# thepowerfuldeez/stylemc

Measured on AMD Instinct MI355X. Metric: find_direction images/sec @ FFHQ-1024 bs=4, 1/2/4/8 GPU; dir cosine-sim vs ref, higher is better.
Workload: dtype f32; 1 GPU; find_direction step: 2x StyleGAN2 S-space synthesis fwd + 1 bwd (HIP), CLIP ViT-B/32 fwd/bwd (HIP), IR-SE50 fwd/bwd (HIP), SGD; resolution=1024, batch_per_gpu=4, global_batch=4, n_seeds=129, parallelism=dp1, clip_type=small, clip_impl=hip, id_impl=hip, batched_loss_pairs=True, landmarks_loss_coef=0, conv_products=x3, vit_products=fp32, irse_products=fp32, direction_finite=True, world_size=1

## Files before the change

### include/stylemc_hip.h

```cpp
#ifndef STYLEMC_HIP_H
#define STYLEMC_HIP_H

#include <stdint.h>

#ifdef __cplusplus
extern "C" {
#endif

#define SMC_ABI_VERSION 6

#define SMC_OK 0
#define SMC_ERR_INVALID 1
#define SMC_ERR_UNSUPPORTED 2
#define SMC_ERR_LAUNCH 3

#define SMC_ACT_LINEAR 1
#define SMC_ACT_RELU 2
#define SMC_ACT_LRELU 3
#define SMC_ACT_TANH 4
#define SMC_ACT_SIGMOID 5
#define SMC_ACT_ELU 6
#define SMC_ACT_SELU 7
#define SMC_ACT_SOFTPLUS 8
#define SMC_ACT_SWISH 9
// ... 21 lines not shown
    int out_sy, out_sx;
    const float* wk;
    const float* wino_u;
    const void* wk_x3;
} smc_conv_phase;

int64_t smc_conv_weights_x3_bytes(int ntaps, int cin, int cout);
int smc_conv_weights_x3(const float* wk, int ntaps, int cin, int cout, void* wk_x3, void* stream);

#define SMC_EPI_STORE 0
#define SMC_EPI_MODACT 1
#define SMC_EPI_PRELU 2
#define SMC_EPI_PRELU_GRAD 3
#define SMC_EPI_AFFINE 4

typedef struct {
    int mode;
    const float* d;
    const float* noise;
    int64_t noise_nstride;
    const float* noise_strength;
    const float* bias;
    int act;
    float alpha, gain, clamp;
    float* u_save;
    const float* scale_c;
    const float* alpha_c;
    const float* act_ref;
    const float* residual;
    int residual_stride;
    int grad_from_y;
} smc_conv_epilogue;

int smc_conv_gemm_last_x3(void);
int64_t smc_conv_gemm_workspace_size(int n, int cin, int cout, int y_h, int y_w, const smc_conv_phase* phases,
                                     int nphases);

#define SMC_ROUTE_SPLIT_K 1
#define SMC_ROUTE_PER_SAMPLE 2
#define SMC_ROUTE_PRESCALE 4
#define SMC_ROUTE_WSAMPLE 8
int smc_conv_gemm_last_route(void);
int smc_conv_gemm_last_route_flags(void);
int smc_conv_gemm_route_count(void);
const char* smc_conv_gemm_route_name(int route);

int smc_conv_gemm_f32(const float* x, int n, int cin, int in_h, int in_w, float* y, int cout, int y_h, int y_w,
                      const smc_conv_phase* phases, int nphases, const float* s_in, const smc_conv_epilogue* epi,
                      float* workspace, int64_t workspace_bytes, void* stream);

int64_t smc_conv_gemm_aux_workspace_size(int n, int cin, int cout, int y_h, int y_w, const smc_conv_phase* phases,
                                         int nphases);
int smc_conv_gemm_aux_f32(const float* x, int n, int cin, int in_h, int in_w, float* y, int cout, int y_h, int y_w,
                          const smc_conv_phase* phases, int nphases, const float* s_in, const smc_conv_epilogue* epi,
                          float* workspace, int64_t workspace_bytes, void* stream);

int smc_conv3x3_wino_supported(int n, int cin, int cout, int h, int w);
int smc_conv3x3_wino_f32(const float* x, int n, int cin, int h, int w, float* y, int cout, const float* uw,
                         const float* s_in, const smc_conv_epilogue* epi, void* stream);
int64_t smc_conv3x3_wino_workspace_size(int n, int cin, int cout, int h, int w);
int smc_conv3x3_wino_ws_f32(const float* x, int n, int cin, int h, int w, float* y, int cout, const float* uw,
                            const float* s_in, const smc_conv_epilogue* epi, float* workspace, int64_t workspace_bytes,
                            void* stream);
int smc_set_wino_x3(int mode);
int smc_wino_weights_f32(const float* w, int cout, int cin, int flip, float* uw, void* stream);

int smc_conv3x3_wino4_supported(int n, int cin, int cout, int h, int w);
int smc_conv3x3_wino4_f32(const float* x, int n, int cin, int h, int w, float* y, int cout, const float* uw,
                          const float* s_in, const smc_conv_epilogue* epi, void* stream);
int smc_wino4_weights_f32(const float* w, int cout, int cin, int flip, float* uw, void* stream);

int smc_wino_sp_supported(int n, int cin, int cout, int h, int w);
int64_t smc_wino_sp_workspace_size(int n, int cin, int cout, int h, int w);
int smc_wino_taps_f32(const smc_conv_phase* phase, int cin, int cout, float* uw, void* stream);
int smc_conv3x3_wino_sp_f32(const float* x, int n, int cin, int h, int w, float* y, int cout, const float* uw,
                            const smc_conv_epilogue* epi, float* workspace, int64_t workspace_bytes, void* stream);

int smc_modconv_epilogue_f32(const float* src, int nsplit, int64_t split_stride, float* y, int n, int c, int h,
                             int w, const smc_conv_epilogue* epi, void* stream);

int smc_modconv_blur_act_f32(const float* t, int nsplit, int64_t split_stride, float* y, int n, int c, int t_h,
                             int t_w, int t_pitch, int y_h, int y_w, const float* f, int fh, int fw, int padx0,
                             int pady0, float fgain, int flip, const smc_conv_epilogue* epi, void* stream);

int smc_modconv_blur_act_bwd_f32(const float* g, const float* u, float* dt, float* dd, int n, int c, int u_h, int u_w,
                                 int t_h, int t_w, int t_pitch, const float* f, int fh, int fw, int padx0, int pady0,
                                 float fgain, int flip, const smc_conv_epilogue* epi, void* workspace,
                                 int64_t workspace_bytes, void* stream);
int64_t smc_modconv_blur_act_bwd_workspace_size(int n, int c, int u_h, int u_w, int t_h, int t_w);

int smc_row_dot_f32(const float* a, int64_t lda, const float* b, int64_t ldb, float* out, int rows, int len,
                    void* stream);

int smc_direction_head_f32(const float* e, int64_t lde, const float* src, int64_t lds, const float* t, float* loss,
                           float* grad, int rows, int len, float eps, void* stream);

int smc_modconv_demod_f32(const float* s, const float* wsq, float* d, int n, int cin, int cout, float eps,
                          void* stream);

int smc_modconv_act_bwd_f32(const float* g, const float* u, float* du, float* dd, int n, int c, int h, int w,
                            const smc_conv_epilogue* epi, void* workspace, int64_t workspace_bytes, void* stream);
int64_t smc_modconv_act_bwd_workspace_size(int n, int c, int h, int w);

int smc_channel_dot_f32(const float* a, const float* b, const float* scale, float* out, float* a_scaled,
                        int64_t rows, int64_t len, int accumulate, void* stream);

int smc_modconv_demod_bwd_f32(const float* s, const float* d, const float* dd, const float* wsq, float* ds, int n,
                              int cin, int cout, void* stream);

int smc_torgb_fwd_f32(const float* x, const float* w, const float* s, const float* b, float* y, int n, int cin,
                      int cout, int h, int w_, float clamp, void* stream);

int smc_torgb_bwd_f32(const float* g, const float* y, const float* w, const float* s, float* dx, int n, int cin,
                      int cout, int h, int w_, float clamp, int scale, int accumulate, void* stream);

int smc_torgb_act_bwd_f32(const float* g_rgb, const float* y_rgb, const float* w, const float* s, float clamp_rgb,
                          const float* g_next, const float* y, float* du, int n, int cin, int cout, int h, int w_,
                          const smc_conv_epilogue* epi, void* stream);

int smc_face_crop_f32(const float* x, int64_t planes, int in_h, int in_w, int pool_h, int pool_w, int crop_y0,
                      int crop_x0, int crop_h, int crop_w, int out_h, int out_w, float* y, void* stream);
int smc_face_crop_bwd_f32(const float* dy, int64_t planes, int in_h, int in_w, int pool_h, int pool_w, int crop_y0,
                          int crop_x0, int crop_h, int crop_w, int out_h, int out_w, float* dx, void* stream);

int smc_clip_unprocess_f32(const float* img, int n, int channels, int in_h, int in_w, int out_h, int out_w,
                           const float* mean, const float* std_, float* y, void* stream);
int smc_clip_unprocess_bwd_f32(const float* img, const float* dy, int n, int channels, int in_h, int in_w, int out_h,
                               int out_w, const float* mean, const float* std_, float* dimg, void* stream);
int smc_clip_preprocess_nada_f32(const float* img, int n, int channels, int in_h, int in_w, int out_h, int out_w,
                                 const float* mean, const float* std_, float* y, void* stream);
int smc_clip_preprocess_nada_bwd_f32(const float* img, const float* dy, int n, int channels, int in_h, int in_w,
                                     int out_h, int out_w, const float* mean, const float* std_, float* dimg,
                                     void* stream);

#define SMC_LIN_ACT_NONE 0
#define SMC_LIN_ACT_QUICKGELU 1

typedef struct {
    const float* bias;
    const float* dact_pre;
    int ld_dact;
    int act;
    float* pre_save;
    int ld_pre;
    const float* residual;
    int ld_res;
} smc_linear_epilogue;

int64_t smc_linear_workspace_size(int M, int N, int K);
int smc_linear_f32(const float* a, int lda, const float* b, int ldb, float* c, int ldc, int M, int N, int K,
                   const smc_linear_epilogue* epi, float* workspace, int64_t workspace_bytes, void* stream);

int64_t smc_linear_counter_ints(int M, int N);
int smc_linear_ex_f32(const float* a, int lda, const float* b, int ldb, float* c, int ldc, int M, int N, int K,
                      const smc_linear_epilogue* epi, float* workspace, int64_t workspace_bytes, const float* bt,
                      const void* planes, int* counters, void* stream);
int64_t smc_linear_x3_planes_bytes(int K, int N);
int smc_linear_x3_planes(const float* b, int ldb, int K, int N, void* planes, void* stream);

#define SMC_LIN_REDUCE_NONE 0
#define SMC_LIN_REDUCE_KERNEL 1
#define SMC_LIN_REDUCE_INLAUNCH 2
int smc_linear_last_route(void);
int smc_linear_last_nsplit(void);
int smc_linear_last_reduce(void);
int smc_linear_route_count(void);
// ... 87 lines not shown
```

### stylemc_amd/_hip.py

```python
import contextlib
import ctypes
import os
import threading

import torch

PKG = os.path.dirname(os.path.abspath(__file__))
LIB_PATH = os.environ.get("SMC_HIP_LIB", os.path.join(PKG, "_lib", "libstylemc_hip.so"))

c_int, c_int64, c_float, c_void_p, c_char_p = ctypes.c_int, ctypes.c_int64, ctypes.c_float, ctypes.c_void_p, ctypes.c_char_p

ACT_CODES = {"linear": 1, "relu": 2, "lrelu": 3, "tanh": 4, "sigmoid": 5, "elu": 6, "selu": 7, "softplus": 8,
             "swish": 9}
EPI_STORE, EPI_MODACT, EPI_PRELU, EPI_PRELU_GRAD, EPI_AFFINE = 0, 1, 2, 3, 4
ROUTE_SPLIT_K, ROUTE_PER_SAMPLE, ROUTE_PRESCALE, ROUTE_WSAMPLE = 1, 2, 4, 8


class ConvPhase(ctypes.Structure):
    _fields_ = [("ntaps", c_int), ("tap_dy", c_int * 9), ("tap_dx", c_int * 9), ("in_stride", c_int),
                ("out_h", c_int), ("out_w", c_int), ("out_oy", c_int), ("out_ox", c_int), ("out_sy", c_int),
                ("out_sx", c_int), ("wk", c_void_p), ("wino_u", c_void_p), ("wk_x3", c_void_p)]


class ConvEpilogue(ctypes.Structure):
    _fields_ = [("mode", c_int), ("d", c_void_p), ("noise", c_void_p), ("noise_nstride", c_int64),
                ("noise_strength", c_void_p), ("bias", c_void_p), ("act", c_int), ("alpha", c_float),
                ("gain", c_float), ("clamp", c_float), ("u_save", c_void_p), ("scale_c", c_void_p),
                ("alpha_c", c_void_p), ("act_ref", c_void_p), ("residual", c_void_p), ("residual_stride", c_int),
                ("grad_from_y", c_int)]


class LinearEpilogue(ctypes.Structure):
    _fields_ = [("bias", c_void_p), ("dact_pre", c_void_p), ("ld_dact", c_int), ("act", c_int),
                ("pre_save", c_void_p), ("ld_pre", c_int), ("residual", c_void_p), ("ld_res", c_int)]


class VitConfig(ctypes.Structure):
    _fields_ = [("width", c_int), ("layers", c_int), ("heads", c_int), ("patch", c_int), ("grid", c_int),
                ("out_dim", c_int), ("in_ch", c_int), ("ln_eps", c_float), ("products", c_int)]


LIN_ACT_NONE, LIN_ACT_QUICKGELU = 0, 1
LIN_REDUCE_NONE, LIN_REDUCE_KERNEL, LIN_REDUCE_INLAUNCH = 0, 1, 2

P = c_void_p
_SIGS = {
    "smc_abi_version": (c_int, []),
    "smc_set_plan_batch": (c_int, [c_int, c_int]),
    "smc_conv_gemm_last_x3": (c_int, []),
    "smc_conv_gemm_last_route": (c_int, []),
    "smc_conv_gemm_last_route_flags": (c_int, []),
    "smc_conv_gemm_route_count": (c_int, []),
    "smc_conv_gemm_route_name": (c_char_p, [c_int]),
    "smc_last_error": (c_char_p, []),
    "smc_bias_act_f32": (c_int, [P, P, P, P, P, P, c_int64, c_int64, c_int64, c_int, c_int, c_float, c_float, c_float,
                                 P]),
    "smc_upfirdn2d_f32": (c_int, [P, P, P, c_int64] + [c_int] * 15 + [c_float, P]),
    "smc_conv_gemm_workspace_size": (c_int64, [c_int, c_int, c_int, c_int, c_int, P, c_int]),
    "smc_conv_gemm_f32": (c_int, [P, c_int, c_int, c_int, c_int, P, c_int, c_int, c_int, P, c_int, P, P, P, c_int64,
                                  P]),
    "smc_conv_gemm_aux_workspace_size": (c_int64, [c_int, c_int, c_int, c_int, c_int, P, c_int]),
    "smc_conv_gemm_aux_f32": (c_int, [P, c_int, c_int, c_int, c_int, P, c_int, c_int, c_int, P, c_int, P, P, P,
                                      c_int64, P]),
    "smc_conv_weights_x3_bytes": (c_int64, [c_int, c_int, c_int]),
    "smc_conv_weights_x3": (c_int, [P, c_int, c_int, c_int, P, P]),
    "smc_conv3x3_wino_supported": (c_int, [c_int, c_int, c_int, c_int, c_int]),
    "smc_conv3x3_wino_f32": (c_int, [P, c_int, c_int, c_int, c_int, P, c_int, P, P, P, P]),
    "smc_conv3x3_wino_workspace_size": (c_int64, [c_int, c_int, c_int, c_int, c_int]),
    "smc_set_wino_x3": (c_int, [c_int]),
    "smc_conv3x3_wino_ws_f32": (c_int, [P, c_int, c_int, c_int, c_int, P, c_int, P, P, P, P, c_int64, P]),
    "smc_wino_weights_f32": (c_int, [P, c_int, c_int, c_int, P, P]),
    "smc_conv3x3_wino4_supported": (c_int, [c_int, c_int, c_int, c_int, c_int]),
    "smc_conv3x3_wino4_f32": (c_int, [P, c_int, c_int, c_int, c_int, P, c_int, P, P, P, P]),
    "smc_wino4_weights_f32": (c_int, [P, c_int, c_int, c_int, P, P]),
    "smc_wino_sp_supported": (c_int, [c_int, c_int, c_int, c_int, c_int]),
    "smc_wino_sp_workspace_size": (c_int64, [c_int, c_int, c_int, c_int, c_int]),
    "smc_wino_taps_f32": (c_int, [P, c_int, c_int, P, P]),
    "smc_conv3x3_wino_sp_f32": (c_int, [P, c_int, c_int, c_int, c_int, P, c_int, P, P, P, c_int64, P]),
    "smc_modconv_epilogue_f32": (c_int, [P, c_int, c_int64, P, c_int, c_int, c_int, c_int, P, P]),
    "smc_modconv_blur_act_f32": (c_int, [P, c_int, c_int64, P, c_int, c_int, c_int, c_int, c_int, c_int, c_int, P,
                                         c_int, c_int, c_int, c_int, c_float, c_int, P, P]),
    "smc_modconv_blur_act_bwd_f32": (c_int, [P, P, P, P, c_int, c_int, c_int, c_int, c_int, c_int, c_int, P, c_int,
                                             c_int, c_int, c_int, c_float, c_int, P, P, c_int64, P]),
    "smc_modconv_blur_act_bwd_workspace_size": (c_int64, [c_int] * 6),
    "smc_modconv_demod_f32": (c_int, [P, P, P, c_int, c_int, c_int, c_float, P]),
    "smc_row_dot_f32": (c_int, [P, c_int64, P, c_int64, P, c_int, c_int, P]),
    "smc_direction_head_f32": (c_int, [P, c_int64, P, c_int64, P, P, P, c_int, c_int, c_float, P]),
    "smc_modconv_act_bwd_f32": (c_int, [P, P, P, P, c_int, c_int, c_int, c_int, P, P, c_int64, P]),
    "smc_modconv_act_bwd_workspace_size": (c_int64, [c_int] * 4),
    "smc_channel_dot_f32": (c_int, [P, P, P, P, P, c_int64, c_int64, c_int, P]),
    "smc_modconv_demod_bwd_f32": (c_int, [P, P, P, P, P, c_int, c_int, c_int, P]),
    "smc_torgb_fwd_f32": (c_int, [P, P, P, P, P, c_int, c_int, c_int, c_int, c_int, c_float, P]),
    "smc_torgb_bwd_f32": (c_int, [P, P, P, P, P, c_int, c_int, c_int, c_int, c_int, c_float, c_int, c_int, P]),
    "smc_torgb_act_bwd_f32": (c_int, [P, P, P, P, c_float, P, P, P, c_int, c_int, c_int, c_int, c_int, P, P]),
    "smc_face_crop_f32": (c_int, [P, c_int64] + [c_int] * 10 + [P, P]),
    "smc_face_crop_bwd_f32": (c_int, [P, c_int64] + [c_int] * 10 + [P, P]),
    "smc_clip_unprocess_f32": (c_int, [P] + [c_int] * 6 + [P, P, P, P]),
    "smc_clip_unprocess_bwd_f32": (c_int, [P, P] + [c_int] * 6 + [P, P, P, P]),
    "smc_clip_preprocess_nada_f32": (c_int, [P] + [c_int] * 6 + [P, P, P, P]),
    "smc_clip_preprocess_nada_bwd_f32": (c_int, [P, P] + [c_int] * 6 + [P, P, P, P]),
    "smc_linear_workspace_size": (c_int64, [c_int, c_int, c_int]),
    "smc_linear_f32": (c_int, [P, c_int, P, c_int, P, c_int, c_int, c_int, c_int, P, P, c_int64, P]),
    "smc_linear_counter_ints": (c_int64, [c_int, c_int]),
    "smc_linear_ex_f32": (c_int, [P, c_int, P, c_int, P, c_int, c_int, c_int, c_int, P, P, c_int64, P, P, P, P]),
    "smc_linear_x3_planes_bytes": (c_int64, [c_int, c_int]),
    "smc_linear_x3_planes": (c_int, [P, c_int, c_int, c_int, P, P]),
    "smc_linear_last_route": (c_int, []),
    "smc_linear_last_nsplit": (c_int, []),
    "smc_linear_last_reduce": (c_int, []),
    "smc_linear_route_count": (c_int, []),
    "smc_linear_route_name": (c_char_p, [c_int]),
    "smc_layernorm_fwd_f32": (c_int, [P, c_int64, P, P, P, c_int64, P, P, c_int, c_int, c_float, P]),
    "smc_layernorm_bwd_f32": (c_int, [P, c_int64, P, c_int64, P, P, P, P, c_int64, P, c_int64, c_int, c_int, P]),
    "smc_attention_fwd_f32": (c_int, [P, P, P, c_int, c_int, c_int, c_int, c_float, P]),
    "smc_attention_bwd_f32": (c_int, [P, P, P, P, c_int, c_int, c_int, c_int, c_float, P]),
    "smc_attention_causal_fwd_f32": (c_int, [P, P, c_int, c_int, c_int, c_int, c_float, P]),
    "smc_patch_im2col_f32": (c_int, [P, P, c_int, c_int, c_int, c_int, c_int, P]),
    "smc_vit_packed_floats": (c_int64, [P]),
    "smc_vit_saved_floats": (c_int64, [P, c_int]),
    "smc_vit_pack_x3": (c_int, [P, P, P]),
    "smc_vit_workspace_bytes": (c_int64, [P, c_int]),
    "smc_vit_forward_f32": (c_int, [P, P, P, c_int, P, P, P, c_int64, P]),
    "smc_vit_backward_f32": (c_int, [P, P, P, c_int, c_int, P, P, P, c_int64, P]),
    "smc_irse_saved_floats": (c_int64, [P, c_int]),
    "smc_irse_workspace_bytes": (c_int64, [P, c_int]),
    "smc_irse_forward_f32": (c_int, [P, P, c_int, P, P, P, c_int64, P]),
    "smc_irse_backward_f32": (c_int, [P, P, c_int, c_int, P, P, P, c_int64, P]),
}

_lib = None
_lock = threading.Lock()


def exported_symbols():
    return sorted(_SIGS)


def load(path=None):
    global _lib
    if _lib is not None and path is None:
        return _lib
    with _lock:
        if _lib is not None and path is None:
            return _lib
        p = path or LIB_PATH
        if not os.path.exists(p):
            raise RuntimeError(f"stylemc_amd: HIP kernel library not found at {p}; build it with "
                               f"`python -m stylemc_amd.build` (there is no CPU fallback)")
        lib = ctypes.CDLL(p, mode=ctypes.RTLD_LOCAL)
        for name, (res, args) in _SIGS.items():
            fn = getattr(lib, name)
            fn.restype = res
            fn.argtypes = args
        if lib.smc_abi_version() != 6:
            raise RuntimeError("stylemc_amd: ABI version mismatch, rebuild the library")
        if path is None:
            _lib = lib
        return lib


def check(rc, name):
    if rc != 0:
        msg = load().smc_last_error().decode(errors="replace")
        raise RuntimeError(f"{name} failed (code {rc}): {msg}")
# ... 89 lines not shown
```

### stylemc_amd/csrc/conv_gemm.hip

```cpp
#include <algorithm>
#include <cstdlib>
#include <type_traits>

#include "common.hpp"

namespace {

constexpr int BK = 16;
constexpr int NT = 256;
typedef float f32x16 __attribute__((ext_vector_type(16)));

struct PhaseDev {
    int ntaps;
    int dy[9];
    int dx[9];
    int in_stride;
    int out_h, out_w, out_oy, out_ox, out_sy, out_sx;
    const float* wk;
    int64_t wstride;
    const short* wx3;
    int64_t wx3_stride;
};

struct GemmParams {
    const float* x;
    int n, cin, in_h, in_w;
    float* y;
    int cout, y_h, y_w;
    PhaseDev ph[4];
    int nphases;
    const float* s;
    int mode;
    const float* d;
    const float* noise;
    int64_t noise_nstride;
    const float* noise_strength;
    const float* bias;
    int act;
    float alpha, gain, clamp;
    float* u_save;
    smc::EpiExt ext;
    int nsplit;
    int64_t split_stride;
    int per_sample;
    int ntn;
};

template <int WO, int WM, int TO, int TM>
__device__ __forceinline__ void gemm_epilogue(const GemmParams& p, const PhaseDev& ph, const f32x16 (&acc)[TO][TM],
                                              int m0, int o0, int M, int hw_out, int split, int wo, int wm, int kh,
                                              int l32, float* lds) {
    constexpr int BO = WO * TO * 32;
    constexpr int BM = WM * TM * 32;
    const int64_t plane = (int64_t)p.y_h * p.y_w;
    if (p.nsplit > 1) {
        float* dst = p.y + (int64_t)split * p.split_stride;
#pragma unroll
        for (int j = 0; j < TM; ++j) {
            const int mc = m0 + wm * TM * 32 + j * 32 + l32;
            if (mc >= M) continue;
            const int en = mc / hw_out;
            const int erem = mc - en * hw_out;
            const int ea = erem / ph.out_w;
            const int64_t pix = (int64_t)(ph.out_oy + ph.out_sy * ea) * p.y_w + ph.out_ox + ph.out_sx * (erem - ea * ph.out_w);
#pragma unroll
            for (int i = 0; i < TO; ++i)
#pragma unroll
                for (int r = 0; r < 16; ++r) {
                    const int o = o0 + wo * TO * 32 + i * 32 + (r & 3) + 8 * (r >> 2) + 4 * kh;
                    if (o < p.cout) dst[((int64_t)en * p.cout + o) * plane + pix] = acc[i][j][r];
                }
        }
        return;
    }
    const int tid = threadIdx.x;
    const int en0 = m0 / hw_out;
    const bool one_img = (min(m0 + BM, M) - 1) / hw_out == en0;
    const int mode = p.mode;
    __syncthreads();
    for (int t = tid; t < BO; t += NT) {
        const int o = o0 + t;
        float mul = 1.f, add = 0.f, al = 0.f;
        if (o < p.cout) {
            if (mode == SMC_EPI_MODACT) {
                mul = (p.d && one_img ? p.d[(int64_t)en0 * p.cout + o] : 1.f) * (p.ext.scale_c ? p.ext.scale_c[o] : 1.f);
                add = p.bias ? p.bias[o] : 0.f;
            } else if (mode == SMC_EPI_PRELU || mode == SMC_EPI_AFFINE) {
                mul = p.ext.scale_c ? p.ext.scale_c[o] : 1.f;
                add = p.bias ? p.bias[o] : 0.f;
            }
            if ((mode == SMC_EPI_PRELU || mode == SMC_EPI_PRELU_GRAD) && p.ext.alpha_c) al = p.ext.alpha_c[o];
        }
        lds[t] = mul;
        lds[BO + t] = add;
        lds[2 * BO + t] = al;
    }
    __syncthreads();
    const float nstr = p.noise_strength ? *p.noise_strength : 1.f;
    const int rs = p.ext.rs;
    const int rh = p.y_h / rs, rw = p.y_w / rs;
    auto body = [&](auto mode_c, auto kind_c) {
        constexpr int MODE = decltype(mode_c)::value;
        constexpr int KIND = decltype(kind_c)::value;
        constexpr bool EX_REF = MODE == SMC_EPI_PRELU_GRAD;
#pragma unroll
        for (int j = 0; j < TM; ++j) {
            const int mc = m0 + wm * TM * 32 + j * 32 + l32;
            if (mc >= M) continue;
            const int en = mc / hw_out;
            const int erem = mc - en * hw_out;
            const int ea = erem / ph.out_w;
            const int eb = erem - ea * ph.out_w;
            const int yy = ph.out_oy + ph.out_sy * ea;
            const int xx = ph.out_ox + ph.out_sx * eb;
            const int64_t pix = (int64_t)yy * p.y_w + xx;
            const bool res_here = p.ext.residual && yy % rs == 0 && xx % rs == 0;
            const bool need_ex = EX_REF || p.ext.residual;
            float nz = 0.f;
            if (MODE == SMC_EPI_MODACT && p.noise) nz = p.noise[en * p.noise_nstride + pix] * nstr;
#pragma unroll
            for (int i = 0; i < TO; ++i) {
                const int ol0 = wo * TO * 32 + i * 32 + 4 * kh;
                float ex[16];
                if (need_ex) {
#pragma unroll
                    for (int r = 0; r < 16; ++r) {
                        const int o = min(o0 + ol0 + (r & 3) + 8 * (r >> 2), p.cout - 1);
                        if (EX_REF) ex[r] = p.ext.act_ref[((int64_t)en * p.cout + o) * plane + pix];
                        else ex[r] = res_here ? p.ext.residual[(((int64_t)en * p.cout + o) * rh + yy / rs) * rw + xx / rs] : 0.f;
// ... 150 lines not shown
            ws_[q] = s_on_w ? sblk[ci0 + wkk] : 1.f;
        }
    };
    auto store_step = [&](int stage) {
        float* Ws = smem + stage * TILE;
        float* Xs = Ws + BKT * BO;
#pragma unroll
        for (int r = 0; r < XR; ++r) {
            float v = xr[r];
            if (s_on_x) {
                const float4 sv = sr[r / 4];
                v *= (r & 3) == 0 ? sv.x : (r & 3) == 1 ? sv.y : (r & 3) == 2 ? sv.z : sv.w;
            }
            if constexpr (!BUF) v = xok ? v : 0.f;
            Xs[(kr0 + r) * BM + ml] = v;
        }
#pragma unroll
        for (int q = 0; q < WPT; ++q) {
            const int v = tid + q * NT;
            const int wkk = v / (BO / 4), wc4 = v - wkk * (BO / 4);
            float4 w = wr[q];
            const float sc = (o0 + wc4 * 4 >= p.cout) ? 0.f : ws_[q];
            w.x *= sc; w.y *= sc; w.z *= sc; w.w *= sc;
            if (v < WV) *reinterpret_cast<float4*>(&Ws[wkk * BO + wc4 * 4]) = w;
        }
    };

    f32x16 acc[TO][TM];
#pragma unroll
    for (int i = 0; i < TO; ++i)
#pragma unroll
        for (int j = 0; j < TM; ++j)
#pragma unroll
            for (int r = 0; r < 16; ++r) acc[i][j][r] = 0.f;

    const int kh = lane >> 5, l32 = lane & 31;
    int stage = 0;
    if (ks_begin < ks_end) {
        load_step(ks_begin);
        store_step(0);
    }
    __syncthreads();
    for (int ks = ks_begin; ks < ks_end; ++ks) {
        const bool more = ks + 1 < ks_end;
        if (more) load_step(ks + 1);
        const float* Ws = smem + stage * TILE;
        const float* Xs = Ws + BKT * BO;
        const float* wrow = Ws + kh * BO + wo * TO * 32 + l32;
        const float* xrow = Xs + kh * BM + wm * TM * 32 + l32;
#pragma unroll
        for (int k0 = 0; k0 < BKT; k0 += 16) {
            float af[8][TO], bf[8][TM];
#pragma unroll
            for (int q = 0; q < 8; ++q) {
#pragma unroll
                for (int i = 0; i < TO; ++i) af[q][i] = wrow[(k0 + 2 * q) * BO + i * 32];
#pragma unroll
                for (int j = 0; j < TM; ++j) bf[q][j] = xrow[(k0 + 2 * q) * BM + j * 32];
            }
            __builtin_amdgcn_sched_barrier(0);
#pragma unroll
            for (int q = 0; q < 8; ++q)
#pragma unroll
                for (int i = 0; i < TO; ++i)
#pragma unroll
                    for (int j = 0; j < TM; ++j)
                        acc[i][j] = __builtin_amdgcn_mfma_f32_32x32x2f32(af[q][i], bf[q][j], acc[i][j], 0, 0, 0);
        }
        if (more) store_step(stage ^ 1);
        __syncthreads();
        stage ^= 1;
    }

    gemm_epilogue<WO, WM, TO, TM>(p, ph, acc, m0, o0, M, hw_out, split, wo, wm, kh, l32, smem);
}


template <int WF>
struct WeightDma {
    static constexpr int ww = WF % 1024 == 0 ? 4 : 1;
    static constexpr int bytes = ww * 4;
};

template <int N>
__device__ __forceinline__ void wait_vmcnt() {
    asm volatile("s_waitcnt vmcnt(%0)" ::"n"(N) : "memory");
}

template <int WO, int WM, int TO, int TM, int BKT, int NST, int TAG = 0>
__global__ __launch_bounds__(NT, 2) void conv_gemm_lds_kernel(GemmParams p) {
    static_assert(WO * WM == 4, "4 waves");
    constexpr int BO = WO * TO * 32;
    constexpr int BM = WM * TM * 32;
    constexpr int TILE = BKT * (BO + BM);
    constexpr int NCH = BM / 64;
    static_assert(NCH >= 1 && NCH <= 4 && 4 % NCH == 0, "BM in {64,128,256}");
    constexpr int RSTEP = 4 / NCH;
    constexpr int XI = BKT * NCH / 4;
    constexpr int WF = BKT * BO;
    constexpr int WW = WeightDma<WF>::ww;
    static_assert(WF % (256 * WW) == 0, "weight slab must split evenly over the 4 waves");
    constexpr int WI = WF / (256 * WW);
    constexpr int PER = XI + WI;
    static_assert(NST >= 2 && NST <= 4 && PER * (NST - 2) <= 63, "vmcnt range");
    __shared__ __attribute__((aligned(16))) float smem[NST * TILE];

    const int tid = threadIdx.x;
    const int lane = tid & 63;
    const int wave = __builtin_amdgcn_readfirstlane(tid >> 6);
    const int wo = wave / WM, wm = wave % WM;
    const int phase = blockIdx.z / p.nsplit;
    const int split = blockIdx.z - phase * p.nsplit;
    const PhaseDev& ph = p.ph[phase];
    const int hw_out = ph.out_h * ph.out_w;
    int tm = blockIdx.x, tn = blockIdx.y;
    if (p.ntn) {
        const int nwg = gridDim.x, orig = blockIdx.x;
        const int xcd = orig % 8, q8 = nwg / 8, r8 = nwg % 8;
        const int wgid = (xcd < r8 ? xcd * (q8 + 1) : r8 * (q8 + 1) + (xcd - r8) * q8) + orig / 8;
        tm = wgid / p.ntn;
        tn = wgid - tm * p.ntn;
    }
    int M = p.n * hw_out;
    int m0 = tm * BM;
    if (p.per_sample) {
        const int tps = (hw_out + BM - 1) / BM;
        const int nb = tm / tps;
        if (nb >= p.n) return;
        m0 = nb * hw_out + (tm - nb * tps) * BM;
        M = (nb + 1) * hw_out;
    }
    if (m0 >= M) return;
    const int o0 = tn * BO;
    const int cpk = p.cin / BKT;
    const int ks_total = ph.ntaps * cpk;
    const int ks_begin = (int)((int64_t)ks_total * split / p.nsplit);
    const int ks_end = (int)((int64_t)ks_total * (split + 1) / p.nsplit);

    const int cw = wave % NCH, r0 = wave / NCH;
    const int m = m0 + cw * 64 + lane;
    const bool mvalid = m < M;
    int nn = 0, a = 0, b = 0;
    if (mvalid) {
        nn = m / hw_out;
        const int rem = m - nn * hw_out;
        a = rem / ph.out_w;
        b = rem - a * ph.out_w;
    }
    const int in_hw = p.in_h * p.in_w;
    const __amdgpu_buffer_rsrc_t xrsrc = __builtin_amdgcn_make_buffer_rsrc(
        (void*)p.x, (short)0, (int)((int64_t)p.n * p.cin * in_hw * 4), 0x00020000);
    const int xvbase = nn * p.cin * in_hw * 4;
    const int ay = a * ph.in_stride, bx = b * ph.in_stride;
    const float* wk = ph.wk + (ph.wstride ? (int64_t)(m0 / hw_out) * ph.wstride : 0);

    auto issue = [&](int ks, int slot) {
        const int t = ks / cpk;
        const int ci0 = (ks - t * cpk) * BKT;
        const int iy = ay + ph.dy[t], ix = bx + ph.dx[t];
        const bool ok = mvalid && iy >= 0 && iy < p.in_h && ix >= 0 && ix < p.in_w;
        const int voff = ok ? xvbase + (iy * p.in_w + ix) * 4 : 0x7ffffff0;
        float* xs = smem + slot * TILE + BKT * BO;
#pragma unroll
        for (int j = 0; j < XI; ++j) {
            const int row = r0 + RSTEP * j;
            __builtin_amdgcn_raw_ptr_buffer_load_lds(
                xrsrc, (__attribute__((address_space(3))) void*)(xs + row * BM + cw * 64), 4, voff,
                (ci0 + row) * in_hw * 4, 0, 0);
        }
        float* ws = smem + slot * TILE;
        const float* wrow = wk + ((int64_t)t * p.cin + ci0) * p.cout + o0;
#pragma unroll
        for (int j = 0; j < WI; ++j) {
            const int f0 = (wave + 4 * j) * 64 * WW;
            const int f = f0 + lane * WW;
            const int row = f / BO, col = f - row * BO;
            const void* src = (const void*)(wrow + (int64_t)row * p.cout + col);
            auto* dst = (__attribute__((address_space(3))) void*)(ws + f0);
            if constexpr (WW == 4) __builtin_amdgcn_global_load_lds(src, dst, 16, 0, 0);
            else __builtin_amdgcn_global_load_lds(src, dst, 4, 0, 0);
        }
    };

    f32x16 acc[TO][TM];
#pragma unroll
    for (int i = 0; i < TO; ++i)
#pragma unroll
        for (int j = 0; j < TM; ++j)
#pragma unroll
            for (int r = 0; r < 16; ++r) acc[i][j][r] = 0.f;

    const int kh = lane >> 5, l32 = lane & 31;
    int issued = ks_begin;
#pragma unroll
    for (int q = 0; q < NST - 1; ++q) {
        if (issued < ks_end) {
            issue(issued, (issued - ks_begin) % NST);
            ++issued;
        }
    }
    for (int ks = ks_begin; ks < ks_end; ++ks) {
        const int ahead = issued - ks - 1;
        if constexpr (NST == 2) {
            wait_vmcnt<0>();
        } else if constexpr (NST == 3) {
            if (ahead >= 1) wait_vmcnt<PER>();
            else wait_vmcnt<0>();
        } else {
            if (ahead >= 2) wait_vmcnt<2 * PER>();
            else if (ahead == 1) wait_vmcnt<PER>();
            else wait_vmcnt<0>();
        }
        __builtin_amdgcn_s_barrier();
        asm volatile("" ::: "memory");
        const int slot = (ks - ks_begin) % NST;
        const float* Ws = smem + slot * TILE;
        const float* Xs = Ws + BKT * BO;
        const float* wrow = Ws + kh * BO + wo * TO * 32 + l32;
        const float* xrow = Xs + kh * BM + wm * TM * 32 + l32;
#pragma unroll
        for (int k0 = 0; k0 < BKT; k0 += 16) {
            float af[8][TO], bf[8][TM];
            auto frag = [&](int q) {
#pragma unroll
                for (int i = 0; i < TO; ++i) af[q][i] = wrow[(k0 + 2 * q) * BO + i * 32];
#pragma unroll
                for (int j = 0; j < TM; ++j) bf[q][j] = xrow[(k0 + 2 * q) * BM + j * 32];
            };
            frag(0);
            frag(1);
            __builtin_amdgcn_sched_barrier(0);
#pragma unroll
            for (int q = 0; q < 8; ++q) {
#pragma unroll
                for (int i = 0; i < TO; ++i)
#pragma unroll
                    for (int j = 0; j < TM; ++j)
                        acc[i][j] = __builtin_amdgcn_mfma_f32_32x32x2f32(af[q][i], bf[q][j], acc[i][j], 0, 0, 0);
                __builtin_amdgcn_sched_barrier(0);
                if (q == 0 && k0 == 0 && issued < ks_end) {
                    issue(issued, (issued - ks_begin) % NST);
                    ++issued;
                }
                if (q + 2 < 8) frag(q + 2);
                __builtin_amdgcn_sched_barrier(0);
            }
        }
        asm volatile("s_waitcnt lgkmcnt(0)" ::: "memory");
    }
    gemm_epilogue<WO, WM, TO, TM>(p, ph, acc, m0, o0, M, hw_out, split, wo, wm, kh, l32, smem);
}


typedef short bf16x8 __attribute__((ext_vector_type(8)));

__device__ __forceinline__ void x3_split8(const float (&x)[8], bf16x8 (&t)[3]) {
    unsigned u0[8], u1[8], u2[8];
#pragma unroll
    for (int j = 0; j < 8; ++j) {
        const unsigned u = __float_as_uint(x[j]);
        const float r1 = x[j] - __uint_as_float(u & 0xffff0000u);
        const unsigned v = __float_as_uint(r1);
        const float r2 = r1 - __uint_as_float(v & 0xffff0000u);
        u0[j] = u;
        u1[j] = v;
        u2[j] = __float_as_uint(r2);
    }
    typedef unsigned u32x4 __attribute__((ext_vector_type(4)));
    u32x4 w0, w1, w2;
#pragma unroll
    for (int j = 0; j < 4; ++j) {
        w0[j] = __builtin_amdgcn_perm(u0[2 * j + 1], u0[2 * j], 0x07060302u);
        w1[j] = __builtin_amdgcn_perm(u1[2 * j + 1], u1[2 * j], 0x07060302u);
        w2[j] = __builtin_amdgcn_perm(u2[2 * j + 1], u2[2 * j], 0x07060302u);
    }
    t[0] = __builtin_bit_cast(bf16x8, w0);
    t[1] = __builtin_bit_cast(bf16x8, w1);
    t[2] = __builtin_bit_cast(bf16x8, w2);
}

__device__ __forceinline__ f32x16 x3_mma(const bf16x8 (&a)[3], const bf16x8 (&b)[3], f32x16 acc) {
    acc = __builtin_amdgcn_mfma_f32_32x32x16_bf16(a[2], b[0], acc, 0, 0, 0);
    acc = __builtin_amdgcn_mfma_f32_32x32x16_bf16(a[1], b[1], acc, 0, 0, 0);
    acc = __builtin_amdgcn_mfma_f32_32x32x16_bf16(a[0], b[2], acc, 0, 0, 0);
    acc = __builtin_amdgcn_mfma_f32_32x32x16_bf16(a[1], b[0], acc, 0, 0, 0);
    acc = __builtin_amdgcn_mfma_f32_32x32x16_bf16(a[0], b[1], acc, 0, 0, 0);
    return __builtin_amdgcn_mfma_f32_32x32x16_bf16(a[0], b[0], acc, 0, 0, 0);
}

__global__ __launch_bounds__(256) void x3_weights_kernel(const float* wk, const float* s_in, short* out, int ntaps,
                                                         int cin, int cout, int n) {
    const int64_t per = (int64_t)ntaps * cin * cout;
    const int64_t total = per * n;
    for (int64_t e = blockIdx.x * (int64_t)blockDim.x + threadIdx.x; e < total; e += (int64_t)gridDim.x * blockDim.x) {
        const int ee = (int)(e & 7);
        int64_t r = e >> 3;
        const int o = (int)(r % cout);
        r /= cout;
        const int kq = (int)(r & 1);
        r >>= 1;
        const int c16 = (int)(r % (cin / 16));
        r /= cin / 16;
        const int t = (int)(r % ntaps);
        const int nn = (int)(r / ntaps);
        const int ci = c16 * 16 + kq * 8 + ee;
        const float v = wk[((int64_t)t * cin + ci) * cout + o] * (s_in ? s_in[(int64_t)nn * cin + ci] : 1.f);
        const unsigned u = __float_as_uint(v);
        const float r1 = v - __uint_as_float(u & 0xffff0000u);
        const unsigned w = __float_as_uint(r1);
        const float r2 = r1 - __uint_as_float(w & 0xffff0000u);
        const unsigned term[3] = {u >> 16, w >> 16, __float_as_uint(r2) >> 16};
        short* dst = out + nn * per * 3;
#pragma unroll
        for (int sidx = 0; sidx < 3; ++sidx)
            dst[((((int64_t)t * (cin / 16) + c16) * 3 + sidx) * 2 + kq) * ((int64_t)cout * 8) + (int64_t)o * 8 + ee] =
                (short)term[sidx];
    }
}

#ifndef SMC_X3_NST
#define SMC_X3_NST 2
#endif
#ifndef SMC_X3_K32_SMALL
#define SMC_X3_K32_SMALL 1
#endif
#ifndef SMC_X3_WO1
#define SMC_X3_WO1 1
#endif
#ifndef SMC_X3_WO1_K16
#define SMC_X3_WO1_K16 1
#endif
#ifndef SMC_X3_PROBE
#define SMC_X3_PROBE 0
#endif

#ifndef SMC_X3_WIDE
#define SMC_X3_WIDE 1
#endif

template <int WO, int WM, int TO, int TM, int BKT, int NST = SMC_X3_NST, int TAG = 0, bool AS = false>
__global__ __launch_bounds__(NT, 2) void conv_gemm_x3_kernel(GemmParams p) {
    static_assert(WO * WM == 4, "4 waves");
    static_assert(BKT % 16 == 0, "16-channel chunks");
    static_assert(!AS || (BKT == 16 && TM == 1 && NST == 2), "streamed A fragments: one 16-channel chunk per step");
    constexpr int BO = WO * TO * 32;
    constexpr int BM = WM * TM * 32;
    constexpr int NKC = BKT / 16;
    constexpr int WB = NKC * 6 * BO * 16;
    constexpr int XB = BKT * BM * 4;
    constexpr int STAGE = WB + XB;
    constexpr int NCH = BM / 64;
    static_assert(NCH >= 1 && NCH <= 4 && 4 % NCH == 0, "BM in {64,128,256}");
    constexpr int RSTEP = 4 / NCH;
    constexpr int XI = BKT * NCH / 4;
    static_assert(WB % 1024 == 0, "weight planes split into whole 1-KB DMAs");
    constexpr int WLI = WB / 1024;
    constexpr int WIW = (WLI + 3) / 4;
    constexpr int PER = XI + WIW;
    static_assert(NST >= 2 && NST <= 4 && PER * (NST - 2) <= 63, "vmcnt range");
    __shared__ __attribute__((aligned(16))) char smem[NST * STAGE];

    const int tid = threadIdx.x;
    const int lane = tid & 63;
    const int wave = __builtin_amdgcn_readfirstlane(tid >> 6);
    const int wo = wave / WM, wm = wave % WM;
    const int phase = blockIdx.z / p.nsplit;
    const int split = blockIdx.z - phase * p.nsplit;
    const PhaseDev& ph = p.ph[phase];
    const int hw_out = ph.out_h * ph.out_w;
    int tm = blockIdx.x, tn = blockIdx.y;
    if (p.ntn) {
// ... 302 lines not shown
#pragma unroll
        for (int j = 0; j < TM; ++j)
#pragma unroll
            for (int r = 0; r < 16; ++r) acc[i][j][r] = 0.f;

    const int kh = lane >> 5, l32 = lane & 31;
    if (ks_total > 0) issue(0, 0);
    for (int ks = 0; ks < ks_total; ++ks) {
        wait_vmcnt<0>();
        __builtin_amdgcn_s_barrier();
        asm volatile("" ::: "memory");
        const int slot = ks & 1;
        const float* Xs = smem + slot * STAGE + kh * PITCH + 3 + wm * TM * 32 + l32;
        const float* Ws = smem + slot * STAGE + C::XF + kh * BO + wo * TO * 32 + l32;
#pragma unroll
        for (int tt = 0; tt < 3; ++tt) {
#pragma unroll
            for (int k0 = 0; k0 < BKT; k0 += 8) {
                float af[4][TO], bf[4][TM];
#pragma unroll
                for (int q = 0; q < 4; ++q) {
#pragma unroll
                    for (int i = 0; i < TO; ++i) af[q][i] = Ws[(tt * BKT + k0 + 2 * q) * BO + i * 32];
#pragma unroll
                    for (int j = 0; j < TM; ++j) bf[q][j] = Xs[(k0 + 2 * q) * PITCH + tt + j * 32];
                }
                __builtin_amdgcn_sched_barrier(0);
#pragma unroll
                for (int q = 0; q < 4; ++q)
#pragma unroll
                    for (int i = 0; i < TO; ++i)
#pragma unroll
                        for (int j = 0; j < TM; ++j)
                            acc[i][j] = __builtin_amdgcn_mfma_f32_32x32x2f32(af[q][i], bf[q][j], acc[i][j], 0, 0, 0);
                __builtin_amdgcn_sched_barrier(0);
                if (tt == 0 && k0 == 0 && ks + 1 < ks_total) issue(ks + 1, slot ^ 1);
            }
        }
        asm volatile("s_waitcnt lgkmcnt(0)" ::: "memory");
    }
    gemm_epilogue<WO, WM, TO, TM>(p, ph, acc, m0, o0, p.n * hw, hw, 0, wo, wm, kh, l32, smem);
}

__global__ __launch_bounds__(256) void xscale_kernel(const float* x, const float* s, float* out, int64_t hw,
                                                     int64_t planes) {
    const int64_t per = hw / 4;
    const int64_t total = per * planes;
    for (int64_t v = blockIdx.x * (int64_t)blockDim.x + threadIdx.x; v < total; v += (int64_t)gridDim.x * blockDim.x) {
        const int64_t pl = v / per;
        const float sc = s[pl];
        float4 a = reinterpret_cast<const float4*>(x)[v];
        a.x *= sc; a.y *= sc; a.z *= sc; a.w *= sc;
        reinterpret_cast<float4*>(out)[v] = a;
    }
}

__global__ __launch_bounds__(256) void wscale_kernel(const float* wk, const float* s, float* out, int rows, int cin,
                                                     int cout, int n) {
    const int64_t per = (int64_t)rows * cout / 4;
    const int64_t total = per * n;
    for (int64_t v = blockIdx.x * (int64_t)blockDim.x + threadIdx.x; v < total; v += (int64_t)gridDim.x * blockDim.x) {
        const int64_t nn = v / per;
        const int64_t e = (v - nn * per) * 4;
        const int row = (int)(e / cout);
        float4 w = *reinterpret_cast<const float4*>(wk + e);
        const float sc = s[nn * cin + row % cin];
        w.x *= sc; w.y *= sc; w.z *= sc; w.w *= sc;
        *reinterpret_cast<float4*>(out + nn * (int64_t)rows * cout + e) = w;
    }
}


struct ConvTParams {
    const float* w[4][4];
};

template <int S>
struct ShiftPhases;
template <> struct ShiftPhases<0> { static constexpr int n = 4; static constexpr int p[4] = {0, 1, 2, 3}; };
template <> struct ShiftPhases<1> { static constexpr int n = 2; static constexpr int p[4] = {0, 1, 0, 0}; };
template <> struct ShiftPhases<2> { static constexpr int n = 2; static constexpr int p[4] = {0, 2, 0, 0}; };
template <> struct ShiftPhases<3> { static constexpr int n = 1; static constexpr int p[4] = {0, 0, 0, 0}; };

__host__ __device__ constexpr int shift_nph(int s) { return s == 0 ? 4 : (s == 3 ? 1 : 2); }

template <int S, int TO, int TM, int BKT, int BO, int BM>
__device__ __forceinline__ void convt_mma(const float* Ws, const float* Xs, int wo, int wm, int kh, int l32,
                                          f32x16 (&acc)[4][TO][TM]) {
    constexpr int NP = ShiftPhases<S>::n;
#pragma unroll
    for (int k0 = 0; k0 < BKT; k0 += 4) {
        float af[2][NP][TO], bf[2][TM];
#pragma unroll
        for (int q = 0; q < 2; ++q) {
            const int kk = k0 + 2 * q + kh;
#pragma unroll
            for (int j = 0; j < TM; ++j) bf[q][j] = Xs[kk * BM + wm * TM * 32 + j * 32 + l32];
#pragma unroll
            for (int ph = 0; ph < NP; ++ph)
#pragma unroll
                for (int i = 0; i < TO; ++i) af[q][ph][i] = Ws[(ph * BKT + kk) * BO + wo * TO * 32 + i * 32 + l32];
        }
        __builtin_amdgcn_sched_barrier(0);
#pragma unroll
        for (int q = 0; q < 2; ++q)
#pragma unroll
            for (int ph = 0; ph < NP; ++ph)
#pragma unroll
                for (int i = 0; i < TO; ++i)
#pragma unroll
                    for (int j = 0; j < TM; ++j)
                        acc[ShiftPhases<S>::p[ph]][i][j] = __builtin_amdgcn_mfma_f32_32x32x2f32(
                            af[q][ph][i], bf[q][j], acc[ShiftPhases<S>::p[ph]][i][j], 0, 0, 0);
    }
}

template <int WO, int WM, int TO, int TM, int BKT>
__global__ __launch_bounds__(NT, 1) void convt_gemm_kernel(GemmParams p, ConvTParams q) {
    static_assert(WO * WM == 4, "4 waves");
    constexpr int BO = WO * TO * 32;
    constexpr int BM = WM * TM * 32;
    constexpr int XR = BKT * BM / NT;
    constexpr int WV = BKT * BO / 4;
    constexpr int WPT = (WV + NT - 1) / NT;
    constexpr int TILE = BKT * (4 * BO + BM);
    static_assert(NT % BM == 0 && XR % 4 == 0, "thread->position map");
    __shared__ float smem[2 * TILE];

    const int tid = threadIdx.x, lane = tid & 63, wave = tid >> 6;
    const int wo = wave / WM, wm = wave % WM;
    const int gh = p.in_h + 1, gw = p.in_w + 1, hw_g = gh * gw;
    const int M = p.n * hw_g;
    const int m0 = blockIdx.x * BM;
    const int o0 = blockIdx.y * BO;
    const int split = blockIdx.z;
    const int cpk = p.cin / BKT;
    const int ks_total = 4 * cpk;
    const int ks_begin = (int)((int64_t)ks_total * split / p.nsplit);
    const int ks_end = (int)((int64_t)ks_total * (split + 1) / p.nsplit);

    const int ml = tid % BM, kr0 = (tid / BM) * XR;
    const int m = m0 + ml;
    const bool mvalid = m < M;
    int nn = 0, a = 0, b = 0;
    if (mvalid) {
        nn = m / hw_g;
        const int rem = m - nn * hw_g;
        a = rem / gw;
        b = rem - a * gw;
    }
    const int64_t in_hw = (int64_t)p.in_h * p.in_w;
    const float* xbase = p.x + (int64_t)nn * p.cin * in_hw + (int64_t)kr0 * in_hw;
    const bool has_s = p.s != nullptr;
    const float* swhere = has_s ? p.s + (int64_t)nn * p.cin + kr0 : p.x;

    float xr[XR];
    float4 sr[XR / 4];
    float4 wr[4][WPT];
    bool xok = false;

    auto load_step = [&](int ks) {
        const int c = ks >> 2, sh = ks & 3;
        const int ci0 = c * BKT;
        const int iy = a - (sh & 1), ix = b - ((sh >> 1) & 1);
        xok = mvalid && iy >= 0 && iy < p.in_h && ix >= 0 && ix < p.in_w;
        const float* src = xbase + (int64_t)ci0 * in_hw + (xok ? (int64_t)iy * p.in_w + ix : 0);
#pragma unroll
        for (int r = 0; r < XR; ++r) xr[r] = src[r * in_hw];
// ... 20 lines not shown
        float* Xs = Ws + 4 * BKT * BO;
#pragma unroll
        for (int r = 0; r < XR; ++r) {
            const float4 sv = sr[r / 4];
            const float sc = has_s ? ((r & 3) == 0 ? sv.x : (r & 3) == 1 ? sv.y : (r & 3) == 2 ? sv.z : sv.w) : 1.f;
            Xs[(kr0 + r) * BM + ml] = xok ? xr[r] * sc : 0.f;
        }
        const int nph = shift_nph(sh);
#pragma unroll
        for (int ph = 0; ph < 4; ++ph) {
            if (ph >= nph) break;
#pragma unroll
            for (int t = 0; t < WPT; ++t) {
                const int v = tid + t * NT;
                const int wkk = v / (BO / 4), wc4 = v - wkk * (BO / 4);
                float4 w = wr[ph][t];
                if (o0 + wc4 * 4 >= p.cout) w = make_float4(0.f, 0.f, 0.f, 0.f);
                if (v < WV) *reinterpret_cast<float4*>(&Ws[(ph * BKT + wkk) * BO + wc4 * 4]) = w;
            }
        }
    };

    f32x16 acc[4][TO][TM];
#pragma unroll
    for (int ph = 0; ph < 4; ++ph)
#pragma unroll
        for (int i = 0; i < TO; ++i)
#pragma unroll
            for (int j = 0; j < TM; ++j)
#pragma unroll
                for (int r = 0; r < 16; ++r) acc[ph][i][j][r] = 0.f;

    const int kh = lane >> 5, l32 = lane & 31;
    int stage = 0;
    if (ks_begin < ks_end) {
        load_step(ks_begin);
        store_step(0, ks_begin & 3);
    }
    __syncthreads();
    for (int ks = ks_begin; ks < ks_end; ++ks) {
        const bool more = ks + 1 < ks_end;
        if (more) load_step(ks + 1);
        const float* Ws = smem + stage * TILE;
        const float* Xs = Ws + 4 * BKT * BO;
        switch (ks & 3) {
            case 0: convt_mma<0, TO, TM, BKT, BO, BM>(Ws, Xs, wo, wm, kh, l32, acc); break;
            case 1: convt_mma<1, TO, TM, BKT, BO, BM>(Ws, Xs, wo, wm, kh, l32, acc); break;
            case 2: convt_mma<2, TO, TM, BKT, BO, BM>(Ws, Xs, wo, wm, kh, l32, acc); break;
            default: convt_mma<3, TO, TM, BKT, BO, BM>(Ws, Xs, wo, wm, kh, l32, acc); break;
        }
        if (more) store_step(stage ^ 1, (ks + 1) & 3);
        __syncthreads();
        stage ^= 1;
    }

    float* dst = p.nsplit > 1 ? p.y + (int64_t)split * p.split_stride : p.y;
    const int64_t plane = (int64_t)p.y_h * p.y_w;
#pragma unroll
    for (int j = 0; j < TM; ++j) {
        const int mc = m0 + wm * TM * 32 + j * 32 + l32;
        if (mc >= M) continue;
        const int en = mc / hw_g;
        const int erem = mc - en * hw_g;
        const int ea = erem / gw;
        const int eb = erem - ea * gw;
#pragma unroll
        for (int i = 0; i < TO; ++i) {
#pragma unroll
            for (int r = 0; r < 16; ++r) {
                const int o = o0 + wo * TO * 32 + i * 32 + (r & 3) + 8 * (r >> 2) + 4 * kh;
                if (o >= p.cout) continue;
                float* row0 = dst + ((int64_t)en * p.cout + o) * plane + (int64_t)(2 * ea) * p.y_w + 2 * eb;
                row0[0] = acc[0][i][j][r];
                if (eb < p.in_w) row0[1] = acc[1][i][j][r];
                if (ea < p.in_h) {
                    row0[p.y_w] = acc[2][i][j][r];
                    if (eb < p.in_w) row0[p.y_w + 1] = acc[3][i][j][r];
                }
            }
        }
    }
}

struct ConvTTaps {
    int tap[4][4];
};

template <int S>
__host__ __device__ constexpr int shift_phase(int j) {
    return S == 0 ? j : (S == 1 ? (j ? 1 : 0) : (S == 2 ? (j ? 2 : 0) : 0));
}

template <int S, int TO, int TM, int BKT, int BO, int BM>
__device__ __forceinline__ void convt_lds_mma(const float* Ws, const float* Xs, int wo, int wm, int kh, int l32,
                                              f32x16 (&acc)[4][TO][TM]) {
    constexpr int NP = shift_nph(S);
    const float* wrow = Ws + kh * BO + wo * TO * 32 + l32;
    const float* xrow = Xs + kh * BM + wm * TM * 32 + l32;
    float af[2][NP][TO], bf[2][TM];
    auto frag = [&](int q, int b) {
#pragma unroll
        for (int j = 0; j < TM; ++j) bf[b][j] = xrow[(2 * q) * BM + j * 32];
#pragma unroll
        for (int ph = 0; ph < NP; ++ph)
#pragma unroll
            for (int i = 0; i < TO; ++i) af[b][ph][i] = wrow[(ph * BKT + 2 * q) * BO + i * 32];
    };
    frag(0, 0);
#pragma unroll
    for (int q = 0; q < BKT / 2; ++q) {
        if (q + 1 < BKT / 2) frag(q + 1, (q + 1) & 1);
        __builtin_amdgcn_sched_barrier(0);
#pragma unroll
        for (int ph = 0; ph < NP; ++ph)
#pragma unroll
            for (int i = 0; i < TO; ++i)
#pragma unroll
                for (int j = 0; j < TM; ++j)
                    acc[shift_phase<S>(ph)][i][j] = __builtin_amdgcn_mfma_f32_32x32x2f32(
                        af[q & 1][ph][i], bf[q & 1][j], acc[shift_phase<S>(ph)][i][j], 0, 0, 0);
        __builtin_amdgcn_sched_barrier(0);
    }
}

template <int WO, int WM, int TO, int TM, int BKT>
__global__ __launch_bounds__(NT, 2) void convt_lds_kernel(GemmParams p, ConvTTaps tt) {
    static_assert(WO * WM == 4, "4 waves");
    constexpr int BO = WO * TO * 32;
    constexpr int BM = WM * TM * 32;
    constexpr int NCH = BM / 64;
    static_assert(NCH >= 1 && NCH <= 4 && 4 % NCH == 0, "BM in {64,128,256}");
    constexpr int RSTEP = 4 / NCH;
    constexpr int XI = BKT * NCH / 4;
    constexpr int WSL = BKT * BO;
    static_assert(WSL % 256 == 0, "weight slabs split into whole 1-KB DMAs");
    constexpr int TILE = BKT * BM + 4 * WSL;
    __shared__ __attribute__((aligned(16))) float smem[2 * TILE];

    const int tid = threadIdx.x;
    const int lane = tid & 63;
    const int wave = __builtin_amdgcn_readfirstlane(tid >> 6);
    const int wo = wave / WM, wm = wave % WM;
    const int gh = p.in_h + 1, gw = p.in_w + 1, hw_g = gh * gw;
    int tm = blockIdx.x, tn = blockIdx.y;
    if (p.ntn) {
        const int nwg = gridDim.x, orig = blockIdx.x;
        const int xcd = orig % 8, q8 = nwg / 8, r8 = nwg % 8;
        const int wgid = (xcd < r8 ? xcd * (q8 + 1) : r8 * (q8 + 1) + (xcd - r8) * q8) + orig / 8;
        tm = wgid / p.ntn;
        tn = wgid - tm * p.ntn;
    }
    int M = p.n * hw_g;
    int m0 = tm * BM;
    if (p.per_sample) {
        const int tps = (hw_g + BM - 1) / BM;
        const int nb = tm / tps;
        if (nb >= p.n) return;
        m0 = nb * hw_g + (tm - nb * tps) * BM;
        M = (nb + 1) * hw_g;
    }
    if (m0 >= M) return;
    const int o0 = tn * BO;
    const int split = blockIdx.z;
    const int cpk = p.cin / BKT;
    const int c_begin = (int)((int64_t)cpk * split / p.nsplit);
    const int c_end = (int)((int64_t)cpk * (split + 1) / p.nsplit);
    const int ks_begin = 4 * c_begin, ks_end = 4 * c_end;

    const int cw = wave % NCH, r0 = wave / NCH;
    const int m = m0 + cw * 64 + lane;
    const bool mvalid = m < M;
    int nn = 0, a = 0, b = 0;
    if (mvalid) {
        nn = m / hw_g;
// ... 15 lines not shown
        const int voff = ok ? xvbase + (iy * p.in_w + ix) * 4 : 0x7ffffff0;
        float* xs = smem + slot * TILE;
#pragma unroll
        for (int j = 0; j < XI; ++j) {
            const int row = r0 + RSTEP * j;
            __builtin_amdgcn_raw_ptr_buffer_load_lds(
                xrsrc, (__attribute__((address_space(3))) void*)(xs + row * BM + cw * 64), 4, voff,
                (ci0 + row) * in_hw * 4, 0, 0);
        }
        float* ws = xs + BKT * BM;
        const int nph = shift_nph(sh);
        for (int j = wave; j < nph * (WSL / 256); j += 4) {
            const int pj = j / (WSL / 256);
            const int phase = sh == 0 ? pj : (sh == 1 ? (pj ? 1 : 0) : (sh == 2 ? (pj ? 2 : 0) : 0));
            const int f = (j - pj * (WSL / 256)) * 256 + lane * 4;
            const int row = f / BO, col = f - row * BO;
            const PhaseDev& q = p.ph[phase];
            const float* src = q.wk + (q.wstride ? (int64_t)wn * q.wstride : 0) +
                               ((int64_t)tt.tap[sh][phase] * p.cin + ci0 + row) * p.cout + o0 + col;
            __builtin_amdgcn_global_load_lds((const void*)src,
                                             (__attribute__((address_space(3))) void*)(ws + pj * WSL + f - lane * 4),
                                             16, 0, 0);
        }
    };

    f32x16 acc[4][TO][TM];
#pragma unroll
    for (int ph = 0; ph < 4; ++ph)
#pragma unroll
        for (int i = 0; i < TO; ++i)
#pragma unroll
            for (int j = 0; j < TM; ++j)
#pragma unroll
                for (int r = 0; r < 16; ++r) acc[ph][i][j][r] = 0.f;

    const int kh = lane >> 5, l32 = lane & 31;
    if (ks_begin < ks_end) issue(ks_begin, 0);
    auto step = [&](auto S_, int ks) {
        constexpr int S = decltype(S_)::value;
        wait_vmcnt<0>();
        __builtin_amdgcn_s_barrier();
        asm volatile("" ::: "memory");
        if (ks + 1 < ks_end) issue(ks + 1, (S + 1) & 1);
        const float* Xs = smem + (S & 1) * TILE;
        convt_lds_mma<S, TO, TM, BKT, BO, BM>(Xs + BKT * BM, Xs, wo, wm, kh, l32, acc);
        asm volatile("s_waitcnt lgkmcnt(0)" ::: "memory");
    };
    for (int ks = ks_begin; ks < ks_end; ks += 4) {
        step(std::integral_constant<int, 0>{}, ks);
        step(std::integral_constant<int, 1>{}, ks + 1);
        step(std::integral_constant<int, 2>{}, ks + 2);
        step(std::integral_constant<int, 3>{}, ks + 3);
    }

    float* dst = p.nsplit > 1 ? p.y + (int64_t)split * p.split_stride : p.y;
    const int64_t plane = (int64_t)p.y_h * p.y_w;
#pragma unroll
    for (int j = 0; j < TM; ++j) {
        const int mc = m0 + wm * TM * 32 + j * 32 + l32;
        if (mc >= M) continue;
        const int en = mc / hw_g;
        const int erem = mc - en * hw_g;
        const int ea = erem / gw;
        const int eb = erem - ea * gw;
#pragma unroll
        for (int i = 0; i < TO; ++i) {
#pragma unroll
            for (int r = 0; r < 16; ++r) {
                const int o = o0 + wo * TO * 32 + i * 32 + (r & 3) + 8 * (r >> 2) + 4 * kh;
                float* row0 = dst + ((int64_t)en * p.cout + o) * plane + (int64_t)(2 * ea) * p.y_w + 2 * eb;
                row0[0] = acc[0][i][j][r];
                if (eb < p.in_w) row0[1] = acc[1][i][j][r];
                if (ea < p.in_h) {
                    row0[p.y_w] = acc[2][i][j][r];
                    if (eb < p.in_w) row0[p.y_w + 1] = acc[3][i][j][r];
                }
            }
        }
    }
}

template <int WO, int WM, int TO, int TM>
__global__ __launch_bounds__(NT, 2) void convt_x3_kernel(GemmParams p, ConvTTaps tt) {
    static_assert(WO * WM == 4, "4 waves");
    constexpr int BKT = 16;
    constexpr int BO = WO * TO * 32;
    constexpr int BM = WM * TM * 32;
    constexpr int NCH = BM / 64;
    static_assert(NCH >= 1 && NCH <= 4 && 4 % NCH == 0, "BM in {64,128,256}");
    constexpr int RSTEP = 4 / NCH;
    constexpr int XI = BKT * NCH / 4;
    constexpr int PB = 6 * BO * 16;
    static_assert(PB % 1024 == 0, "phase planes split into whole 1-KB DMAs");
    constexpr int XB = BKT * BM * 4;
    constexpr int STAGE = XB + 4 * PB;
    __shared__ __attribute__((aligned(16))) char smem[2 * STAGE];

    const int tid = threadIdx.x;
    const int lane = tid & 63;
    const int wave = __builtin_amdgcn_readfirstlane(tid >> 6);
    const int wo = wave / WM, wm = wave % WM;
    const int gh = p.in_h + 1, gw = p.in_w + 1, hw_g = gh * gw;
    int tm = blockIdx.x, tn = blockIdx.y;
    if (p.ntn) {
        const int nwg = gridDim.x, orig = blockIdx.x;
        const int xcd = orig % 8, q8 = nwg / 8, r8 = nwg % 8;
        const int wgid = (xcd < r8 ? xcd * (q8 + 1) : r8 * (q8 + 1) + (xcd - r8) * q8) + orig / 8;
        tm = wgid / p.ntn;
        tn = wgid - tm * p.ntn;
    }
    int M = p.n * hw_g;
    int m0 = tm * BM;
    if (p.per_sample) {
        const int tps = (hw_g + BM - 1) / BM;
        const int nb = tm / tps;
        if (nb >= p.n) return;
        m0 = nb * hw_g + (tm - nb * tps) * BM;
        M = (nb + 1) * hw_g;
    }
    if (m0 >= M) return;
    const int o0 = tn * BO;
    const int split = blockIdx.z;
    const int cpk = p.cin / BKT;
    const int c_begin = (int)((int64_t)cpk * split / p.nsplit);
    const int c_end = (int)((int64_t)cpk * (split + 1) / p.nsplit);
    const int ks_begin = 4 * c_begin, ks_end = 4 * c_end;

    const int cw = wave % NCH, r0 = wave / NCH;
    const int m = m0 + cw * 64 + lane;
    const bool mvalid = m < M;
    int nn = 0, a = 0, b = 0;
    if (mvalid) {
        nn = m / hw_g;
        const int rem = m - nn * hw_g;
        a = rem / gw;
        b = rem - a * gw;
    }
    const int in_hw = p.in_h * p.in_w;
    const __amdgpu_buffer_rsrc_t xrsrc = __builtin_amdgcn_make_buffer_rsrc(
        (void*)p.x, (short)0, (int)((int64_t)p.n * p.cin * in_hw * 4), 0x00020000);
    const int xvbase = nn * p.cin * in_hw * 4;
    const int wn = m0 / hw_g;
    const int c16n = p.cin / 16;

    auto issue = [&](int ks, int slot) {
        const int c = ks >> 2, sh = ks & 3;
        const int ci0 = c * BKT;
        const int iy = a - (sh & 1), ix = b - (sh >> 1);
        const bool ok = mvalid && iy >= 0 && iy < p.in_h && ix >= 0 && ix < p.in_w;
        const int voff = ok ? xvbase + (iy * p.in_w + ix) * 4 : 0x7ffffff0;
        char* st = smem + slot * STAGE;
        float* xs = reinterpret_cast<float*>(st);
#pragma unroll
        for (int j = 0; j < XI; ++j) {
            const int row = r0 + RSTEP * j;
            __builtin_amdgcn_raw_ptr_buffer_load_lds(
                xrsrc, (__attribute__((address_space(3))) void*)(xs + row * BM + cw * 64), 4, voff,
                (ci0 + row) * in_hw * 4, 0, 0);
        }
        const int nph = shift_nph(sh);
        for (int j = wave; j < nph * (PB / 1024); j += 4) {
            const int pj = j / (PB / 1024);
            const int phase = sh == 0 ? pj : (sh == 1 ? (pj ? 1 : 0) : (sh == 2 ? (pj ? 2 : 0) : 0));
            const int L = (j - pj * (PB / 1024)) * 64 + lane;
            const int run = L / BO, o = L - run * BO;
            const PhaseDev& q = p.ph[phase];
            const short* src = q.wx3 + (q.wx3_stride ? (int64_t)wn * q.wx3_stride : 0) +
                               ((((int64_t)tt.tap[sh][phase] * c16n + ci0 / 16) * 6 + run) * p.cout + o0 + o) * 8;
            __builtin_amdgcn_global_load_lds((const void*)src, (__attribute__((address_space(3))) void*)(st + XB + j * 1024),
                                             16, 0, 0);
        }
    };

    f32x16 acc[4][TO][TM];
#pragma unroll
    for (int ph = 0; ph < 4; ++ph)
#pragma unroll
        for (int i = 0; i < TO; ++i)
#pragma unroll
            for (int j = 0; j < TM; ++j)
#pragma unroll
                for (int r = 0; r < 16; ++r) acc[ph][i][j][r] = 0.f;

    const int kh = lane >> 5, l32 = lane & 31;
    if (ks_begin < ks_end) issue(ks_begin, 0);
    auto step = [&](auto S_, int ks) {
        constexpr int S = decltype(S_)::value;
        constexpr int NP = shift_nph(S);
        wait_vmcnt<0>();
        __builtin_amdgcn_s_barrier();
        asm volatile("" ::: "memory");
        const char* st = smem + (S & 1) * STAGE;
        const float* xcol = reinterpret_cast<const float*>(st) + wm * TM * 32 + l32;
        bf16x8 bt[TM][3];
#pragma unroll
        for (int j = 0; j < TM; ++j) {
            float xv[8];
#pragma unroll
            for (int e = 0; e < 8; ++e) xv[e] = xcol[(8 * kh + e) * BM + j * 32];
            x3_split8(xv, bt[j]);
        }
        __builtin_amdgcn_sched_barrier(0);
        if (ks + 1 < ks_end) issue(ks + 1, (S + 1) & 1);
#pragma unroll
        for (int pj = 0; pj < NP; ++pj) {
            const short* Wp = reinterpret_cast<const short*>(st + XB + pj * PB);
            bf16x8 at[TO][3];
#pragma unroll
            for (int i = 0; i < TO; ++i)
#pragma unroll
                for (int s = 0; s < 3; ++s)
                    at[i][s] = *reinterpret_cast<const bf16x8*>(Wp + (((s * 2 + kh) * BO) + wo * TO * 32 + i * 32 + l32) * 8);
#pragma unroll
            for (int i = 0; i < TO; ++i)
#pragma unroll
                for (int j = 0; j < TM; ++j)
                    acc[shift_phase<S>(pj)][i][j] = x3_mma(at[i], bt[j], acc[shift_phase<S>(pj)][i][j]);
        }
        asm volatile("s_waitcnt lgkmcnt(0)" ::: "memory");
    };
    for (int ks = ks_begin; ks < ks_end; ks += 4) {
        step(std::integral_constant<int, 0>{}, ks);
        step(std::integral_constant<int, 1>{}, ks + 1);
        step(std::integral_constant<int, 2>{}, ks + 2);
        step(std::integral_constant<int, 3>{}, ks + 3);
    }

    float* dst = p.nsplit > 1 ? p.y + (int64_t)split * p.split_stride : p.y;
    const int64_t plane = (int64_t)p.y_h * p.y_w;
#pragma unroll
    for (int j = 0; j < TM; ++j) {
        const int mc = m0 + wm * TM * 32 + j * 32 + l32;
        if (mc >= M) continue;
        const int en = mc / hw_g;
        const int erem = mc - en * hw_g;
        const int ea = erem / gw;
        const int eb = erem - ea * gw;
#pragma unroll
        for (int i = 0; i < TO; ++i) {
#pragma unroll
            for (int r = 0; r < 16; ++r) {
                const int o = o0 + wo * TO * 32 + i * 32 + (r & 3) + 8 * (r >> 2) + 4 * kh;
                float* row0 = dst + ((int64_t)en * p.cout + o) * plane + (int64_t)(2 * ea) * p.y_w + 2 * eb;
                row0[0] = acc[0][i][j][r];
                if (eb < p.in_w) row0[1] = acc[1][i][j][r];
                if (ea < p.in_h) {
                    row0[p.y_w] = acc[2][i][j][r];
                    if (eb < p.in_w) row0[p.y_w + 1] = acc[3][i][j][r];
                }
            }
        }
    }
}

bool convt_structure(int cin, int cout, int in_h, int in_w, int y_h, int y_w, const smc_conv_phase* ph, int nph,
                     const smc_conv_epilogue* epi, ConvTParams* q) {
    if (nph != 4 || y_h != 2 * in_h + 1 || y_w != 2 * in_w + 1) return false;
    if (epi && (epi->mode != SMC_EPI_STORE || epi->residual)) return false;
    ConvTParams t{};
    int count = 0;
    for (int k = 0; k < 4; ++k) {
        const int py = k >> 1, px = k & 1;
        const smc_conv_phase& f = ph[k];
        if (f.in_stride != 1 || f.out_sy != 2 || f.out_sx != 2 || f.out_oy != py || f.out_ox != px) return false;
        for (int tp = 0; tp < f.ntaps; ++tp) {
            const int dy = f.tap_dy[tp], dx = f.tap_dx[tp];
            if ((dy != 0 && dy != -1) || (dx != 0 && dx != -1)) return false;
            const int s = (dy == -1 ? 1 : 0) + (dx == -1 ? 2 : 0);
            if (t.w[s][k]) return false;
            t.w[s][k] = f.wk + (int64_t)tp * cin * cout;
            ++count;
        }
    }
    if (count != 9) return false;
    for (int s = 0; s < 4; ++s)
        for (int k = 0; k < 4; ++k) {
            const bool want = s == 0 || (s == 1 && (k == 0 || k == 1)) || (s == 2 && (k == 0 || k == 2)) || (s == 3 && k == 0);
            if (want != (t.w[s][k] != nullptr)) return false;
        }
    if (q) *q = t;
    return true;
}

bool convt_fusable(int cin, int cout, int in_h, int in_w, int y_h, int y_w, const smc_conv_phase* ph, int nph,
                   const smc_conv_epilogue* epi, ConvTParams* q) {
    return cout <= 32 && convt_structure(cin, cout, in_h, in_w, y_h, y_w, ph, nph, epi, q);
}

struct ConvTCfg {
    int bo, bm, id;
};

ConvTCfg convt_cfg(int cout) {
    if (cout % 128 == 0) return {128, 64, 0};
    if (cout % 64 == 0) return {64, 128, 1};
    return {32, 128, 3};
}

int plan_split_convt(int n, int cin, int cout, int in_h, int in_w) {
    const ConvTCfg c = convt_cfg(cout);
    const int64_t M = (int64_t)smc::plan_batch(n) * (in_h + 1) * (in_w + 1);
    const int64_t blocks = smc::ceil_div(M, c.bm) * smc::ceil_div(cout, c.bo);
    const int ks = 4 * (cin / BK);
    const int64_t target = 2LL * smc::device_cu_count();
    if (blocks >= target) return 1;
    int s = (int)smc::ceil_div(target, blocks > 0 ? blocks : 1);
    int cap = ks / 4;
    if (cap > 16) cap = 16;
    if (s > cap) s = cap;
    return s < 1 ? 1 : s;
}

struct ConvTL {
    int bo, bm, id;
};

bool convt_lds_plan(int n, int cin, int cout, int in_h, int in_w, int y_h, int y_w, const smc_conv_phase* ph, int nph,
                    const smc_conv_epilogue* epi, ConvTTaps* tt, ConvTL* cfg) {
    ConvTParams q{};
    if (!convt_structure(cin, cout, in_h, in_w, y_h, y_w, ph, nph, epi, &q)) return false;
    if (cin % 16 != 0 || cout % 32 != 0 || cout > 64 || (int64_t)n * cin * in_h * in_w * 4 >= (1LL << 31)) return false;
    if (tt) {
        for (int sh = 0; sh < 4; ++sh)
            for (int k = 0; k < 4; ++k)
                tt->tap[sh][k] = q.w[sh][k] ? (int)((q.w[sh][k] - ph[k].wk) / ((int64_t)cin * cout)) : -1;
    }
    if (cfg) *cfg = cout % 64 == 0 ? ConvTL{64, 128, 1} : ConvTL{32, 128, 0};
    return true;
}

int plan_split_convt_lds(int n, int cin, int cout, int in_h, int in_w, const ConvTL& c, bool per_sample) {
    n = smc::plan_batch(n);
    const int64_t hw_g = (int64_t)(in_h + 1) * (in_w + 1);
    const int64_t mt = per_sample ? n * smc::ceil_div(hw_g, c.bm) : smc::ceil_div(n * hw_g, c.bm);
    const int64_t blocks = mt * (cout / c.bo);
    const int64_t target = 2LL * smc::device_cu_count();
    if (blocks >= target) return 1;
    int s = (int)smc::ceil_div(target, blocks > 0 ? blocks : 1);
    int cap = (cin / 16) / 2;
    if (cap > 16) cap = 16;
    if (s > cap) s = cap;
    return s < 1 ? 1 : s;
}

struct Cfg {
    int bo, bm;
};

int pick_cfg(int cout, Cfg* c) {
    if (cout % 128 == 0) { *c = {128, 128}; return 0; }
    if (cout % 64 == 0) { *c = {64, 128}; return 5; }
    if (cout % 32 == 0 || cout == 16) { *c = {32, 128}; return 4; }
    return -1;
}

int plan_split(int n, int cin, int cout, const smc_conv_phase* ph, int nph, const Cfg& c, int target_per_cu = 2) {
    int64_t blocks = 0;
    int min_ks = 1 << 30;
    for (int i = 0; i < nph; ++i) {
        const int64_t M = (int64_t)smc::plan_batch(n) * ph[i].out_h * ph[i].out_w;
        blocks += smc::ceil_div(M, c.bm) * smc::ceil_div(cout, c.bo);
        const int ks = ph[i].ntaps * (cin / BK);
        if (ks < min_ks) min_ks = ks;
    }
    const int64_t target = (int64_t)target_per_cu * smc::device_cu_count();
    if (blocks >= target) return 1;
    int s = (int)smc::ceil_div(target, blocks > 0 ? blocks : 1);
    int cap = min_ks / 4;
    if (cap > 16) cap = 16;
    if (s > cap) s = cap;
    return s < 1 ? 1 : s;
}

bool lds_shape_ok(int n, int cin, int cout, int in_h, int in_w, const smc_conv_phase* ph, int nph, const Cfg& c,
                  bool* scaled_ok) {
    bool so = true;
    for (int i = 0; i < nph; ++i) so = so && ((int64_t)ph[i].out_h * ph[i].out_w) % c.bm == 0;
    if (scaled_ok) *scaled_ok = so;
    return cout % c.bo == 0 && cin % BK == 0 && (int64_t)n * cin * in_h * in_w * 4 < (1LL << 31);
}

bool row_ok(int n, int cin, int cout, int in_h, int in_w, int y_h, int y_w, const smc_conv_phase* ph, int nph,
            const Cfg& c, RowTaps* rt) {
    if (nph != 1 || cin % 16 != 0 || cout % c.bo != 0 || in_w % c.bm != 0 || in_w % 4 != 0) return false;
    const smc_conv_phase& q = ph[0];
    if (q.ntaps != 9 || q.in_stride != 1 || q.out_h != in_h || q.out_w != in_w || y_h != in_h || y_w != in_w ||
        q.out_oy != 0 || q.out_ox != 0 || q.out_sy != 1 || q.out_sx != 1)
        return false;
    int seen = 0;
    for (int t = 0; t < 9; ++t) {
        const int dy = q.tap_dy[t], dx = q.tap_dx[t];
        if (dy < -1 || dy > 1 || dx < -1 || dx > 1) return false;
        const int bit = 1 << ((dy + 1) * 3 + dx + 1);
        if (seen & bit) return false;
        seen |= bit;
        if (rt) rt->t[dy + 1][dx + 1] = t;
    }
    return seen == 511 && (int64_t)n * cin * in_h * in_w * 4 < (1LL << 31);
}

bool phases_x3(const smc_conv_phase* ph, int nph) {
    for (int i = 0; i < nph; ++i)
        if (!ph[i].wk_x3) return false;
    return nph > 0;
}

int64_t wsample_floats(int n, int cin, int cout, const smc_conv_phase* ph, int nph) {
    int64_t t = 0;
    for (int i = 0; i < nph; ++i) t += (int64_t)ph[i].ntaps * cin * cout;
    if (phases_x3(ph, nph)) t = (t * 3 + 1) / 2;
    return ((t * n + 63) / 64) * 64;
}

bool lds_bk32(int cfg, int cin) { return cfg == 0 && cin % 32 == 0 && cin >= 512; }

bool small_tile_ok(int n, int cin, int cout, int in_h, int in_w, const smc_conv_phase* ph, int nph, bool has_s,
                   const Cfg& base) {
    if (cout % 64 != 0) return false;
    int64_t blocks = 0;
    int taps_all = 0;
    for (int i = 0; i < nph; ++i) {
        blocks += smc::ceil_div((int64_t)smc::plan_batch(n) * ph[i].out_h * ph[i].out_w, base.bm) *
                  smc::ceil_div(cout, base.bo);
        taps_all += ph[i].ntaps;
    }
    if (blocks >= 128) return false;
    const Cfg sm{64, 64};
    bool scaled_ok = false;
    if (!lds_shape_ok(n, cin, cout, in_h, in_w, ph, nph, sm, &scaled_ok)) return false;
    return !has_s || scaled_ok || (int64_t)taps_all * cout <= (int64_t)in_h * in_w;
}

int64_t prescale_floats(int n, int cin, int cout, const smc_conv_phase* ph, int nph) {
    int64_t hw = 0;
    int taps_all = 0;
    for (int i = 0; i < nph; ++i) {
        if (ph[i].in_stride != 1) return 0;
        hw = std::max<int64_t>(hw, (int64_t)ph[i].out_h * ph[i].out_w);
        taps_all += ph[i].ntaps;
    }
    return hw <= (int64_t)taps_all * cout ? (((int64_t)n * cin * hw + 63) / 64) * 64 : 0;
}

int validate(const float* x, int n, int cin, int in_h, int in_w, float* y, int cout, int y_h, int y_w,
             const smc_conv_phase* phases, int nphases) {
    SMC_CHECK(x && y && phases, "smc_conv_gemm_f32: null pointer");
    SMC_CHECK(n >= 1 && in_h >= 1 && in_w >= 1 && y_h >= 1 && y_w >= 1, "smc_conv_gemm_f32: bad shape");
    SMC_CHECK(nphases >= 1 && nphases <= 4, "smc_conv_gemm_f32: 1..4 phases (got %d)", nphases);
    if (cin % BK != 0) {
        smc::set_error("smc_conv_gemm_f32: cin=%d must be a multiple of %d", cin, BK);
        return SMC_ERR_UNSUPPORTED;
    }
    Cfg c;
    if (pick_cfg(cout, &c) < 0) {
        smc::set_error("smc_conv_gemm_f32: cout=%d must be 16 or a multiple of 32", cout);
        return SMC_ERR_UNSUPPORTED;
    }
    for (int i = 0; i < nphases; ++i) {
        const smc_conv_phase& q = phases[i];
        SMC_CHECK(q.ntaps >= 1 && q.ntaps <= 9, "smc_conv_gemm_f32: phase %d ntaps=%d", i, q.ntaps);
        SMC_CHECK(q.in_stride >= 1 && q.out_h >= 1 && q.out_w >= 1 && q.out_sy >= 1 && q.out_sx >= 1,
                  "smc_conv_gemm_f32: phase %d bad geometry", i);
        SMC_CHECK(q.out_oy >= 0 && q.out_ox >= 0 && q.out_oy + q.out_sy * (q.out_h - 1) < y_h &&
                      q.out_ox + q.out_sx * (q.out_w - 1) < y_w,
                  "smc_conv_gemm_f32: phase %d writes outside y", i);
        SMC_CHECK(q.wk != nullptr && (reinterpret_cast<uintptr_t>(q.wk) & 15) == 0,
                  "smc_conv_gemm_f32: phase %d weights must be 16-B aligned", i);
    }
    return SMC_OK;
}

}

namespace {

#ifndef SMC_AUX_SPLIT_PER_CU
#define SMC_AUX_SPLIT_PER_CU 2
#endif
constexpr int kSplitPerCuAux = SMC_AUX_SPLIT_PER_CU;

int64_t workspace_size_impl(int n, int cin, int cout, int y_h, int y_w, const smc_conv_phase* phases, int nphases,
                            int split_per_cu) {
    Cfg c;
    if (pick_cfg(cout, &c) < 0 || cin % BK != 0 || nphases < 1 || nphases > 4 || !phases) return 0;
    int s;
    ConvTL tl;
    if (nphases == 4 && y_h % 2 == 1 && y_w % 2 == 1 &&
        convt_lds_plan(n, cin, cout, (y_h - 1) / 2, (y_w - 1) / 2, y_h, y_w, phases, nphases, nullptr, nullptr, &tl))
        s = std::max(plan_split_convt_lds(n, cin, cout, (y_h - 1) / 2, (y_w - 1) / 2, tl, true),
                     plan_split_convt_lds(n, cin, cout, (y_h - 1) / 2, (y_w - 1) / 2, tl, false));
    else if (nphases == 4 && y_h % 2 == 1 && y_w % 2 == 1 &&
             convt_fusable(cin, cout, (y_h - 1) / 2, (y_w - 1) / 2, y_h, y_w, phases, nphases, nullptr, nullptr))
        s = plan_split_convt(n, cin, cout, (y_h - 1) / 2, (y_w - 1) / 2);
    else
        s = plan_split(n, cin, cout, phases, nphases, c, split_per_cu);
    if (cout % 64 == 0) s = std::max(s, plan_split(n, cin, cout, phases, nphases, Cfg{64, 64}, split_per_cu));
    int64_t bytes = s > 1 ? (int64_t)s * n * cout * y_h * y_w * (int64_t)sizeof(float) : 0;
    bool scaled_ok = false;
    const int64_t pre = prescale_floats(n, cin, cout, phases, nphases);
    if (lds_shape_ok(n, cin, cout, 1, 1, phases, nphases, c, &scaled_ok) || pre > 0)
        bytes = ((bytes + 255) / 256) * 256 +
                std::max(wsample_floats(n, cin, cout, phases, nphases), pre) * (int64_t)sizeof(float);
    return bytes;
}

}

SMC_API int64_t smc_conv_gemm_workspace_size(int n, int cin, int cout, int y_h, int y_w, const smc_conv_phase* phases,
                                             int nphases) {
    return workspace_size_impl(n, cin, cout, y_h, y_w, phases, nphases, 2);
}

namespace {

thread_local int g_last_x3 = 0;

#define SMC_ROUTES(X)                                                   \
    X(R_CONVT_X3_1421, "convt_x3_kernel<1,4,2,1>")                      \
    X(R_CONVT_X3_2212, "convt_x3_kernel<2,2,1,2>")                      \
    X(R_CONVT_X3_1411, "convt_x3_kernel<1,4,1,1>")                      \
    X(R_CONVT_LDS_2212, "convt_lds_kernel<2,2,1,2,16>")                 \
    X(R_CONVT_LDS_1411, "convt_lds_kernel<1,4,1,1,16>")                 \
    X(R_CONVT_GEMM_2221, "convt_gemm_kernel<2,2,2,1,16>")               \
    X(R_CONVT_GEMM_1421, "convt_gemm_kernel<1,4,2,1,16>")               \
// ... 12 lines not shown
    X(R_X3_2211_16_T1, "conv_gemm_x3_kernel<2,2,1,1,16,NST,1>")         \
    X(R_X3_2211_32, "conv_gemm_x3_kernel<2,2,1,1,32>")                  \
    X(R_X3_2211_16, "conv_gemm_x3_kernel<2,2,1,1,16>")                  \
    X(R_X3_1411_32, "conv_gemm_x3_kernel<1,4,1,1,32>")                  \
    X(R_X3_1411_16, "conv_gemm_x3_kernel<1,4,1,1,16>")                  \
    X(R_X3_2212_32, "conv_gemm_x3_kernel<2,2,1,2,32>")                  \
    X(R_X3_2212_16, "conv_gemm_x3_kernel<2,2,1,2,16>")                  \
    X(R_ROW_1412, "conv_row_kernel<1,4,1,2,8>")                         \
    X(R_ROW_1422, "conv_row_kernel<1,4,2,2,8>")                         \
    X(R_LDS_2222_32_T1, "conv_gemm_lds_kernel<2,2,2,2,32,2,1>")         \
    X(R_LDS_2222_32, "conv_gemm_lds_kernel<2,2,2,2,32,2>")              \
    X(R_LDS_2222_16_T1, "conv_gemm_lds_kernel<2,2,2,2,16,2,1>")         \
    X(R_LDS_2222_16, "conv_gemm_lds_kernel<2,2,2,2,16,2>")              \
    X(R_LDS_2211_32_T1, "conv_gemm_lds_kernel<2,2,1,1,32,2,1>")         \
    X(R_LDS_2211_16_T1, "conv_gemm_lds_kernel<2,2,1,1,16,2,1>")         \
    X(R_LDS_2211_16, "conv_gemm_lds_kernel<2,2,1,1,16,2>")              \
    X(R_LDS_1411_16_T1, "conv_gemm_lds_kernel<1,4,1,1,16,2,1>")         \
    X(R_LDS_1411_16, "conv_gemm_lds_kernel<1,4,1,1,16,2>")              \
    X(R_LDS_2212_16_T1, "conv_gemm_lds_kernel<2,2,1,2,16,2,1>")         \
    X(R_LDS_2212_16, "conv_gemm_lds_kernel<2,2,1,2,16,2>")              \
    SMC_ROUTES_REG(X, 2222, "2,2,2,2")                                  \
    SMC_ROUTES_REG(X, 1411, "1,4,1,1")                                  \
    SMC_ROUTES_REG(X, 2212, "2,2,1,2")                                  \
    SMC_ROUTES_REG(X, 2211, "2,2,1,1")
#define SMC_ROUTES_REG(X, T, S)                                         \
    X(R_REG_##T##_32_BUF_T1, "conv_gemm_kernel<" S ",32,true,1>")       \
    X(R_REG_##T##_16_BUF_T1, "conv_gemm_kernel<" S ",16,true,1>")       \
    X(R_REG_##T##_32_BUF, "conv_gemm_kernel<" S ",32,true>")            \
    X(R_REG_##T##_32, "conv_gemm_kernel<" S ",32,false>")               \
    X(R_REG_##T##_16_BUF, "conv_gemm_kernel<" S ",16,true>")            \
    X(R_REG_##T##_16, "conv_gemm_kernel<" S ",16,false>")

enum Route {
    R_NONE = 0,
#define SMC_ROUTE_ENUM(id, name) id,
    SMC_ROUTES(SMC_ROUTE_ENUM)
#undef SMC_ROUTE_ENUM
    kRouteCount
};

constexpr const char* kRouteNames[] = {
    "none",
#define SMC_ROUTE_NAME(id, name) name,
    SMC_ROUTES(SMC_ROUTE_NAME)
#undef SMC_ROUTE_NAME
};
static_assert(sizeof(kRouteNames) / sizeof(kRouteNames[0]) == kRouteCount, "one name per route");
static_assert(R_REG_2211_16 == kRouteCount - 1, "the route list and the enum agree");

thread_local int g_last_route = R_NONE;
thread_local int g_last_flags = 0;

int conv_gemm_impl(const float* x, int n, int cin, int in_h, int in_w, float* y, int cout, int y_h, int y_w,
                   const smc_conv_phase* phases, int nphases, const float* s_in, const smc_conv_epilogue* epi,
                   float* workspace, int64_t workspace_bytes, void* stream, int tag) {
    g_last_x3 = 0;
    g_last_route = R_NONE;
    g_last_flags = 0;
    int rc = validate(x, n, cin, in_h, in_w, y, cout, y_h, y_w, phases, nphases);
    if (rc != SMC_OK) return rc;
    Cfg c;
    int cfg = pick_cfg(cout, &c);
    ConvTParams ctp{};
    ConvTTaps ctt{};
    ConvTL tl{};
    const bool x3 = phases_x3(phases, nphases);
    const bool convt_lds = convt_lds_plan(n, cin, cout, in_h, in_w, y_h, y_w, phases, nphases, epi, &ctt, &tl);
    const bool fused_t = !convt_lds && convt_fusable(cin, cout, in_h, in_w, y_h, y_w, phases, nphases, epi, &ctp);
    const int64_t pre_fl = prescale_floats(n, cin, cout, phases, nphases);
    const bool prescale = s_in && !fused_t && pre_fl > 0 && (int64_t)n * cin * in_h * in_w <= pre_fl &&
                          (in_h * in_w) % 4 == 0 && (reinterpret_cast<uintptr_t>(x) & 15) == 0;
    const float* s_prescale = s_in;
    if (prescale) s_in = nullptr;
    if (!fused_t && !convt_lds && small_tile_ok(n, cin, cout, in_h, in_w, phases, nphases, s_in != nullptr, c)) {
        cfg = 3;
        c = Cfg{64, 64};
    }
    if (SMC_X3_WIDE && x3 && !tag && !s_in && cfg == 0 && !fused_t && !convt_lds && cout % 256 == 0 &&
        plan_split(n, cin, cout, phases, nphases, Cfg{256, 128}) == 1 &&
        lds_shape_ok(n, cin, cout, in_h, in_w, phases, nphases, Cfg{256, 128}, nullptr)) {
        cfg = 6;
        c = Cfg{256, 128};
    }
    const bool t_per_sample = convt_lds && s_in && ((int64_t)(in_h + 1) * (in_w + 1)) % tl.bm != 0;
    const int nsplit = convt_lds ? plan_split_convt_lds(n, cin, cout, in_h, in_w, tl, t_per_sample)
                                 : fused_t ? plan_split_convt(n, cin, cout, in_h, in_w)
                                           : plan_split(n, cin, cout, phases, nphases, c, tag ? kSplitPerCuAux : 2);
    const int64_t plane_elems = (int64_t)n * cout * y_h * y_w;
    if (nsplit > 1) {
        const int64_t need = nsplit * plane_elems * (int64_t)sizeof(float);
        SMC_CHECK(workspace && workspace_bytes >= need, "smc_conv_gemm_f32: workspace %lld < %lld bytes",
                  (long long)workspace_bytes, (long long)need);
    }
    if (nsplit > 1) g_last_flags |= SMC_ROUTE_SPLIT_K;
    if (prescale) {
        g_last_flags |= SMC_ROUTE_PRESCALE;
        const int64_t part = nsplit > 1 ? ((nsplit * plane_elems * (int64_t)sizeof(float) + 255) / 256) * 256 : 0;
        const int64_t need = part + pre_fl * (int64_t)sizeof(float);
        SMC_CHECK(workspace && workspace_bytes >= need, "smc_conv_gemm_f32: workspace %lld < %lld bytes",
                  (long long)workspace_bytes, (long long)need);
        float* xs = reinterpret_cast<float*>(reinterpret_cast<char*>(workspace) + part);
        const int64_t planes = (int64_t)n * cin, hw = (int64_t)in_h * in_w;
        hipLaunchKernelGGL(xscale_kernel, dim3((unsigned)std::min<int64_t>(smc::ceil_div(planes * hw / 4, 256), 4096)),
                           dim3(256), 0, smc::as_stream(stream), x, s_prescale, xs, hw, planes);
        rc = smc::check_launch("smc_conv_gemm_f32 (prescaled input)");
        if (rc != SMC_OK) return rc;
        x = xs;
    }
    GemmParams p{};
    p.x = x; p.n = n; p.cin = cin; p.in_h = in_h; p.in_w = in_w;
    p.y = nsplit > 1 ? workspace : y;
    p.cout = cout; p.y_h = y_h; p.y_w = y_w;
    p.nphases = nphases;
    int64_t max_m = 0;
    for (int i = 0; i < nphases; ++i) {
        const smc_conv_phase& q = phases[i];
        PhaseDev& d = p.ph[i];
        d.ntaps = q.ntaps;
        for (int t = 0; t < 9; ++t) { d.dy[t] = q.tap_dy[t]; d.dx[t] = q.tap_dx[t]; }
        d.in_stride = q.in_stride; d.out_h = q.out_h; d.out_w = q.out_w;
        d.out_oy = q.out_oy; d.out_ox = q.out_ox; d.out_sy = q.out_sy; d.out_sx = q.out_sx;
        d.wk = q.wk;
        d.wx3 = reinterpret_cast<const short*>(q.wk_x3);
        d.wx3_stride = 0;
        const int64_t M = (int64_t)n * q.out_h * q.out_w;
        if (M > max_m) max_m = M;
    }
    SMC_CHECK(max_m < (1LL << 31), "smc_conv_gemm_f32: too many positions");
    p.s = s_in;
    smc_conv_epilogue e{};
    e.mode = SMC_EPI_STORE; e.act = SMC_ACT_LINEAR; e.gain = 1.f; e.clamp = -1.f;
    if (epi) e = *epi;
    p.mode = e.mode; p.d = e.d; p.noise = e.noise; p.noise_nstride = e.noise_nstride;
    p.noise_strength = e.noise_strength; p.bias = e.bias; p.act = e.act; p.alpha = e.alpha; p.gain = e.gain;
    p.clamp = e.clamp; p.u_save = e.u_save;
    p.ext = smc::epi_ext(epi);
    if ((e.mode == SMC_EPI_PRELU || e.mode == SMC_EPI_PRELU_GRAD) && !e.alpha_c) {
        smc::set_error("smc_conv_gemm_f32: PReLU epilogue needs alpha_c");
        return SMC_ERR_INVALID;
    }
    SMC_CHECK(e.mode != SMC_EPI_PRELU_GRAD || e.act_ref, "smc_conv_gemm_f32: PRELU_GRAD needs act_ref");
    SMC_CHECK(e.mode >= SMC_EPI_STORE && e.mode <= SMC_EPI_AFFINE, "smc_conv_gemm_f32: bad epilogue mode %d", e.mode);
    p.nsplit = nsplit;
    p.split_stride = plane_elems;

    hipStream_t st = smc::as_stream(stream);
    auto make_wsample = [&]() -> int {
        g_last_flags |= SMC_ROUTE_WSAMPLE;
        const int64_t part = nsplit > 1 ? ((nsplit * plane_elems * (int64_t)sizeof(float) + 255) / 256) * 256 : 0;
        const int64_t need = part + wsample_floats(n, cin, cout, phases, nphases) * (int64_t)sizeof(float);
        SMC_CHECK(workspace && workspace_bytes >= need, "smc_conv_gemm_f32: workspace %lld < %lld bytes",
                  (long long)workspace_bytes, (long long)need);
        float* wsamp = reinterpret_cast<float*>(reinterpret_cast<char*>(workspace) + part);
        if (x3) {
            short* wp = reinterpret_cast<short*>(wsamp);
            int64_t off = 0;
            for (int i = 0; i < nphases; ++i) {
                const int64_t per = (int64_t)phases[i].ntaps * cin * cout;
                hipLaunchKernelGGL(x3_weights_kernel, dim3((unsigned)std::min<int64_t>(smc::ceil_div(per * n, 256), 4096)),
                                   dim3(256), 0, st, phases[i].wk, s_in, wp + off, phases[i].ntaps, cin, cout, n);
                p.ph[i].wx3 = wp + off;
                p.ph[i].wx3_stride = per * 3;
                off += per * 3 * n;
            }
            return smc::check_launch("smc_conv_gemm_f32 (per-sample split weights)");
        }
        int64_t off = 0;
// ... 110 lines not shown
            { g_last_route = R_LDS_2222_32; hipLaunchKernelGGL((conv_gemm_lds_kernel<2, 2, 2, 2, 32, 2>), grid, dim3(NT), 0, st, p); }
        else if (cfg == 0) SMC_LAUNCH_LDS(2, 2, 2, 2);
        else if (cfg == 3 && cin % 32 == 0 && tag)
            { g_last_route = R_LDS_2211_32_T1; hipLaunchKernelGGL((conv_gemm_lds_kernel<2, 2, 1, 1, 32, 2, 1>), grid, dim3(NT), 0, st, p); }
        else if (cfg == 3) SMC_LAUNCH_LDS(2, 2, 1, 1);
        else if (cfg == 4) SMC_LAUNCH_LDS(1, 4, 1, 1);
        else SMC_LAUNCH_LDS(2, 2, 1, 2);
#undef SMC_LAUNCH_LDS
        rc = smc::check_launch("smc_conv_gemm_f32 (LDS-DMA)");
        if (rc != SMC_OK || nsplit == 1) return rc;
        return smc_modconv_epilogue_f32(workspace, nsplit, plane_elems, y, n, cout, y_h, y_w, &e, stream);
    }
    const bool k32 = cin % 32 == 0 && cin >= 512;
    const bool buf = (int64_t)n * cin * in_h * in_w * 4 < (1LL << 31);
#define SMC_LAUNCH(WO_, WM_, TO_, TM_)                                                                       \
    do {                                                                                                   \
        if (k32 && buf && tag) { g_last_route = R_REG_##WO_##WM_##TO_##TM_##_32_BUF_T1; hipLaunchKernelGGL((conv_gemm_kernel<WO_, WM_, TO_, TM_, 32, true, 1>), grid, dim3(NT), 0, st, p); } \
        else if (buf && tag) { g_last_route = R_REG_##WO_##WM_##TO_##TM_##_16_BUF_T1; hipLaunchKernelGGL((conv_gemm_kernel<WO_, WM_, TO_, TM_, 16, true, 1>), grid, dim3(NT), 0, st, p); } \
        else if (k32 && buf) { g_last_route = R_REG_##WO_##WM_##TO_##TM_##_32_BUF; hipLaunchKernelGGL((conv_gemm_kernel<WO_, WM_, TO_, TM_, 32, true>), grid, dim3(NT), 0, st, p); }   \
        else if (k32) { g_last_route = R_REG_##WO_##WM_##TO_##TM_##_32; hipLaunchKernelGGL((conv_gemm_kernel<WO_, WM_, TO_, TM_, 32, false>), grid, dim3(NT), 0, st, p); }    \
        else if (buf) { g_last_route = R_REG_##WO_##WM_##TO_##TM_##_16_BUF; hipLaunchKernelGGL((conv_gemm_kernel<WO_, WM_, TO_, TM_, 16, true>), grid, dim3(NT), 0, st, p); }     \
        else { g_last_route = R_REG_##WO_##WM_##TO_##TM_##_16; hipLaunchKernelGGL((conv_gemm_kernel<WO_, WM_, TO_, TM_, 16, false>), grid, dim3(NT), 0, st, p); }             \
    } while (0)
    if (cfg == 0) SMC_LAUNCH(2, 2, 2, 2);
    else if (cfg == 4) SMC_LAUNCH(1, 4, 1, 1);
    else if (cfg == 5) SMC_LAUNCH(2, 2, 1, 2);
    else SMC_LAUNCH(2, 2, 1, 1);
#undef SMC_LAUNCH
    rc = smc::check_launch("smc_conv_gemm_f32");
    if (rc != SMC_OK || nsplit == 1) return rc;
    return smc_modconv_epilogue_f32(workspace, nsplit, plane_elems, y, n, cout, y_h, y_w, &e, stream);
}

}

SMC_API int smc_conv_gemm_last_x3(void) { return g_last_x3; }

SMC_API int smc_conv_gemm_last_route(void) { return g_last_route; }

SMC_API int smc_conv_gemm_last_route_flags(void) { return g_last_flags; }

SMC_API int smc_conv_gemm_route_count(void) { return kRouteCount; }

SMC_API const char* smc_conv_gemm_route_name(int route) {
    return route >= 0 && route < kRouteCount ? kRouteNames[route] : nullptr;
}

SMC_API int64_t smc_conv_weights_x3_bytes(int ntaps, int cin, int cout) {
    if (ntaps < 1 || ntaps > 9 || cin < 16 || cin % 16 || cout < 1) return 0;
    return (int64_t)ntaps * cin * cout * 3 * (int64_t)sizeof(short);
}

SMC_API int smc_conv_weights_x3(const float* wk, int ntaps, int cin, int cout, void* wk_x3, void* stream) {
    SMC_CHECK(wk && wk_x3, "smc_conv_weights_x3: null pointer");
    SMC_CHECK(smc_conv_weights_x3_bytes(ntaps, cin, cout) > 0, "smc_conv_weights_x3: bad shape taps=%d cin=%d cout=%d",
              ntaps, cin, cout);
    SMC_CHECK((reinterpret_cast<uintptr_t>(wk_x3) & 15) == 0, "smc_conv_weights_x3: planes must be 16-B aligned");
    const int64_t total = (int64_t)ntaps * cin * cout;
    hipLaunchKernelGGL(x3_weights_kernel, dim3((unsigned)std::min<int64_t>(smc::ceil_div(total, 256), 4096)), dim3(256),
                       0, smc::as_stream(stream), wk, nullptr, reinterpret_cast<short*>(wk_x3), ntaps, cin, cout, 1);
    return smc::check_launch("smc_conv_weights_x3");
}

SMC_API int smc_conv_gemm_f32(const float* x, int n, int cin, int in_h, int in_w, float* y, int cout, int y_h,
                              int y_w, const smc_conv_phase* phases, int nphases, const float* s_in,
                              const smc_conv_epilogue* epi, float* workspace, int64_t workspace_bytes,
                              void* stream) {
    return conv_gemm_impl(x, n, cin, in_h, in_w, y, cout, y_h, y_w, phases, nphases, s_in, epi, workspace,
                          workspace_bytes, stream, 0);
}

namespace smc {
int64_t conv_gemm_aux_workspace_size(int n, int cin, int cout, int y_h, int y_w, const smc_conv_phase* phases,
                                     int nphases) {
    return workspace_size_impl(n, cin, cout, y_h, y_w, phases, nphases, kSplitPerCuAux);
}

int conv_gemm_aux(const float* x, int n, int cin, int in_h, int in_w, float* y, int cout, int y_h, int y_w,
                  const smc_conv_phase* phases, int nphases, const float* s_in, const smc_conv_epilogue* epi,
                  float* workspace, int64_t workspace_bytes, void* stream) {
    return conv_gemm_impl(x, n, cin, in_h, in_w, y, cout, y_h, y_w, phases, nphases, s_in, epi, workspace,
                          workspace_bytes, stream, 1);
}
}

SMC_API int64_t smc_conv_gemm_aux_workspace_size(int n, int cin, int cout, int y_h, int y_w,
                                                 const smc_conv_phase* phases, int nphases) {
    return smc::conv_gemm_aux_workspace_size(n, cin, cout, y_h, y_w, phases, nphases);
}

SMC_API int smc_conv_gemm_aux_f32(const float* x, int n, int cin, int in_h, int in_w, float* y, int cout, int y_h,
                                  int y_w, const smc_conv_phase* phases, int nphases, const float* s_in,
                                  const smc_conv_epilogue* epi, float* workspace, int64_t workspace_bytes,
                                  void* stream) {
    return smc::conv_gemm_aux(x, n, cin, in_h, in_w, y, cout, y_h, y_w, phases, nphases, s_in, epi, workspace,
                              workspace_bytes, stream);
}
```

### stylemc_amd/csrc/modconv_aux.hip

```cpp
#include "common.hpp"

namespace {

struct Epi {
    int mode;
    const float* d;
    const float* noise;
    int64_t noise_nstride;
    const float* noise_strength;
    const float* bias;
    int act;
    float alpha, gain, clamp;
    float* u_save;
    smc::EpiExt ext;
    int grad_from_y;
    float* dd_part;
};

Epi to_epi(const smc_conv_epilogue* e) {
    Epi r{};
    r.mode = SMC_EPI_STORE;
    r.act = SMC_ACT_LINEAR;
    r.gain = 1.f;
    r.clamp = -1.f;
    if (e) {
        r.mode = e->mode; r.d = e->d; r.noise = e->noise; r.noise_nstride = e->noise_nstride;
        r.noise_strength = e->noise_strength; r.bias = e->bias; r.act = e->act; r.alpha = e->alpha;
        r.gain = e->gain; r.clamp = e->clamp; r.u_save = e->u_save; r.grad_from_y = e->grad_from_y;
    }
    r.ext = smc::epi_ext(e);
    return r;
}

__device__ __forceinline__ float wave_sum(float v) {
#pragma unroll
    for (int off = 32; off > 0; off >>= 1) v += __shfl_xor(v, off, 64);
    return v;
}

__device__ __forceinline__ float block_sum256(float v, float* red) {
    v = wave_sum(v);
    const int lane = threadIdx.x & 63, wave = threadIdx.x >> 6;
    __syncthreads();
    if (lane == 0) red[wave] = v;
    __syncthreads();
    return red[0] + red[1] + red[2] + red[3];
}


__global__ __launch_bounds__(256) void epilogue_kernel(const float* src, int nsplit, int64_t split_stride, float* y,
                                                       int c, int h, int w, int64_t total, Epi e) {
    const float nstr = e.noise_strength ? *e.noise_strength : 1.f;
    const int64_t stride = (int64_t)gridDim.x * blockDim.x;
    const int64_t hw = (int64_t)h * w;
    for (int64_t idx = (int64_t)blockIdx.x * blockDim.x + threadIdx.x; idx < total; idx += stride) {
        float v = src[idx];
        for (int s0 = 1; s0 < nsplit; s0 += 8) {
            float t[8];
#pragma unroll
            for (int k = 0; k < 8; ++k) t[k] = src[min(s0 + k, nsplit - 1) * split_stride + idx];
#pragma unroll
            for (int k = 0; k < 8; ++k)
                if (s0 + k < nsplit) v += t[k];
        }
        if (e.mode == SMC_EPI_STORE && !e.ext.residual) {
            y[idx] = v;
            continue;
        }
        const int64_t nc = idx / hw;
        const int64_t pix = idx - nc * hw;
        const int n = (int)(nc / c), o = (int)(nc - (int64_t)n * c);
        const int yy = (int)(pix / w), xx = (int)(pix - (int64_t)yy * w);
        if (e.mode == SMC_EPI_MODACT) {
            if (e.u_save) e.u_save[idx] = v;
            const float nz = e.noise ? e.noise[n * e.noise_nstride + pix] * nstr : 0.f;
            const float dd = (e.d ? e.d[nc] : 1.f) * (e.ext.scale_c ? e.ext.scale_c[o] : 1.f);
            float r = smc::epi_y(v, dd, nz, e.bias ? e.bias[o] : 0.f, e.act, e.alpha, e.gain, e.clamp);
            if (e.ext.residual) r = smc::epi_ext_apply(SMC_EPI_STORE, r, n, o, idx, yy, xx, c, h, w, nullptr, nullptr, e.ext);
            y[idx] = r;
        } else {
            y[idx] = smc::epi_ext_apply(e.mode, v, n, o, idx, yy, xx, c, h, w, e.bias, e.u_save, e.ext);
        }
    }
}

// ... 50 lines not shown
        const int64_t idx = nc * (int64_t)y_h * y_w + pix;
        if (e.mode == SMC_EPI_STORE) {
            y[idx] = u;
            continue;
        }
        if (e.u_save) e.u_save[idx] = u;
        const float nz = e.noise ? e.noise[n * e.noise_nstride + pix] * nstr : 0.f;
        y[idx] = smc::epi_y(u, dv, nz, bv, e.act, e.alpha, e.gain, e.clamp);
    }
}


constexpr int kFH = 32, kFW = 64;
inline dim3 fir_grid_bwd(int64_t planes, int w, int h) {
    return dim3((unsigned)planes, (unsigned)smc::ceil_div(w, kFW), (unsigned)smc::ceil_div(h, kFH));
}
inline dim3 fir_grid_fwd(int64_t planes, int w, int h) {
    return dim3((unsigned)smc::ceil_div(w, kFW), (unsigned)smc::ceil_div(h, kFH), (unsigned)planes);
}

template <int FH, int FW>
__device__ __forceinline__ void fir_block(const float* tile, int stride, int ly0, int lx0, const float (&tp)[FH][FW],
                                          float (&out)[4][2]) {
#pragma unroll
    for (int i = 0; i < 4; ++i) out[i][0] = out[i][1] = 0.f;
#pragma unroll
    for (int r = 0; r < 4 + FH - 1; ++r) {
        float v[2 + FW - 1];
#pragma unroll
        for (int c = 0; c < 2 + FW - 1; ++c) v[c] = tile[(ly0 + r) * stride + lx0 + c];
#pragma unroll
        for (int i = 0; i < 4; ++i) {
            const int jy = r - i;
            if (jy < 0 || jy >= FH) continue;
#pragma unroll
            for (int j = 0; j < 2; ++j)
#pragma unroll
                for (int jx = 0; jx < FW; ++jx) out[i][j] = __fmaf_rn(tp[jy][jx], v[j + jx], out[i][j]);
        }
    }
}

template <int FH, int FW>
__device__ __forceinline__ void fir_block_split(const float* tile, int stride, int ly0, int lx0,
                                                const float (&tp)[FH][FW], float (&out)[4][2]) {
#pragma unroll
    for (int i = 0; i < 4; ++i) out[i][0] = out[i][1] = 0.f;
#pragma unroll
    for (int r = 0; r < 4 + FH - 1; ++r) {
        float v[2][FW];
#pragma unroll
        for (int j = 0; j < 2; ++j)
#pragma unroll
            for (int c = 0; c < FW; ++c) v[j][c] = tile[(ly0 + r) * stride + lx0 + 32 * j + c];
#pragma unroll
        for (int i = 0; i < 4; ++i) {
            const int jy = r - i;
            if (jy < 0 || jy >= FH) continue;
#pragma unroll
            for (int j = 0; j < 2; ++j)
#pragma unroll
                for (int jx = 0; jx < FW; ++jx) out[i][j] = __fmaf_rn(tp[jy][jx], v[j][jx], out[i][j]);
        }
    }
}

template <int FH, int FW>
__device__ __forceinline__ void load_taps(const float* f, int flip, float fgain, float (&tp)[FH][FW]) {
    if (FH == 4 && FW == 4 && !f) {
        constexpr float k[4] = {1.f, 3.f, 3.f, 1.f};
#pragma unroll
        for (int jy = 0; jy < FH; ++jy)
#pragma unroll
            for (int jx = 0; jx < FW; ++jx) tp[jy][jx] = k[jy] * k[jx] * (1.f / 64.f) * fgain;
        return;
    }
#pragma unroll
    for (int jy = 0; jy < FH; ++jy)
#pragma unroll
        for (int jx = 0; jx < FW; ++jx)
            tp[jy][jx] = f[(flip ? jy : FH - 1 - jy) * FW + (flip ? jx : FW - 1 - jx)] * fgain;
}

template <int FH, int FW>
__device__ __forceinline__ void std_taps(float (&tp)[FH][FW]) {
    constexpr float k[4] = {1.f, 3.f, 3.f, 1.f};
#pragma unroll
    for (int jy = 0; jy < FH; ++jy)
#pragma unroll
        for (int jx = 0; jx < FW; ++jx) tp[jy][jx] = k[jy] * k[jx] * 0.0625f;
}

template <int FH, int FW>
__global__ __launch_bounds__(256) void blur_act_fast(const float* t, int nsplit, int64_t split_stride, float* y, int c,
                                                     int t_h, int t_w, int tp_w, int y_h, int y_w, const float* f,
                                                     int padx0, int pady0, float fgain, int flip, Epi e) {
    constexpr int ROWS = kFH + FH - 1, COLS = kFW + FW - 1, STRIDE = COLS + 1;
    __shared__ float tile[ROWS * STRIDE];
    const int tid = threadIdx.x, tx = tid & 31, ty = tid >> 5;
    const int ox0 = blockIdx.x * kFW, oy0 = blockIdx.y * kFH;
    const int64_t nc = blockIdx.z;
    const int n = (int)(nc / c), o = (int)(nc - (int64_t)n * c);
    float tp[FH][FW];
    load_taps<FH, FW>(f, flip, fgain, tp);
    const int iy0 = oy0 - pady0, ix0 = ox0 - padx0;
    const float* tpl = t + nc * (int64_t)t_h * tp_w;
    constexpr int NL = (ROWS * COLS + 255) / 256;
    float v[NL];
    int off[NL];
#pragma unroll
    for (int l = 0; l < NL; ++l) {
        const int i = tid + 256 * l;
        const int r = i / COLS, cc = i - r * COLS;
        const int iy = iy0 + r, ix = ix0 + cc;
        const bool ok = i < ROWS * COLS && iy >= 0 && iy < t_h && ix >= 0 && ix < t_w;
        off[l] = ok ? iy * tp_w + ix : -1;
        const float a = tpl[ok ? off[l] : 0];
        v[l] = ok ? a : 0.f;
    }
    for (int s = 1; s < nsplit; ++s) {
        const float* sp = tpl + s * split_stride;
#pragma unroll
        for (int l = 0; l < NL; ++l) {
            const float a = sp[off[l] >= 0 ? off[l] : 0];
            v[l] += off[l] >= 0 ? a : 0.f;
        }
    }
#pragma unroll
    for (int l = 0; l < NL; ++l) {
        const int i = tid + 256 * l;
        const int r = i / COLS, cc = i - r * COLS;
        if (i < ROWS * COLS) tile[r * STRIDE + cc] = v[l];
    }
    __syncthreads();
    float out[4][2];
    fir_block<FH, FW>(tile, STRIDE, 4 * ty, 2 * tx, tp, out);
    const float nstr = e.noise_strength ? *e.noise_strength : 1.f;
    const float dv = e.d ? e.d[nc] : 1.f;
    const float bv = e.bias ? e.bias[o] : 0.f;
    const int64_t plane = nc * (int64_t)y_h * y_w;
    const int ox = ox0 + 2 * tx;
    if (ox >= y_w) return;
    const bool pair = (y_w & 1) == 0 && ((e.noise_nstride & 1) == 0) &&
                      (((uintptr_t)y | (uintptr_t)e.u_save | (uintptr_t)e.noise) & 7) == 0;
#pragma unroll
    for (int i = 0; i < 4; ++i) {
        const int oy = oy0 + 4 * ty + i;
        if (oy >= y_h) continue;
        const int64_t pix = (int64_t)oy * y_w + ox;
        if (pair) {
            const float2 u2 = make_float2(out[i][0], out[i][1]);
            if (e.mode == SMC_EPI_STORE) {
                *reinterpret_cast<float2*>(y + plane + pix) = u2;
                continue;
            }
            if (e.u_save) *reinterpret_cast<float2*>(e.u_save + plane + pix) = u2;
            float2 nz = make_float2(0.f, 0.f);
            if (e.noise) {
                nz = *reinterpret_cast<const float2*>(e.noise + n * e.noise_nstride + pix);
                nz.x *= nstr;
                nz.y *= nstr;
            }
            *reinterpret_cast<float2*>(y + plane + pix) =
                make_float2(smc::epi_y(u2.x, dv, nz.x, bv, e.act, e.alpha, e.gain, e.clamp),
                            smc::epi_y(u2.y, dv, nz.y, bv, e.act, e.alpha, e.gain, e.clamp));
            continue;
        }
#pragma unroll
        for (int j = 0; j < 2; ++j) {
            if (ox + j >= y_w) continue;
            const float u = out[i][j];
            if (e.mode == SMC_EPI_STORE) {
                y[plane + pix + j] = u;
                continue;
            }
            if (e.u_save) e.u_save[plane + pix + j] = u;
            const float nz = e.noise ? e.noise[n * e.noise_nstride + pix + j] * nstr : 0.f;
            y[plane + pix + j] = smc::epi_y(u, dv, nz, bv, e.act, e.alpha, e.gain, e.clamp);
        }
    }
}

#ifndef SMC_BLUR_TPB
#define SMC_BLUR_TPB 4
#endif
#ifndef SMC_BLUR_NT
#define SMC_BLUR_NT 1
#endif
#ifndef SMC_BLUR_WGS
#define SMC_BLUR_WGS 4
#endif
#ifndef SMC_BLUR_STDF
#define SMC_BLUR_STDF 1
#endif
#ifndef SMC_BLUR_PIPE
#define SMC_BLUR_PIPE 1
#endif
template <bool NT>
__device__ __forceinline__ void st_f2(float* p, float2 v) {
    if (NT) {
        typedef float f32x2 __attribute__((ext_vector_type(2)));
        __builtin_nontemporal_store(f32x2{v.x, v.y}, reinterpret_cast<f32x2*>(p));
    } else {
        *reinterpret_cast<float2*>(p) = v;
    }
}

template <int FH, int FW, int TPB, bool NT, bool STDF = false>
__global__ __launch_bounds__(256, STDF ? SMC_BLUR_WGS : 1) void blur_act_v4(const float* t, int nsplit, int64_t split_stride, float* y, int c,
                                                   int t_h, int t_w, int tp_w, int y_h, int y_w, const float* f,
                                                   int padx0, int pady0, float fgain, int flip, Epi e) {
    constexpr int ROWS = kFH + FH - 1, COLS = kFW + FW - 1, STRIDE = COLS + 1;
    constexpr int G4 = (kFW + 8) / 4 + 1;
    constexpr int NL = (ROWS * G4 + 255) / 256;
    __shared__ float tile[ROWS * STRIDE];
    const int tid = threadIdx.x, tx = tid & 31, ty = tid >> 5;
    const int ox0 = blockIdx.x * kFW;
    const int64_t nc = blockIdx.z;
    const int n = (int)(nc / c), o = (int)(nc - (int64_t)n * c);
    float tp[FH][FW];
    if constexpr (STDF) std_taps<FH, FW>(tp);
    else load_taps<FH, FW>(f, flip, fgain, tp);
    const float nstr = e.noise_strength ? *e.noise_strength : 1.f;
    const float dv = e.d ? e.d[nc] : 1.f;
    const float bv = e.bias ? e.bias[o] : 0.f;
    const int ix0 = ox0 - padx0;
    const int64_t pbase = nc * (int64_t)t_h * tp_w;
    const int pmis = (int)(pbase & 3);
    const float* tpl = t + (pbase - pmis);
    float4 v[NL];
    int off[NL];
    int gx[NL];
    auto load_tile = [&](int tb) {
        const int iy0 = (blockIdx.y * TPB + tb) * kFH - pady0;
#pragma unroll
        for (int l = 0; l < NL; ++l) {
            const int i = tid + 256 * l;
            const int r = i / G4, q = i - r * G4;
            const int iy = iy0 + r;
            const int row = pmis + iy * tp_w;
            const int g0 = ((row + ox0 - 4) & ~3) + 4 * q;
            gx[l] = g0 - row;
            const bool ok = i < ROWS * G4 && iy >= 0 && iy < t_h && gx[l] + 3 >= 0 && gx[l] < t_w;
            off[l] = ok ? g0 : -1;
            v[l] = *reinterpret_cast<const float4*>(tpl + (ok ? g0 : 0));
        }
    };
    if (blockIdx.y * TPB * kFH < y_h) load_tile(0);
    for (int tb = 0; tb < TPB; ++tb) {
        const int oy0 = (blockIdx.y * TPB + tb) * kFH;
        if (oy0 >= y_h) break;
        if (tb > 0) __syncthreads();
        if (!SMC_BLUR_PIPE && tb > 0) load_tile(tb);
        for (int s = 1; s < nsplit; ++s) {
            const float* sp = tpl + s * split_stride;
#pragma unroll
            for (int l = 0; l < NL; ++l) {
                const float4 a = *reinterpret_cast<const float4*>(sp + (off[l] >= 0 ? off[l] : 0));
                v[l].x += a.x; v[l].y += a.y; v[l].z += a.z; v[l].w += a.w;
            }
        }
#pragma unroll
        for (int l = 0; l < NL; ++l) {
            const int i = tid + 256 * l;
            if (i >= ROWS * G4) continue;
            const int r = i / G4;
            const float a[4] = {v[l].x, v[l].y, v[l].z, v[l].w};
#pragma unroll
            for (int k = 0; k < 4; ++k) {
                const int ix = gx[l] + k;
                const int cc = ix - ix0;
                if (cc >= 0 && cc < COLS) tile[r * STRIDE + cc] = (off[l] >= 0 && ix >= 0 && ix < t_w) ? a[k] : 0.f;
            }
        }
        __syncthreads();
        if (SMC_BLUR_PIPE && tb + 1 < TPB && oy0 + kFH < y_h) load_tile(tb + 1);
        float out[4][2];
        fir_block<FH, FW>(tile, STRIDE, 4 * ty, 2 * tx, tp, out);
        const int64_t plane = nc * (int64_t)y_h * y_w;
        const int ox = ox0 + 2 * tx;
        if (ox >= y_w) continue;
        float2 nz[4];
#pragma unroll
        for (int i = 0; i < 4; ++i) {
            const int oy = min(oy0 + 4 * ty + i, y_h - 1);
            nz[i] = make_float2(0.f, 0.f);
            if (e.mode != SMC_EPI_STORE && e.noise) {
                nz[i] = *reinterpret_cast<const float2*>(e.noise + n * e.noise_nstride + (int64_t)oy * y_w + ox);
                nz[i].x *= nstr;
                nz[i].y *= nstr;
            }
        }
        const bool lrelu_clamp = e.act == SMC_ACT_LRELU && e.alpha >= 0.f && e.alpha <= 1.f && e.clamp >= 0.f;
#pragma unroll
        for (int i = 0; i < 4; ++i) {
            const int oy = oy0 + 4 * ty + i;
            if (oy >= y_h) continue;
            const int64_t pix = (int64_t)oy * y_w + ox;
            const float2 u2 = make_float2(out[i][0], out[i][1]);
            if (e.mode == SMC_EPI_STORE) {
                st_f2<NT>(y + plane + pix, u2);
                continue;
            }
            if (e.u_save) st_f2<NT>(e.u_save + plane + pix, u2);
            float2 q;
            if (lrelu_clamp) {
                const float zx = __fmaf_rn(u2.x, dv, nz[i].x) + bv, zy = __fmaf_rn(u2.y, dv, nz[i].y) + bv;
                q.x = smc::lrelu_gain_clamp(zx, e.alpha, e.gain, e.clamp);
                q.y = smc::lrelu_gain_clamp(zy, e.alpha, e.gain, e.clamp);
            } else {
                q = make_float2(smc::epi_y(u2.x, dv, nz[i].x, bv, e.act, e.alpha, e.gain, e.clamp),
                                smc::epi_y(u2.y, dv, nz[i].y, bv, e.act, e.alpha, e.gain, e.clamp));
            }
            st_f2<NT>(y + plane + pix, q);
        }
    }
}

template <int FH, int FW, bool V2 = false, bool FROMY = false>
__global__ __launch_bounds__(256) void blur_act_bwd_fast(const float* g, const float* u, float* dt, float* dd, int c,
                                                         int u_h, int u_w, int t_h, int t_w, int tp_w, const float* f,
                                                         int padx0,
                                                         int pady0, float fgain, int flip, Epi e) {
    constexpr int ROWS = kFH + FH - 1, COLS = kFW + FW - 1, STRIDE = COLS + 1;
    __shared__ __attribute__((aligned(16))) float tile[ROWS * STRIDE];
    __shared__ float red[4];
    const int tid = threadIdx.x, tx = tid & 31, ty = tid >> 5;
    const int ox0 = blockIdx.y * kFW, oy0 = blockIdx.z * kFH;
    const int64_t nc = blockIdx.x;
    const int n = (int)(nc / c), o = (int)(nc - (int64_t)n * c);
    float tp[FH][FW];
    load_taps<FH, FW>(f, flip, fgain, tp);
    const float nstr = e.noise_strength ? *e.noise_strength : 1.f;
    const float dv = e.d ? e.d[nc] : 1.f;
    const float bv = e.bias ? e.bias[o] : 0.f;
    const int iy0 = oy0 - pady0, ix0 = ox0 - padx0;
    const int64_t uplane = nc * (int64_t)u_h * u_w;
    float part = 0.f;
    const float* up = u + uplane;
    const float* gp = g + uplane;
    const float* np_ = !FROMY && e.noise ? e.noise + n * e.noise_nstride : nullptr;
    auto elem = [&](float uu, float gg, float nn, int iy, int ix) {
        if constexpr (FROMY) return smc::act_grad_y(e.act, gg, uu, e.alpha, e.gain, e.clamp) * dv;
        const float yv = smc::epi_y(uu, dv, nn * nstr, bv, e.act, e.alpha, e.gain, e.clamp);
        const float dz = smc::act_grad_y(e.act, gg, yv, e.alpha, e.gain, e.clamp);
        if (iy >= oy0 && iy < oy0 + kFH && ix >= ox0 && ix < ox0 + kFW) part += dz * uu;
        return dz * dv;
    };
    if constexpr (V2) {
        constexpr int C2 = (COLS + 1) / 2;
        constexpr int NL = (ROWS * C2 + 255) / 256;
        float2 uv[NL], gv[NL], nv[NL];
#pragma unroll
        for (int l = 0; l < NL; ++l) {
            const int i = tid + 256 * l;
            const int r = i / C2, c2 = i - r * C2;
            const int iy = iy0 + r, ix = ix0 + 2 * c2;
            const bool ok = i < ROWS * C2 && iy >= 0 && iy < u_h && ix >= 0 && ix < u_w;
            const int pix = ok ? iy * u_w + ix : 0;
            uv[l] = *reinterpret_cast<const float2*>(up + pix);
            gv[l] = *reinterpret_cast<const float2*>(gp + pix);
            nv[l] = np_ ? *reinterpret_cast<const float2*>(np_ + pix) : make_float2(0.f, 0.f);
        }
#pragma unroll
        for (int l = 0; l < NL; ++l) {
            const int i = tid + 256 * l;
            const int r = i / C2, c2 = i - r * C2;
            const int iy = iy0 + r, ix = ix0 + 2 * c2;
            const bool ok = i < ROWS * C2 && iy >= 0 && iy < u_h && ix >= 0 && ix < u_w;
            float2 v = make_float2(0.f, 0.f);
            if (ok) {
                v.x = elem(uv[l].x, gv[l].x, nv[l].x, iy, ix);
                v.y = elem(uv[l].y, gv[l].y, nv[l].y, iy, ix + 1);
            }
            if (i < ROWS * C2) *reinterpret_cast<float2*>(&tile[r * STRIDE + 2 * c2]) = v;
        }
    } else {
        constexpr int NL = (ROWS * COLS + 255) / 256;
        float uv[NL], gv[NL], nv[NL];
#pragma unroll
        for (int l = 0; l < NL; ++l) {
            const int i = tid + 256 * l;
            const int r = i / COLS, cc = i - r * COLS;
            const int iy = iy0 + r, ix = ix0 + cc;
            const bool ok = i < ROWS * COLS && iy >= 0 && iy < u_h && ix >= 0 && ix < u_w;
            const int pix = ok ? iy * u_w + ix : 0;
            uv[l] = up[pix];
            gv[l] = gp[pix];
            nv[l] = np_ ? np_[pix] : 0.f;
        }
#pragma unroll
        for (int l = 0; l < NL; ++l) {
            const int i = tid + 256 * l;
            const int r = i / COLS, cc = i - r * COLS;
            const int iy = iy0 + r, ix = ix0 + cc;
            const bool ok = i < ROWS * COLS && iy >= 0 && iy < u_h && ix >= 0 && ix < u_w;
// ... 525 lines not shown
```

### stylemc_amd/modconv.py

```python
import ctypes

import torch

from . import _hip


def _phase(taps, in_stride, out_h, out_w, out_oy, out_ox, out_sy, out_sx, wk, wk_x3=None):
    ph = _hip.ConvPhase()
    ph.ntaps = len(taps)
    for t, (dy, dx) in enumerate(taps):
        ph.tap_dy[t] = dy
        ph.tap_dx[t] = dx
    ph.in_stride = in_stride
    ph.out_h, ph.out_w, ph.out_oy, ph.out_ox, ph.out_sy, ph.out_sx = out_h, out_w, out_oy, out_ox, out_sy, out_sx
    ph.wk = wk.data_ptr()
    ph.wk_x3 = wk_x3.data_ptr() if wk_x3 is not None else None
    return ph


X3 = True


def x3_planes(wk, cin, cout, enabled=None):
    if not ((X3 if enabled is None else enabled) and wk.is_cuda):
# ... 90 lines not shown
                th, tw = 2 * h + 1, 2 * w + 1
                ph = [_phase(t, 1, (th - py + 1) // 2, (tw - px + 1) // 2, py, px, 2, 2, wk, wx)
                      for (py, px, t, wk), wx in zip(self.phases, self.x3_phases)]
                self._cache[key] = ((_hip.ConvPhase * 4)(*ph), 4, th, tw)
        return self._cache[key]

    def bwd_phases(self, h, w):
        key = ("b", h, w)
        if key not in self._cache:
            stride = 1 if self.up == 1 else 2
            self._cache[key] = ((_hip.ConvPhase * 1)(_phase(self.bwd_taps, stride, h, w, 0, 0, 1, 1, self.wk_bwd,
                                                            self.x3_bwd)), 1)
        return self._cache[key]


def conv_flops(n, cin, cout, h_out, w_out, taps):
    return 2.0 * n * cin * cout * h_out * w_out * taps


def gemm(x, y, phases, nph, cin, cout, s=None, epi=None, alg_flops=0.0, alg_bytes=0):
    n, _, ih, iw = x.shape
    yh, yw = y.shape[2], y.shape[3]
    lib = _hip.load()
    ws_bytes = lib.smc_conv_gemm_workspace_size(n, cin, cout, yh, yw, phases, nph)
    ws = torch.empty(max(ws_bytes // 4, 1), device=x.device, dtype=torch.float32) if ws_bytes > 0 else None
    tm = _hip.timer()
    tok = tm.wrap(alg_flops, alg_bytes, kind="direct") if tm is not None else None
    _hip.call("smc_conv_gemm_f32", x.data_ptr(), n, cin, ih, iw, y.data_ptr(), cout, yh, yw, phases, nph,
              _hip.ptr(s), ctypes.byref(epi) if epi is not None else None, _hip.ptr(ws), ws_bytes, _hip.stream())
    if tok is not None:
        tm.finish(tok, kind="direct_x3" if lib.smc_conv_gemm_last_x3() else "direct")


WINOGRAD = True


def wino_ok(n, cin, cout, h, w):
    return WINOGRAD and bool(_hip.load().smc_conv3x3_wino_supported(n, cin, cout, h, w))


WINO_SPLIT = True


def wino(x, y, uw, cin, cout, s=None, epi=None, alg_flops=0.0, alg_bytes=0):
    n, _, h, w = x.shape
    ws_bytes = _hip.load().smc_conv3x3_wino_workspace_size(n, cin, cout, h, w) if WINO_SPLIT else 0
    ws = torch.empty(ws_bytes // 4, device=x.device, dtype=torch.float32) if ws_bytes > 0 else None
    tm = _hip.timer()
    tok = tm.wrap(alg_flops, alg_bytes, kind="wino", equiv_flops=alg_flops * 36 / 16) if tm is not None else None
    _hip.call("smc_conv3x3_wino_ws_f32", x.data_ptr(), n, cin, h, w, y.data_ptr(), cout, uw.data_ptr(), _hip.ptr(s),
              ctypes.byref(epi) if epi is not None else None, _hip.ptr(ws), ws_bytes, _hip.stream())
    if tok is not None:
        tm.finish(tok)


def wino4_ok(n, cin, cout, h, w):
    return WINOGRAD and bool(_hip.load().smc_conv3x3_wino4_supported(n, cin, cout, h, w))


WINO4 = True
WINO4_MIN_CIN = 64


def wino4_pick(n, cin, cout, h, w):
    return WINO4 and cin >= WINO4_MIN_CIN and wino4_ok(n, cin, cout, h, w)


def wino4(x, y, uw, cin, cout, s=None, epi=None, alg_flops=0.0, alg_bytes=0):
    n, _, h, w = x.shape
    tm = _hip.timer()
    tok = tm.wrap(alg_flops, alg_bytes, kind="wino4", equiv_flops=alg_flops * 4) if tm is not None else None
    _hip.call("smc_conv3x3_wino4_f32", x.data_ptr(), n, cin, h, w, y.data_ptr(), cout, uw.data_ptr(), _hip.ptr(s),
              ctypes.byref(epi) if epi is not None else None, _hip.stream())
    if tok is not None:
        tm.finish(tok)


def wino4_flops(n, cin, cout, h, w):
    return 2.0 * n * cin * cout * (h // 4) * (w // 4) * 36


def wino_flops(n, cin, cout, h, w):
    return 2.0 * n * cin * cout * (h // 2) * (w // 2) * 16


def _epilogue(mode, d=None, noise=None, noise_nstride=0, strength=None, bias=None, act="linear", alpha=0.0,
              gain=1.0, clamp=-1.0, u_save=None):
    e = _hip.ConvEpilogue()
    e.mode = mode
    e.d = _hip.ptr(d)
    e.noise = _hip.ptr(noise)
    e.noise_nstride = noise_nstride
    e.noise_strength = _hip.ptr(strength)
    e.bias = _hip.ptr(bias)
    e.act = _hip.ACT_CODES[act]
    e.alpha, e.gain, e.clamp = float(alpha), float(gain), float(clamp)
    e.u_save = _hip.ptr(u_save)
    return e


class LayerSpec:

    def __init__(self, weight, bias, up, resample_filter, demodulate=True, act="lrelu", alpha=0.2, resolution=None):
        self.packed = PackedConv(weight, up)
        self.bias = bias.detach().float().contiguous() if bias is not None else None
        self.up = up
        self.filter = resample_filter.detach().float().contiguous() if resample_filter is not None else None
        k = torch.tensor([1.0, 3.0, 3.0, 1.0])
        self.std_filter = self.filter is not None and tuple(self.filter.shape) == (4, 4) and torch.equal(
            self.filter.detach().cpu(), torch.outer(k, k) / 64.0)
        self.demodulate = demodulate
        self.act = act
        self.alpha = alpha
        P = self.packed
        if weight.is_cuda:
            direct = [True, True]
            if resolution is not None and up == 1 and P.k == 3:
                for flip, (ci, co) in enumerate([(P.cin, P.cout), (P.cout, P.cin)]):
                    if wino4_pick(1, ci, co, resolution, resolution):
                        P.wino4_weights(flip)
                        direct[flip] = False
                    elif wino_ok(1, ci, co, resolution, resolution):
                        P.wino_weights(flip)
                        direct[flip] = False
            if resolution is not None:
                if direct[0]:
                    P.x3_fwd if up == 1 else P.x3_phases
                if direct[1]:
                    P.x3_bwd
            torch.cuda.current_stream(weight.device).synchronize()


def _noise_args(noise):
    if noise is None:
        return None, 0
    noise = noise.contiguous()
    if noise.ndim == 2:
        return noise, 0
    assert noise.ndim == 4 and noise.shape[1] == 1, "noise must be [H, W] or [N, 1, H, W]"
    return noise, noise.shape[2] * noise.shape[3]


def _modconv_fwd(ctx, x, styles, spec, noise, strength, gain, clamp, need_dx, need_ds):
    x = x.contiguous()
    styles = styles.contiguous()
    P = spec.packed
    n, cin, h, w = x.shape
    assert cin == P.cin and styles.shape == (n, cin), (x.shape, styles.shape, P.cin)
    r_h, r_w = h * spec.up, w * spec.up
    d = None
    if spec.demodulate:
        d = torch.empty(n, P.cout, device=x.device, dtype=torch.float32)
        _hip.call("smc_modconv_demod_f32", _hip.ptr(styles), _hip.ptr(P.wsq), _hip.ptr(d), n, cin, P.cout, 1e-8,
                  _hip.stream())
    save = need_dx or need_ds
    from_y = save and not need_ds
    y = torch.empty(n, P.cout, r_h, r_w, device=x.device, dtype=torch.float32)
    u = torch.empty_like(y) if save and not from_y else None
    nz, nstride = _noise_args(noise)
    epi = _epilogue(_hip.EPI_MODACT, d, nz, nstride, strength, spec.bias, spec.act, spec.alpha, gain, clamp, u)
    phases, nph, th, tw = P.fwd_phases(h, w)
    wbytes = 4 * P.k * P.k * cin * P.cout
    if spec.up == 1 and P.k == 3 and wino4_pick(n, cin, P.cout, h, w):
        wino4(x, y, P.wino4_weights(0), cin, P.cout, s=styles, epi=epi, alg_flops=wino4_flops(n, cin, P.cout, h, w),
              alg_bytes=4 * x.numel() + 4 * y.numel() * (2 if u is not None else 1) + 36 * 4 * cin * P.cout)
    elif spec.up == 1 and P.k == 3 and wino_ok(n, cin, P.cout, h, w):
        wino(x, y, P.wino_weights(0), cin, P.cout, s=styles, epi=epi, alg_flops=wino_flops(n, cin, P.cout, h, w),
             alg_bytes=4 * x.numel() + 4 * y.numel() * (2 if u is not None else 1) + 16 * 4 * cin * P.cout)
    elif spec.up == 1:
        gemm(x, y, phases, nph, cin, P.cout, s=styles, epi=epi,
             alg_flops=conv_flops(n, cin, P.cout, r_h, r_w, P.k * P.k),
             alg_bytes=4 * x.numel() + 4 * y.numel() * (2 if u is not None else 1) + wbytes)
    else:
        t = torch.empty(n, P.cout, th, tw, device=x.device, dtype=torch.float32)
        gemm(x, t, phases, nph, cin, P.cout, s=styles, epi=_epilogue(_hip.EPI_STORE),
             alg_flops=conv_flops(n, cin, P.cout, h, w, 9), alg_bytes=4 * x.numel() + 4 * t.numel() + wbytes)
        f = None if spec.std_filter else spec.filter.to(x.device)
        _hip.call("smc_modconv_blur_act_f32", t.data_ptr(), 1, 0, y.data_ptr(), n, P.cout, th, tw, 0, r_h, r_w,
                  _hip.ptr(f), 4 if f is None else f.shape[0], 4 if f is None else f.shape[1], 1, 1, 4.0, 0,
                  ctypes.byref(epi), _hip.stream())
    ctx.spec, ctx.gain, ctx.clamp = spec, gain, clamp
    ctx.noise, ctx.nstride, ctx.strength = nz, nstride, strength
    ctx.from_y = from_y
    return y, (x, styles, d, y if from_y else u)


def _modconv_epi_bwd(ctx, d):
    spec = ctx.spec
    epi = _epilogue(_hip.EPI_MODACT, d, ctx.noise, ctx.nstride, ctx.strength, spec.bias, spec.act, spec.alpha,
                    ctx.gain, ctx.clamp)
    epi.grad_from_y = 1 if ctx.from_y else 0
    return epi


def _dd_workspace(dd, nbytes, device):
    if dd is None or nbytes <= 0:
        return None
    return torch.empty(nbytes // 4, device=device, dtype=torch.float32)


def _nbytes(t):
    return 0 if t is None else 4 * t.numel()


def _modconv_bwd(ctx, saved, gy, need_dx, need_ds, g=None):
    x, styles, d, u = saved
    spec = ctx.spec
    P = spec.packed
    n, cin, h, w = x.shape
    dd = torch.zeros(n, P.cout, device=x.device, dtype=torch.float32) if (need_ds and spec.demodulate) else None
    assert dd is None or not ctx.from_y
    if g is None:
        gy = gy.contiguous()
        epi = _modconv_epi_bwd(ctx, d)
        if spec.up == 1:
            g = torch.empty_like(u)
            ws = _dd_workspace(dd, _hip.load().smc_modconv_act_bwd_workspace_size(n, P.cout, u.shape[2], u.shape[3]),
                               x.device)
            _hip.call("smc_modconv_act_bwd_f32", gy.data_ptr(), u.data_ptr(), g.data_ptr(), _hip.ptr(dd), n, P.cout,
                      u.shape[2], u.shape[3], ctypes.byref(epi), _hip.ptr(ws), _nbytes(ws), _hip.stream())
        else:
            f = None if spec.std_filter else spec.filter.to(x.device)
            fh, fw = (4, 4) if f is None else f.shape
            th, tw = 2 * h + 1, 2 * w + 1
            pitch = (tw + 3) // 4 * 4
            g = torch.empty(n, P.cout, th, pitch, device=x.device, dtype=torch.float32)
            ws = _dd_workspace(dd, _hip.load().smc_modconv_blur_act_bwd_workspace_size(n, P.cout, u.shape[2],
                                                                                        u.shape[3], th, tw), x.device)
            _hip.call("smc_modconv_blur_act_bwd_f32", gy.data_ptr(), u.data_ptr(), g.data_ptr(), _hip.ptr(dd), n,
                      P.cout, u.shape[2], u.shape[3], th, tw, pitch, _hip.ptr(f), fh, fw, fw - 2, fh - 2, 4.0, 1,
                      ctypes.byref(epi), _hip.ptr(ws), _nbytes(ws), _hip.stream())
    else:
        assert spec.up == 1 and dd is None
    dx = torch.empty_like(x) if need_dx else None
    dxs = torch.empty_like(x) if need_ds else None
    if need_dx:
        ebw = _epilogue(_hip.EPI_MODACT, d=styles, act="linear", u_save=dxs)
        out = dx
    else:
        ebw = _epilogue(_hip.EPI_STORE)
        out = dxs
    g_bytes = 4 * g.numel() if spec.up == 1 else 4 * n * P.cout * (2 * h + 1) * (2 * w + 1)
    out_bytes = 4 * out.numel() * (2 if (need_dx and need_ds) else 1)
    if spec.up == 1 and P.k == 3 and wino4_pick(n, P.cout, cin, h, w):
        wino4(g, out, P.wino4_weights(1), P.cout, cin, epi=ebw, alg_flops=wino4_flops(n, P.cout, cin, h, w),
              alg_bytes=g_bytes + out_bytes + 36 * 4 * cin * P.cout)
    elif spec.up == 1 and P.k == 3 and wino_ok(n, P.cout, cin, h, w):
        wino(g, out, P.wino_weights(1), P.cout, cin, epi=ebw, alg_flops=wino_flops(n, P.cout, cin, h, w),
             alg_bytes=g_bytes + out_bytes + 16 * 4 * cin * P.cout)
    else:
        phases, nph = P.bwd_phases(h, w)
        gemm(g, out, phases, nph, P.cout, cin, epi=ebw, alg_flops=conv_flops(n, P.cout, cin, h, w, P.k * P.k),
             alg_bytes=g_bytes + out_bytes + 4 * P.k * P.k * cin * P.cout)
    ds = None
    if need_ds:
# ... 131 lines not shown
```

Before: 473.3 images/s.

## Fuse stride-2 transposed modconv with FIR blur and activation epilogue

Adds a fused up2 modulated-conv kernel that runs the x3 split-bf16 transposed conv and then applies the standard 4x4 blur, demodulation, noise, bias and activation in the same launch. It replaces the separate gemm-to-temporary plus blur_act pass. The kernel loop is factored into a shared header so both paths reuse it. The fused path is only taken for cout=32 with the standard filter when the planner picks no split-K, which removes a full-resolution temporary write and read in the upsampling layers. In exchange it adds register and LDS pressure and a halo-exchange design inside one kernel.

```diff
diff --git a/include/stylemc_hip.h b/include/stylemc_hip.h
--- a/include/stylemc_hip.h
+++ b/include/stylemc_hip.h
@@ -127,6 +127,15 @@
 int smc_modconv_blur_act_f32(const float* t, int nsplit, int64_t split_stride, float* y, int n, int c, int t_h,
                              int t_w, int t_pitch, int y_h, int y_w, const float* f, int fh, int fw, int padx0,
                              int pady0, float fgain, int flip, const smc_conv_epilogue* epi, void* stream);
+
+int smc_modconv_up2_supported(int n, int cin, int cout, int h, int w);
+int smc_modconv_up2_plan_ok(int n, int cin, int cout, int h, int w);
+int smc_modconv_up2_f32(const float* x, int n, int cin, int h, int w, float* y, int cout,
+                        const smc_conv_phase* phases, int nphases, const float* s_in, const float* f, int fh, int fw,
+                        float fgain, const smc_conv_epilogue* epi, float* workspace, int64_t workspace_bytes,
+                        void* stream);
+int smc_modconv_up2_last_route(void);
+const char* smc_modconv_up2_route_name(int route);
 
 int smc_modconv_blur_act_bwd_f32(const float* g, const float* u, float* dt, float* dd, int n, int c, int u_h, int u_w,
                                  int t_h, int t_w, int t_pitch, const float* f, int fh, int fw, int padx0, int pady0,
diff --git a/stylemc_amd/_hip.py b/stylemc_amd/_hip.py
--- a/stylemc_amd/_hip.py
+++ b/stylemc_amd/_hip.py
@@ -80,6 +80,12 @@
     "smc_modconv_epilogue_f32": (c_int, [P, c_int, c_int64, P, c_int, c_int, c_int, c_int, P, P]),
     "smc_modconv_blur_act_f32": (c_int, [P, c_int, c_int64, P, c_int, c_int, c_int, c_int, c_int, c_int, c_int, P,
                                          c_int, c_int, c_int, c_int, c_float, c_int, P, P]),
+    "smc_modconv_up2_supported": (c_int, [c_int] * 5),
+    "smc_modconv_up2_plan_ok": (c_int, [c_int] * 5),
+    "smc_modconv_up2_f32": (c_int, [P, c_int, c_int, c_int, c_int, P, c_int, P, c_int, P, P, c_int, c_int, c_float, P,
+                                    P, c_int64, P]),
+    "smc_modconv_up2_last_route": (c_int, []),
+    "smc_modconv_up2_route_name": (c_char_p, [c_int]),
     "smc_modconv_blur_act_bwd_f32": (c_int, [P, P, P, P, c_int, c_int, c_int, c_int, c_int, c_int, c_int, P, c_int,
                                              c_int, c_int, c_int, c_float, c_int, P, P, c_int64, P]),
     "smc_modconv_blur_act_bwd_workspace_size": (c_int64, [c_int] * 6),
diff --git a/stylemc_amd/csrc/conv_gemm.hip b/stylemc_amd/csrc/conv_gemm.hip
--- a/stylemc_amd/csrc/conv_gemm.hip
+++ b/stylemc_amd/csrc/conv_gemm.hip
@@ -3,48 +3,13 @@
 #include <type_traits>
 
 #include "common.hpp"
+#include "convt_x3.hpp"
 
 namespace {
 
+using namespace smc::cg;
+
 constexpr int BK = 16;
-constexpr int NT = 256;
-typedef float f32x16 __attribute__((ext_vector_type(16)));
-
-struct PhaseDev {
-    int ntaps;
-    int dy[9];
-    int dx[9];
-    int in_stride;
-    int out_h, out_w, out_oy, out_ox, out_sy, out_sx;
-    const float* wk;
-    int64_t wstride;
-    const short* wx3;
-    int64_t wx3_stride;
-};
-
-struct GemmParams {
-    const float* x;
-    int n, cin, in_h, in_w;
-    float* y;
-    int cout, y_h, y_w;
-    PhaseDev ph[4];
-    int nphases;
-    const float* s;
-    int mode;
-    const float* d;
-    const float* noise;
-    int64_t noise_nstride;
-    const float* noise_strength;
-    const float* bias;
-    int act;
-    float alpha, gain, clamp;
-    float* u_save;
-    smc::EpiExt ext;
-    int nsplit;
-    int64_t split_stride;
-    int per_sample;
-    int ntn;
-};
 
 template <int WO, int WM, int TO, int TM>
 __device__ __forceinline__ void gemm_epilogue(const GemmParams& p, const PhaseDev& ph, const f32x16 (&acc)[TO][TM],
@@ -361,11 +326,6 @@
     static constexpr int bytes = ww * 4;
 };
 
-template <int N>
-__device__ __forceinline__ void wait_vmcnt() {
-    asm volatile("s_waitcnt vmcnt(%0)" ::"n"(N) : "memory");
-}
-
 template <int WO, int WM, int TO, int TM, int BKT, int NST, int TAG = 0>
 __global__ __launch_bounds__(NT, 2) void conv_gemm_lds_kernel(GemmParams p) {
     static_assert(WO * WM == 4, "4 waves");
@@ -531,41 +491,6 @@
 }
 
 
-typedef short bf16x8 __attribute__((ext_vector_type(8)));
-
-__device__ __forceinline__ void x3_split8(const float (&x)[8], bf16x8 (&t)[3]) {
-    unsigned u0[8], u1[8], u2[8];
-#pragma unroll
-    for (int j = 0; j < 8; ++j) {
-        const unsigned u = __float_as_uint(x[j]);
-        const float r1 = x[j] - __uint_as_float(u & 0xffff0000u);
-        const unsigned v = __float_as_uint(r1);
-        const float r2 = r1 - __uint_as_float(v & 0xffff0000u);
-        u0[j] = u;
-        u1[j] = v;
-        u2[j] = __float_as_uint(r2);
-    }
-    typedef unsigned u32x4 __attribute__((ext_vector_type(4)));
-    u32x4 w0, w1, w2;
-#pragma unroll
-    for (int j = 0; j < 4; ++j) {
-        w0[j] = __builtin_amdgcn_perm(u0[2 * j + 1], u0[2 * j], 0x07060302u);
-        w1[j] = __builtin_amdgcn_perm(u1[2 * j + 1], u1[2 * j], 0x07060302u);
-        w2[j] = __builtin_amdgcn_perm(u2[2 * j + 1], u2[2 * j], 0x07060302u);
-    }
-    t[0] = __builtin_bit_cast(bf16x8, w0);
-    t[1] = __builtin_bit_cast(bf16x8, w1);
-    t[2] = __builtin_bit_cast(bf16x8, w2);
-}
-
-__device__ __forceinline__ f32x16 x3_mma(const bf16x8 (&a)[3], const bf16x8 (&b)[3], f32x16 acc) {
-    acc = __builtin_amdgcn_mfma_f32_32x32x16_bf16(a[2], b[0], acc, 0, 0, 0);
-    acc = __builtin_amdgcn_mfma_f32_32x32x16_bf16(a[1], b[1], acc, 0, 0, 0);
-    acc = __builtin_amdgcn_mfma_f32_32x32x16_bf16(a[0], b[2], acc, 0, 0, 0);
-    acc = __builtin_amdgcn_mfma_f32_32x32x16_bf16(a[1], b[0], acc, 0, 0, 0);
-    acc = __builtin_amdgcn_mfma_f32_32x32x16_bf16(a[0], b[1], acc, 0, 0, 0);
-    return __builtin_amdgcn_mfma_f32_32x32x16_bf16(a[0], b[0], acc, 0, 0, 0);
-}
 
 __global__ __launch_bounds__(256) void x3_weights_kernel(const float* wk, const float* s_in, short* out, int ntaps,
                                                          int cin, int cout, int n) {
@@ -1034,8 +959,6 @@
 template <> struct ShiftPhases<2> { static constexpr int n = 2; static constexpr int p[4] = {0, 2, 0, 0}; };
 template <> struct ShiftPhases<3> { static constexpr int n = 1; static constexpr int p[4] = {0, 0, 0, 0}; };
 
-__host__ __device__ constexpr int shift_nph(int s) { return s == 0 ? 4 : (s == 3 ? 1 : 2); }
-
 template <int S, int TO, int TM, int BKT, int BO, int BM>
 __device__ __forceinline__ void convt_mma(const float* Ws, const float* Xs, int wo, int wm, int kh, int l32,
                                           f32x16 (&acc)[4][TO][TM]) {
@@ -1222,14 +1145,6 @@
     }
 }
 
-struct ConvTTaps {
-    int tap[4][4];
-};
-
-template <int S>
-__host__ __device__ constexpr int shift_phase(int j) {
-    return S == 0 ? j : (S == 1 ? (j ? 1 : 0) : (S == 2 ? (j ? 2 : 0) : 0));
-}
 
 template <int S, int TO, int TM, int BKT, int BO, int BM>
 __device__ __forceinline__ void convt_lds_mma(const float* Ws, const float* Xs, int wo, int wm, int kh, int l32,
@@ -1411,19 +1326,9 @@
 
 template <int WO, int WM, int TO, int TM>
 __global__ __launch_bounds__(NT, 2) void convt_x3_kernel(GemmParams p, ConvTTaps tt) {
-    static_assert(WO * WM == 4, "4 waves");
-    constexpr int BKT = 16;
-    constexpr int BO = WO * TO * 32;
-    constexpr int BM = WM * TM * 32;
-    constexpr int NCH = BM / 64;
-    static_assert(NCH >= 1 && NCH <= 4 && 4 % NCH == 0, "BM in {64,128,256}");
-    constexpr int RSTEP = 4 / NCH;
-    constexpr int XI = BKT * NCH / 4;
-    constexpr int PB = 6 * BO * 16;
-    static_assert(PB % 1024 == 0, "phase planes split into whole 1-KB DMAs");
-    constexpr int XB = BKT * BM * 4;
-    constexpr int STAGE = XB + 4 * PB;
-    __shared__ __attribute__((aligned(16))) char smem[2 * STAGE];
+    typedef ConvTX3<WO, WM, TO, TM> C;
+    constexpr int BKT = C::BKT, BO = C::BO, BM = C::BM, NCH = C::NCH;
+    __shared__ __attribute__((aligned(16))) char smem[C::RING];
 
     const int tid = threadIdx.x;
     const int lane = tid & 63;
@@ -1455,7 +1360,7 @@
     const int c_end = (int)((int64_t)cpk * (split + 1) / p.nsplit);
     const int ks_begin = 4 * c_begin, ks_end = 4 * c_end;
 
-    const int cw = wave % NCH, r0 = wave / NCH;
+    const int cw = wave % NCH;
     const int m = m0 + cw * 64 + lane;
     const bool mvalid = m < M;
     int nn = 0, a = 0, b = 0;
@@ -1465,95 +1370,11 @@
         a = rem / gw;
         b = rem - a * gw;
     }
-    const int in_hw = p.in_h * p.in_w;
-    const __amdgpu_buffer_rsrc_t xrsrc = __builtin_amdgcn_make_buffer_rsrc(
-        (void*)p.x, (short)0, (int)((int64_t)p.n * p.cin * in_hw * 4), 0x00020000);
-    const int xvbase = nn * p.cin * in_hw * 4;
     const int wn = m0 / hw_g;
-    const int c16n = p.cin / 16;
-
-    auto issue = [&](int ks, int slot) {
-        const int c = ks >> 2, sh = ks & 3;
-        const int ci0 = c * BKT;
-        const int iy = a - (sh & 1), ix = b - (sh >> 1);
-        const bool ok = mvalid && iy >= 0 && iy < p.in_h && ix >= 0 && ix < p.in_w;
-        const int voff = ok ? xvbase + (iy * p.in_w + ix) * 4 : 0x7ffffff0;
-        char* st = smem + slot * STAGE;
-        float* xs = reinterpret_cast<float*>(st);
-#pragma unroll
-        for (int j = 0; j < XI; ++j) {
-            const int row = r0 + RSTEP * j;
-            __builtin_amdgcn_raw_ptr_buffer_load_lds(
-                xrsrc, (__attribute__((address_space(3))) void*)(xs + row * BM + cw * 64), 4, voff,
-                (ci0 + row) * in_hw * 4, 0, 0);
-        }
-        const int nph = shift_nph(sh);
-        for (int j = wave; j < nph * (PB / 1024); j += 4) {
-            const int pj = j / (PB / 1024);
-            const int phase = sh == 0 ? pj : (sh == 1 ? (pj ? 1 : 0) : (sh == 2 ? (pj ? 2 : 0) : 0));
-            const int L = (j - pj * (PB / 1024)) * 64 + lane;
-            const int run = L / BO, o = L - run * BO;
-            const PhaseDev& q = p.ph[phase];
-            const short* src = q.wx3 + (q.wx3_stride ? (int64_t)wn * q.wx3_stride : 0) +
-                               ((((int64_t)tt.tap[sh][phase] * c16n + ci0 / 16) * 6 + run) * p.cout + o0 + o) * 8;
-            __builtin_amdgcn_global_load_lds((const void*)src, (__attribute__((address_space(3))) void*)(st + XB + j * 1024),
-                                             16, 0, 0);
-        }
-    };
 
     f32x16 acc[4][TO][TM];
-#pragma unroll
-    for (int ph = 0; ph < 4; ++ph)
-#pragma unroll
-        for (int i = 0; i < TO; ++i)
-#pragma unroll
-            for (int j = 0; j < TM; ++j)
-#pragma unroll
-                for (int r = 0; r < 16; ++r) acc[ph][i][j][r] = 0.f;
-
+    convt_x3_loop<WO, WM, TO, TM>(p, tt, smem, mvalid, nn, a, b, wn, o0, ks_begin, ks_end, acc);
     const int kh = lane >> 5, l32 = lane & 31;
-    if (ks_begin < ks_end) issue(ks_begin, 0);
-    auto step = [&](auto S_, int ks) {
-        constexpr int S = decltype(S_)::value;
-        constexpr int NP = shift_nph(S);
-        wait_vmcnt<0>();
-        __builtin_amdgcn_s_barrier();
-        asm volatile("" ::: "memory");
-        const char* st = smem + (S & 1) * STAGE;
-        const float* xcol = reinterpret_cast<const float*>(st) + wm * TM * 32 + l32;
-        bf16x8 bt[TM][3];
-#pragma unroll
-        for (int j = 0; j < TM; ++j) {
-            float xv[8];
-#pragma unroll
-            for (int e = 0; e < 8; ++e) xv[e] = xcol[(8 * kh + e) * BM + j * 32];
-            x3_split8(xv, bt[j]);
-        }
-        __builtin_amdgcn_sched_barrier(0);
-        if (ks + 1 < ks_end) issue(ks + 1, (S + 1) & 1);
-#pragma unroll
-        for (int pj = 0; pj < NP; ++pj) {
-            const short* Wp = reinterpret_cast<const short*>(st + XB + pj * PB);
-            bf16x8 at[TO][3];
-#pragma unroll
-            for (int i = 0; i < TO; ++i)
-#pragma unroll
-                for (int s = 0; s < 3; ++s)
-                    at[i][s] = *reinterpret_cast<const bf16x8*>(Wp + (((s * 2 + kh) * BO) + wo * TO * 32 + i * 32 + l32) * 8);
-#pragma unroll
-            for (int i = 0; i < TO; ++i)
-#pragma unroll
-                for (int j = 0; j < TM; ++j)
-                    acc[shift_phase<S>(pj)][i][j] = x3_mma(at[i], bt[j], acc[shift_phase<S>(pj)][i][j]);
-        }
-        asm volatile("s_waitcnt lgkmcnt(0)" ::: "memory");
-    };
-    for (int ks = ks_begin; ks < ks_end; ks += 4) {
-        step(std::integral_constant<int, 0>{}, ks);
-        step(std::integral_constant<int, 1>{}, ks + 1);
-        step(std::integral_constant<int, 2>{}, ks + 2);
-        step(std::integral_constant<int, 3>{}, ks + 3);
-    }
 
     float* dst = p.nsplit > 1 ? p.y + (int64_t)split * p.split_stride : p.y;
     const int64_t plane = (int64_t)p.y_h * p.y_w;
@@ -1644,17 +1465,23 @@
     int bo, bm, id;
 };
 
+bool convt_lds_shape_ok(int n, int cin, int cout, int in_h, int in_w) {
+    return cin % 16 == 0 && cout % 32 == 0 && cout <= 64 && (int64_t)n * cin * in_h * in_w * 4 < (1LL << 31);
+}
+ConvTL convt_lds_tile(int cout) { return cout % 64 == 0 ? ConvTL{64, 128, 1} : ConvTL{32, 128, 0}; }
+bool convt_lds_per_sample(int in_h, int in_w, const ConvTL& c) { return ((int64_t)(in_h + 1) * (in_w + 1)) % c.bm != 0; }
+
 bool convt_lds_plan(int n, int cin, int cout, int in_h, int in_w, int y_h, int y_w, const smc_conv_phase* ph, int nph,
                     const smc_conv_epilogue* epi, ConvTTaps* tt, ConvTL* cfg) {
     ConvTParams q{};
     if (!convt_structure(cin, cout, in_h, in_w, y_h, y_w, ph, nph, epi, &q)) return false;
-    if (cin % 16 != 0 || cout % 32 != 0 || cout > 64 || (int64_t)n * cin * in_h * in_w * 4 >= (1LL << 31)) return false;
+    if (!convt_lds_shape_ok(n, cin, cout, in_h, in_w)) return false;
     if (tt) {
         for (int sh = 0; sh < 4; ++sh)
             for (int k = 0; k < 4; ++k)
                 tt->tap[sh][k] = q.w[sh][k] ? (int)((q.w[sh][k] - ph[k].wk) / ((int64_t)cin * cout)) : -1;
     }
-    if (cfg) *cfg = cout % 64 == 0 ? ConvTL{64, 128, 1} : ConvTL{32, 128, 0};
+    if (cfg) *cfg = convt_lds_tile(cout);
     return true;
 }
 
@@ -1760,6 +1587,8 @@
     return !has_s || scaled_ok || (int64_t)taps_all * cout <= (int64_t)in_h * in_w;
 }
 
+bool prescale_shape(int64_t hw, int taps_all, int cout) { return hw <= (int64_t)taps_all * cout; }
+
 int64_t prescale_floats(int n, int cin, int cout, const smc_conv_phase* ph, int nph) {
     int64_t hw = 0;
     int taps_all = 0;
@@ -1768,7 +1597,7 @@
         hw = std::max<int64_t>(hw, (int64_t)ph[i].out_h * ph[i].out_w);
         taps_all += ph[i].ntaps;
     }
-    return hw <= (int64_t)taps_all * cout ? (((int64_t)n * cin * hw + 63) / 64) * 64 : 0;
+    return prescale_shape(hw, taps_all, cout) ? (((int64_t)n * cin * hw + 63) / 64) * 64 : 0;
 }
 
 int validate(const float* x, int n, int cin, int in_h, int in_w, float* y, int cout, int y_h, int y_w,
@@ -1947,7 +1776,7 @@
         cfg = 6;
         c = Cfg{256, 128};
     }
-    const bool t_per_sample = convt_lds && s_in && ((int64_t)(in_h + 1) * (in_w + 1)) % tl.bm != 0;
+    const bool t_per_sample = convt_lds && s_in && convt_lds_per_sample(in_h, in_w, tl);
     const int nsplit = convt_lds ? plan_split_convt_lds(n, cin, cout, in_h, in_w, tl, t_per_sample)
                                  : fused_t ? plan_split_convt(n, cin, cout, in_h, in_w)
                                            : plan_split(n, cin, cout, phases, nphases, c, tag ? kSplitPerCuAux : 2);
@@ -2224,6 +2053,57 @@
     return conv_gemm_impl(x, n, cin, in_h, in_w, y, cout, y_h, y_w, phases, nphases, s_in, epi, workspace,
                           workspace_bytes, stream, 1);
 }
+
+bool convt_up2_shape_ok(int n, int cin, int cout, int h, int w) {
+    return n >= 1 && h >= 1 && w >= 1 && cin >= 16 && cout >= 32 && convt_lds_shape_ok(n, cin, cout, h, w);
+}
+
+bool convt_up2_plan_ok(int n, int cin, int cout, int h, int w) {
+    const ConvTL tl = convt_lds_tile(cout);
+    if (plan_split_convt_lds(n, cin, cout, h, w, tl, convt_lds_per_sample(h, w, tl)) != 1) return false;
+    return !prescale_shape((int64_t)(h + 1) * (w + 1), 9, cout);
+}
+
+int convt_up2_prepare(const float* x, int n, int cin, int h, int w, float* y, int cout, const smc_conv_phase* phases,
+                      int nphases, const float* s_in, float* workspace, int64_t workspace_bytes, void* stream,
+                      GemmParams* pp, ConvTTaps* tt) {
+    const int th = 2 * h + 1, tw = 2 * w + 1;
+    int rc = validate(x, n, cin, h, w, y, cout, th, tw, phases, nphases);
+    if (rc != SMC_OK) return rc;
+    ConvTL tl{};
+    if (!convt_up2_shape_ok(n, cin, cout, h, w) || !phases_x3(phases, nphases) ||
+        !convt_lds_plan(n, cin, cout, h, w, th, tw, phases, nphases, nullptr, tt, &tl)) {
+        set_error("smc_modconv_up2_f32: needs the 4-phase stride-2 transposed 3x3 conv with split-bf16 planes, "
+                  "cin %% 16 == 0, cout 32 or 64 and an input below 2 GiB");
+        return SMC_ERR_UNSUPPORTED;
+    }
+    GemmParams& p = *pp;
+    p.x = x; p.n = n; p.cin = cin; p.in_h = h; p.in_w = w;
+    p.cout = cout; p.y_h = th; p.y_w = tw;
+    p.nphases = nphases;
+    for (int i = 0; i < nphases; ++i) {
+        p.ph[i].ntaps = phases[i].ntaps;
+        p.ph[i].wk = phases[i].wk;
+        p.ph[i].wx3 = reinterpret_cast<const short*>(phases[i].wk_x3);
+        p.ph[i].wx3_stride = 0;
+    }
+    if (!s_in) return SMC_OK;
+    const int64_t need = wsample_floats(n, cin, cout, phases, nphases) * (int64_t)sizeof(float);
+    SMC_CHECK(workspace && workspace_bytes >= need && (reinterpret_cast<uintptr_t>(workspace) & 15) == 0,
+              "smc_modconv_up2_f32: workspace %lld < %lld bytes (or not 16-B aligned)", (long long)workspace_bytes,
+              (long long)need);
+    short* wp = reinterpret_cast<short*>(workspace);
+    int64_t off = 0;
+    for (int i = 0; i < nphases; ++i) {
+        const int64_t per = (int64_t)phases[i].ntaps * cin * cout;
+        hipLaunchKernelGGL(x3_weights_kernel, dim3((unsigned)std::min<int64_t>(ceil_div(per * n, 256), 4096)), dim3(256),
+                           0, as_stream(stream), phases[i].wk, s_in, wp + off, phases[i].ntaps, cin, cout, n);
+        p.ph[i].wx3 = wp + off;
+        p.ph[i].wx3_stride = per * 3;
+        off += per * 3 * n;
+    }
+    return check_launch("smc_modconv_up2_f32 (per-sample split weights)");
+}
 }
 
 SMC_API int64_t smc_conv_gemm_aux_workspace_size(int n, int cin, int cout, int y_h, int y_w,
diff --git a/stylemc_amd/csrc/convt_fir.hip b/stylemc_amd/csrc/convt_fir.hip
--- /dev/null
+++ b/stylemc_amd/csrc/convt_fir.hip
@@ -0,0 +1,208 @@
+#include "convt_x3.hpp"
+#include "fir_epi.hpp"
+
+namespace {
+
+using namespace smc::cg;
+
+constexpr int kPB = 18, kTC = 2 * kPB, kYC = kTC - 4;
+
+template <int TM>
+struct FirTile {
+    static constexpr int PA = 7 * TM;
+    static constexpr int TR = 2 * PA;
+    static constexpr int YR = TR - 4;
+    static constexpr int CH = 32 / TM;
+    static constexpr int RT = YR / TM;
+    static constexpr int CHS = TM == 1 ? 544 : 1056;
+    static constexpr int BYTES = CH * CHS * 4;
+    static_assert(PA * kPB <= 128 * TM && CHS >= TR * kTC && CHS % 64 == 32 && kYC == 32 && YR % TM == 0 &&
+                      CH * 8 * TM == NT, "tile geometry");
+};
+
+template <bool V4>
+__device__ __forceinline__ void st_row(float* p, const float (&v)[4], bool hi) {
+    if (V4) {
+        typedef float f32x4 __attribute__((ext_vector_type(4)));
+        __builtin_nontemporal_store(f32x4{v[0], v[1], v[2], v[3]}, reinterpret_cast<f32x4*>(p));
+    } else {
+        smc::st_f2<true>(p, make_float2(v[0], v[1]));
+        if (hi) smc::st_f2<true>(p + 2, make_float2(v[2], v[3]));
+    }
+}
+
+template <int TO, int TM, bool V4>
+__global__ __launch_bounds__(NT, 2) void convt_x3_fir_kernel(GemmParams p, ConvTTaps tt, int nty, int ntx) {
+    typedef ConvTX3<1, 4, TO, TM> C;
+    typedef FirTile<TM> F;
+    constexpr int LDSB = C::RING > F::BYTES ? C::RING : F::BYTES;
+    __shared__ __attribute__((aligned(16))) char smem[LDSB];
+
+    const int tid = threadIdx.x;
+    const int lane = tid & 63;
+    const int wave = __builtin_amdgcn_readfirstlane(tid >> 6);
+    const int nwg = gridDim.x, orig = blockIdx.x;
+    const int xcd = orig % 8, q8 = nwg / 8, r8 = nwg % 8;
+    const int wgid = (xcd < r8 ? xcd * (q8 + 1) : r8 * (q8 + 1) + (xcd - r8) * q8) + orig / 8;
+    const int tps = nty * ntx;
+    const int nb = wgid / tps;
+    const int trem = wgid - nb * tps;
+    const int ti = trem / ntx, tj = trem - ti * ntx;
+    const int a0 = ti * (F::YR / 2) - 1, b0 = tj * (kYC / 2) - 1;
+
+    const int ms = (wave % C::NCH) * 64 + lane;
+    const int spa = ms / kPB;
+    f32x16 acc[4][TO][TM];
+    convt_x3_loop<1, 4, TO, TM>(p, tt, smem, ms < F::PA * kPB, nb, a0 + spa, b0 + (ms - spa * kPB), nb, 0, 0,
+                                4 * (p.cin / C::BKT), acc);
+
+    const int kh = lane >> 5, l32 = lane & 31;
+    float* T = reinterpret_cast<float*>(smem);
+    float* tw[TM];
+    bool tv[TM];
+#pragma unroll
+    for (int j = 0; j < TM; ++j) {
+        const int me = (wave * TM + j) * 32 + l32;
+        const int epa = me / kPB, epb = me - epa * kPB;
+        tv[j] = me < F::PA * kPB;
+        tw[j] = T + (2 * epa) * kTC + 2 * epb;
+    }
+
+    const int q = tid & 7, chl = (tid >> 3) % F::CH, rg = (tid >> 3) / F::CH;
+    const int ox = tj * kYC + 4 * q, oy0 = ti * F::YR + rg * F::RT;
+    const bool lo = ox < p.y_w, hi = ox + 2 < p.y_w;
+    const float* tr = T + chl * F::CHS + (rg * F::RT) * kTC + 4 * q;
+    const float nstr = p.noise_strength ? *p.noise_strength : 1.f;
+    const bool lrelu_clamp = smc::modact_lrelu_clamp(p.act, p.alpha, p.clamp);
+    float tp[4][4];
+    smc::std_taps<4, 4>(tp);
+    const int64_t plane = (int64_t)p.y_h * p.y_w;
+
+#pragma unroll
+    for (int pass = 0; pass < TO * TM; ++pass) {
+        const int i = pass / TM, cp = pass % TM;
+        __syncthreads();
+#pragma unroll
+        for (int j = 0; j < TM; ++j) {
+            if (!tv[j]) continue;
+#pragma unroll
+            for (int r = 0; r < 16; ++r) {
+                if (r / (16 / TM) != cp) continue;
+                float* t0 = tw[j] + ((r & 3) + 8 * ((r >> 2) % (4 / TM)) + 4 * kh) * F::CHS;
+                *reinterpret_cast<float2*>(t0) = make_float2(acc[0][i][j][r], acc[1][i][j][r]);
+                *reinterpret_cast<float2*>(t0 + kTC) = make_float2(acc[2][i][j][r], acc[3][i][j][r]);
+            }
+        }
+        __syncthreads();
+        const int o = i * 32 + cp * F::CH + chl;
+        const int64_t nc = (int64_t)nb * p.cout + o;
+        const float dv = p.d ? p.d[nc] : 1.f;
+        const float bv = p.bias ? p.bias[o] : 0.f;
+        float nz[F::RT][4];
+#pragma unroll
+        for (int yi = 0; yi < F::RT; ++yi) {
+            nz[yi][0] = nz[yi][1] = nz[yi][2] = nz[yi][3] = 0.f;
+            if (p.noise && lo) {
+                const float* np = p.noise + nb * p.noise_nstride + (int64_t)min(oy0 + yi, p.y_h - 1) * p.y_w + ox;
+                const float2 n0 = *reinterpret_cast<const float2*>(np);
+                nz[yi][0] = n0.x * nstr;
+                nz[yi][1] = n0.y * nstr;
+                if (hi) {
+                    const float2 n1 = *reinterpret_cast<const float2*>(np + 2);
+                    nz[yi][2] = n1.x * nstr;
+                    nz[yi][3] = n1.y * nstr;
+                }
+            }
+        }
+        float out[F::RT][4];
+#pragma unroll
+        for (int yi = 0; yi < F::RT; ++yi) out[yi][0] = out[yi][1] = out[yi][2] = out[yi][3] = 0.f;
+#pragma unroll
+        for (int r = 1; r < F::RT + 4; ++r) {
+            const float4 v0 = *reinterpret_cast<const float4*>(tr + r * kTC);
+            const float4 v1 = *reinterpret_cast<const float4*>(tr + r * kTC + 4);
+            const float v[8] = {v0.x, v0.y, v0.z, v0.w, v1.x, v1.y, v1.z, v1.w};
+#pragma unroll
+            for (int yi = 0; yi < F::RT; ++yi) {
+                const int jy = r - 1 - yi;
+                if (jy < 0 || jy >= 4) continue;
+#pragma unroll
+                for (int j = 0; j < 4; ++j)
+#pragma unroll
+                    for (int jx = 0; jx < 4; ++jx) out[yi][j] = __fmaf_rn(tp[jy][jx], v[1 + j + jx], out[yi][j]);
+            }
+            if (r < 4) continue;
+            const int yi = r - 4;
+            const int oy = oy0 + yi;
+            if (!lo || oy >= p.y_h) continue;
+            const int64_t pix = nc * plane + (int64_t)oy * p.y_w + ox;
+            if (p.u_save) st_row<V4>(p.u_save + pix, out[yi], hi);
+            const float2 qa = smc::modact2(make_float2(out[yi][0], out[yi][1]), dv, make_float2(nz[yi][0], nz[yi][1]),
+                                           bv, lrelu_clamp, p.act, p.alpha, p.gain, p.clamp);
+            const float2 qb = smc::modact2(make_float2(out[yi][2], out[yi][3]), dv, make_float2(nz[yi][2], nz[yi][3]),
+                                           bv, lrelu_clamp, p.act, p.alpha, p.gain, p.clamp);
+            const float yv[4] = {qa.x, qa.y, qb.x, qb.y};
+            st_row<V4>(p.y + pix, yv, hi);
+        }
+    }
+}
+
+enum Up2Route { U_NONE = 0, U_FIR_12, U_FIR_12_V4, U_FIR_21, U_FIR_21_V4, kUp2Routes };
+constexpr const char* kUp2Names[] = {"none", "convt_x3_fir_kernel<1,2,false>", "convt_x3_fir_kernel<1,2,true>",
+                                     "convt_x3_fir_kernel<2,1,false>", "convt_x3_fir_kernel<2,1,true>"};
+static_assert(sizeof(kUp2Names) / sizeof(kUp2Names[0]) == kUp2Routes, "one name per route");
+thread_local int g_up2_route = U_NONE;
+
+}
+
+SMC_API int smc_modconv_up2_supported(int n, int cin, int cout, int h, int w) {
+    return smc::convt_up2_shape_ok(n, cin, cout, h, w) ? 1 : 0;
+}
+
+SMC_API int smc_modconv_up2_plan_ok(int n, int cin, int cout, int h, int w) {
+    return smc::convt_up2_shape_ok(n, cin, cout, h, w) && smc::convt_up2_plan_ok(n, cin, cout, h, w) ? 1 : 0;
+}
+
+SMC_API int smc_modconv_up2_last_route(void) { return g_up2_route; }
+
+SMC_API const char* smc_modconv_up2_route_name(int route) {
+    return route >= 0 && route < kUp2Routes ? kUp2Names[route] : nullptr;
+}
+
+SMC_API int smc_modconv_up2_f32(const float* x, int n, int cin, int h, int w, float* y, int cout,
+                                const smc_conv_phase* phases, int nphases, const float* s_in, const float* f, int fh,
+                                int fw, float fgain, const smc_conv_epilogue* epi, float* workspace,
+                                int64_t workspace_bytes, void* stream) {
+    g_up2_route = U_NONE;
+    SMC_CHECK(x && y && phases && epi && n >= 1 && h >= 1 && w >= 1, "smc_modconv_up2_f32: bad args");
+    if (f || fh != 4 || fw != 4 || fgain != 4.f) {
+        smc::set_error("smc_modconv_up2_f32: only the built-in [1,3,3,1] filter (f = NULL, 4x4) at gain 4");
+        return SMC_ERR_UNSUPPORTED;
+    }
+    SMC_CHECK(epi->mode == SMC_EPI_MODACT && !epi->residual && !epi->scale_c && !epi->grad_from_y,
+              "smc_modconv_up2_f32: the MODACT epilogue only");
+    const uintptr_t al = (uintptr_t)y | (uintptr_t)epi->u_save | (uintptr_t)epi->noise;
+    SMC_CHECK(al % 8 == 0 && epi->noise_nstride % 2 == 0, "smc_modconv_up2_f32: y / u_save / noise need 8-B alignment");
+    GemmParams p{};
+    ConvTTaps tt{};
+    int rc = smc::convt_up2_prepare(x, n, cin, h, w, y, cout, phases, nphases, s_in, workspace, workspace_bytes, stream, &p,
+                                    &tt);
+    if (rc != SMC_OK) return rc;
+    p.y = y; p.y_h = 2 * h; p.y_w = 2 * w;
+    p.mode = epi->mode; p.d = epi->d; p.noise = epi->noise; p.noise_nstride = epi->noise_nstride;
+    p.noise_strength = epi->noise_strength; p.bias = epi->bias; p.act = epi->act; p.alpha = epi->alpha;
+    p.gain = epi->gain; p.clamp = epi->clamp; p.u_save = epi->u_save;
+    p.nsplit = 1;
+    const int yr = cout == 32 ? FirTile<2>::YR : FirTile<1>::YR;
+    const int nty = (int)smc::ceil_div(p.y_h, yr), ntx = (int)smc::ceil_div(p.y_w, kYC);
+    const int64_t nwg = (int64_t)n * nty * ntx;
+    SMC_CHECK(nwg < (1LL << 31), "smc_modconv_up2_f32: too many tiles");
+    const bool v4 = p.y_w % 4 == 0 && ((uintptr_t)y | (uintptr_t)epi->u_save) % 16 == 0;
+    const dim3 g((unsigned)nwg);
+    hipStream_t st = smc::as_stream(stream);
+    if (cout == 32 && v4) { g_up2_route = U_FIR_12_V4; hipLaunchKernelGGL((convt_x3_fir_kernel<1, 2, true>), g, dim3(NT), 0, st, p, tt, nty, ntx); }
+    else if (cout == 32) { g_up2_route = U_FIR_12; hipLaunchKernelGGL((convt_x3_fir_kernel<1, 2, false>), g, dim3(NT), 0, st, p, tt, nty, ntx); }
+    else if (v4) { g_up2_route = U_FIR_21_V4; hipLaunchKernelGGL((convt_x3_fir_kernel<2, 1, true>), g, dim3(NT), 0, st, p, tt, nty, ntx); }
+    else { g_up2_route = U_FIR_21; hipLaunchKernelGGL((convt_x3_fir_kernel<2, 1, false>), g, dim3(NT), 0, st, p, tt, nty, ntx); }
+    return smc::check_launch("smc_modconv_up2_f32");
+}
diff --git a/stylemc_amd/csrc/convt_x3.hpp b/stylemc_amd/csrc/convt_x3.hpp
--- /dev/null
+++ b/stylemc_amd/csrc/convt_x3.hpp
@@ -0,0 +1,226 @@
+#pragma once
+#include <type_traits>
+
+#include "common.hpp"
+
+namespace smc {
+namespace cg {
+
+constexpr int NT = 256;
+typedef float f32x16 __attribute__((ext_vector_type(16)));
+
+struct PhaseDev {
+    int ntaps;
+    int dy[9];
+    int dx[9];
+    int in_stride;
+    int out_h, out_w, out_oy, out_ox, out_sy, out_sx;
+    const float* wk;
+    int64_t wstride;
+    const short* wx3;
+    int64_t wx3_stride;
+};
+
+struct GemmParams {
+    const float* x;
+    int n, cin, in_h, in_w;
+    float* y;
+    int cout, y_h, y_w;
+    PhaseDev ph[4];
+    int nphases;
+    const float* s;
+    int mode;
+    const float* d;
+    const float* noise;
+    int64_t noise_nstride;
+    const float* noise_strength;
+    const float* bias;
+    int act;
+    float alpha, gain, clamp;
+    float* u_save;
+    smc::EpiExt ext;
+    int nsplit;
+    int64_t split_stride;
+    int per_sample;
+    int ntn;
+};
+
+template <int N>
+__device__ __forceinline__ void wait_vmcnt() {
+    asm volatile("s_waitcnt vmcnt(%0)" ::"n"(N) : "memory");
+}
+
+typedef short bf16x8 __attribute__((ext_vector_type(8)));
+
+__device__ __forceinline__ void x3_split8(const float (&x)[8], bf16x8 (&t)[3]) {
+    unsigned u0[8], u1[8], u2[8];
+#pragma unroll
+    for (int j = 0; j < 8; ++j) {
+        const unsigned u = __float_as_uint(x[j]);
+        const float r1 = x[j] - __uint_as_float(u & 0xffff0000u);
+        const unsigned v = __float_as_uint(r1);
+        const float r2 = r1 - __uint_as_float(v & 0xffff0000u);
+        u0[j] = u;
+        u1[j] = v;
+        u2[j] = __float_as_uint(r2);
+    }
+    typedef unsigned u32x4 __attribute__((ext_vector_type(4)));
+    u32x4 w0, w1, w2;
+#pragma unroll
+    for (int j = 0; j < 4; ++j) {
+        w0[j] = __builtin_amdgcn_perm(u0[2 * j + 1], u0[2 * j], 0x07060302u);
+        w1[j] = __builtin_amdgcn_perm(u1[2 * j + 1], u1[2 * j], 0x07060302u);
+        w2[j] = __builtin_amdgcn_perm(u2[2 * j + 1], u2[2 * j], 0x07060302u);
+    }
+    t[0] = __builtin_bit_cast(bf16x8, w0);
+    t[1] = __builtin_bit_cast(bf16x8, w1);
+    t[2] = __builtin_bit_cast(bf16x8, w2);
+}
+
+__device__ __forceinline__ f32x16 x3_mma(const bf16x8 (&a)[3], const bf16x8 (&b)[3], f32x16 acc) {
+    acc = __builtin_amdgcn_mfma_f32_32x32x16_bf16(a[2], b[0], acc, 0, 0, 0);
+    acc = __builtin_amdgcn_mfma_f32_32x32x16_bf16(a[1], b[1], acc, 0, 0, 0);
+    acc = __builtin_amdgcn_mfma_f32_32x32x16_bf16(a[0], b[2], acc, 0, 0, 0);
+    acc = __builtin_amdgcn_mfma_f32_32x32x16_bf16(a[1], b[0], acc, 0, 0, 0);
+    acc = __builtin_amdgcn_mfma_f32_32x32x16_bf16(a[0], b[1], acc, 0, 0, 0);
+    return __builtin_amdgcn_mfma_f32_32x32x16_bf16(a[0], b[0], acc, 0, 0, 0);
+}
+
+__host__ __device__ constexpr int shift_nph(int s) { return s == 0 ? 4 : (s == 3 ? 1 : 2); }
+
+struct ConvTTaps {
+    int tap[4][4];
+};
+
+template <int S>
+__host__ __device__ constexpr int shift_phase(int j) {
+    return S == 0 ? j : (S == 1 ? (j ? 1 : 0) : (S == 2 ? (j ? 2 : 0) : 0));
+}
+
+template <int WO, int WM, int TO, int TM>
+struct ConvTX3 {
+    static_assert(WO * WM == 4, "4 waves");
+    static constexpr int BKT = 16;
+    static constexpr int BO = WO * TO * 32;
+    static constexpr int BM = WM * TM * 32;
+    static constexpr int NCH = BM / 64;
+    static_assert(NCH >= 1 && NCH <= 4 && 4 % NCH == 0, "BM in {64,128,256}");
+    static constexpr int RSTEP = 4 / NCH;
+    static constexpr int XI = BKT * NCH / 4;
+    static constexpr int PB = 6 * BO * 16;
+    static_assert(PB % 1024 == 0, "phase planes split into whole 1-KB DMAs");
+    static constexpr int XB = BKT * BM * 4;
+    static constexpr int STAGE = XB + 4 * PB;
+    static constexpr int RING = 2 * STAGE;
+};
+
+template <int WO, int WM, int TO, int TM>
+__device__ __forceinline__ void convt_x3_loop(const GemmParams& p, const ConvTTaps& tt, char* smem, bool mvalid,
+                                              int nn, int a, int b, int wn, int o0, int ks_begin, int ks_end,
+                                              f32x16 (&acc)[4][TO][TM]) {
+    typedef ConvTX3<WO, WM, TO, TM> C;
+    constexpr int BKT = C::BKT, BO = C::BO, BM = C::BM, NCH = C::NCH, RSTEP = C::RSTEP, XI = C::XI, PB = C::PB,
+                  XB = C::XB, STAGE = C::STAGE;
+    const int tid = threadIdx.x;
+    const int lane = tid & 63;
+    const int wave = __builtin_amdgcn_readfirstlane(tid >> 6);
+    const int wo = wave / WM, wm = wave % WM;
+    const int cw = wave % NCH, r0 = wave / NCH;
+    const int in_hw = p.in_h * p.in_w;
+    const __amdgpu_buffer_rsrc_t xrsrc = __builtin_amdgcn_make_buffer_rsrc(
+        (void*)p.x, (short)0, (int)((int64_t)p.n * p.cin * in_hw * 4), 0x00020000);
+    const int xvbase = nn * p.cin * in_hw * 4;
+    const int c16n = p.cin / 16;
+
+    auto issue = [&](int ks, int slot) {
+        const int c = ks >> 2, sh = ks & 3;
+        const int ci0 = c * BKT;
+        const int iy = a - (sh & 1), ix = b - (sh >> 1);
+        const bool ok = mvalid && iy >= 0 && iy < p.in_h && ix >= 0 && ix < p.in_w;
+        const int voff = ok ? xvbase + (iy * p.in_w + ix) * 4 : 0x7ffffff0;
+        char* st = smem + slot * STAGE;
+        float* xs = reinterpret_cast<float*>(st);
+#pragma unroll
+        for (int j = 0; j < XI; ++j) {
+            const int row = r0 + RSTEP * j;
+            __builtin_amdgcn_raw_ptr_buffer_load_lds(
+                xrsrc, (__attribute__((address_space(3))) void*)(xs + row * BM + cw * 64), 4, voff,
+                (ci0 + row) * in_hw * 4, 0, 0);
+        }
+        const int nph = shift_nph(sh);
+        for (int j = wave; j < nph * (PB / 1024); j += 4) {
+            const int pj = j / (PB / 1024);
+            const int phase = sh == 0 ? pj : (sh == 1 ? (pj ? 1 : 0) : (sh == 2 ? (pj ? 2 : 0) : 0));
+            const int L = (j - pj * (PB / 1024)) * 64 + lane;
+            const int run = L / BO, o = L - run * BO;
+            const PhaseDev& q = p.ph[phase];
+            const short* src = q.wx3 + (q.wx3_stride ? (int64_t)wn * q.wx3_stride : 0) +
+                               ((((int64_t)tt.tap[sh][phase] * c16n + ci0 / 16) * 6 + run) * p.cout + o0 + o) * 8;
+            __builtin_amdgcn_global_load_lds((const void*)src, (__attribute__((address_space(3))) void*)(st + XB + j * 1024),
+                                             16, 0, 0);
+        }
+    };
+
+#pragma unroll
+    for (int ph = 0; ph < 4; ++ph)
+#pragma unroll
+        for (int i = 0; i < TO; ++i)
+#pragma unroll
+            for (int j = 0; j < TM; ++j)
+#pragma unroll
+                for (int r = 0; r < 16; ++r) acc[ph][i][j][r] = 0.f;
+
+    const int kh = lane >> 5, l32 = lane & 31;
+    if (ks_begin < ks_end) issue(ks_begin, 0);
+    auto step = [&](auto S_, int ks) {
+        constexpr int S = decltype(S_)::value;
+        constexpr int NP = shift_nph(S);
+        wait_vmcnt<0>();
+        __builtin_amdgcn_s_barrier();
+        asm volatile("" ::: "memory");
+        const char* st = smem + (S & 1) * STAGE;
+        const float* xcol = reinterpret_cast<const float*>(st) + wm * TM * 32 + l32;
+        bf16x8 bt[TM][3];
+#pragma unroll
+        for (int j = 0; j < TM; ++j) {
+            float xv[8];
+#pragma unroll
+            for (int e = 0; e < 8; ++e) xv[e] = xcol[(8 * kh + e) * BM + j * 32];
+            x3_split8(xv, bt[j]);
+        }
+        __builtin_amdgcn_sched_barrier(0);
+        if (ks + 1 < ks_end) issue(ks + 1, (S + 1) & 1);
+#pragma unroll
+        for (int pj = 0; pj < NP; ++pj) {
+            const short* Wp = reinterpret_cast<const short*>(st + XB + pj * PB);
+            bf16x8 at[TO][3];
+#pragma unroll
+            for (int i = 0; i < TO; ++i)
+#pragma unroll
+                for (int s = 0; s < 3; ++s)
+                    at[i][s] = *reinterpret_cast<const bf16x8*>(Wp + (((s * 2 + kh) * BO) + wo * TO * 32 + i * 32 + l32) * 8);
+#pragma unroll
+            for (int i = 0; i < TO; ++i)
+#pragma unroll
+                for (int j = 0; j < TM; ++j)
+                    acc[shift_phase<S>(pj)][i][j] = x3_mma(at[i], bt[j], acc[shift_phase<S>(pj)][i][j]);
+        }
+        asm volatile("s_waitcnt lgkmcnt(0)" ::: "memory");
+    };
+    for (int ks = ks_begin; ks < ks_end; ks += 4) {
+        step(std::integral_constant<int, 0>{}, ks);
+        step(std::integral_constant<int, 1>{}, ks + 1);
+        step(std::integral_constant<int, 2>{}, ks + 2);
+        step(std::integral_constant<int, 3>{}, ks + 3);
+    }
+}
+
+}
+
+int convt_up2_prepare(const float* x, int n, int cin, int h, int w, float* y, int cout, const smc_conv_phase* phases,
+                      int nphases, const float* s_in, float* workspace, int64_t workspace_bytes, void* stream,
+                      cg::GemmParams* p, cg::ConvTTaps* tt);
+bool convt_up2_shape_ok(int n, int cin, int cout, int h, int w);
+bool convt_up2_plan_ok(int n, int cin, int cout, int h, int w);
+
+}
diff --git a/stylemc_amd/csrc/fir_epi.hpp b/stylemc_amd/csrc/fir_epi.hpp
--- /dev/null
+++ b/stylemc_amd/csrc/fir_epi.hpp
@@ -0,0 +1,43 @@
+#pragma once
+#include "common.hpp"
+
+namespace smc {
+
+template <int FH, int FW>
+__device__ __forceinline__ void std_taps(float (&tp)[FH][FW]) {
+    constexpr float k[4] = {1.f, 3.f, 3.f, 1.f};
+#pragma unroll
+    for (int jy = 0; jy < FH; ++jy)
+#pragma unroll
+        for (int jx = 0; jx < FW; ++jx) tp[jy][jx] = k[jy] * k[jx] * 0.0625f;
+}
+
+template <bool NT>
+__device__ __forceinline__ void st_f2(float* p, float2 v) {
+    if (NT) {
+        typedef float f32x2 __attribute__((ext_vector_type(2)));
+        __builtin_nontemporal_store(f32x2{v.x, v.y}, reinterpret_cast<f32x2*>(p));
+    } else {
+        *reinterpret_cast<float2*>(p) = v;
+    }
+}
+
+__device__ __forceinline__ bool modact_lrelu_clamp(int act, float alpha, float clamp) {
+    return act == SMC_ACT_LRELU && alpha >= 0.f && alpha <= 1.f && clamp >= 0.f;
+}
+
+__device__ __forceinline__ float2 modact2(float2 u2, float dv, float2 nz, float bv, bool lrelu_clamp, int act,
+                                          float alpha, float gain, float clamp) {
+    float2 q;
+    if (lrelu_clamp) {
+        const float zx = __fmaf_rn(u2.x, dv, nz.x) + bv, zy = __fmaf_rn(u2.y, dv, nz.y) + bv;
+        q.x = lrelu_gain_clamp(zx, alpha, gain, clamp);
+        q.y = lrelu_gain_clamp(zy, alpha, gain, clamp);
+    } else {
+        q = make_float2(epi_y(u2.x, dv, nz.x, bv, act, alpha, gain, clamp),
+                        epi_y(u2.y, dv, nz.y, bv, act, alpha, gain, clamp));
+    }
+    return q;
+}
+
+}
diff --git a/stylemc_amd/csrc/modconv_aux.hip b/stylemc_amd/csrc/modconv_aux.hip
--- a/stylemc_amd/csrc/modconv_aux.hip
+++ b/stylemc_amd/csrc/modconv_aux.hip
@@ -1,6 +1,10 @@
 #include "common.hpp"
+#include "fir_epi.hpp"
 
 namespace {
+
+using smc::st_f2;
+using smc::std_taps;
 
 struct Epi {
     int mode;
@@ -217,14 +221,6 @@
             tp[jy][jx] = f[(flip ? jy : FH - 1 - jy) * FW + (flip ? jx : FW - 1 - jx)] * fgain;
 }
 
-template <int FH, int FW>
-__device__ __forceinline__ void std_taps(float (&tp)[FH][FW]) {
-    constexpr float k[4] = {1.f, 3.f, 3.f, 1.f};
-#pragma unroll
-    for (int jy = 0; jy < FH; ++jy)
-#pragma unroll
-        for (int jx = 0; jx < FW; ++jx) tp[jy][jx] = k[jy] * k[jx] * 0.0625f;
-}
 
 template <int FH, int FW>
 __global__ __launch_bounds__(256) void blur_act_fast(const float* t, int nsplit, int64_t split_stride, float* y, int c,
@@ -331,16 +327,6 @@
 #ifndef SMC_BLUR_PIPE
 #define SMC_BLUR_PIPE 1
 #endif
-template <bool NT>
-__device__ __forceinline__ void st_f2(float* p, float2 v) {
-    if (NT) {
-        typedef float f32x2 __attribute__((ext_vector_type(2)));
-        __builtin_nontemporal_store(f32x2{v.x, v.y}, reinterpret_cast<f32x2*>(p));
-    } else {
-        *reinterpret_cast<float2*>(p) = v;
-    }
-}
-
 template <int FH, int FW, int TPB, bool NT, bool STDF = false>
 __global__ __launch_bounds__(256, STDF ? SMC_BLUR_WGS : 1) void blur_act_v4(const float* t, int nsplit, int64_t split_stride, float* y, int c,
                                                    int t_h, int t_w, int tp_w, int y_h, int y_w, const float* f,
@@ -426,7 +412,7 @@
                 nz[i].y *= nstr;
             }
         }
-        const bool lrelu_clamp = e.act == SMC_ACT_LRELU && e.alpha >= 0.f && e.alpha <= 1.f && e.clamp >= 0.f;
+        const bool lrelu_clamp = smc::modact_lrelu_clamp(e.act, e.alpha, e.clamp);
 #pragma unroll
         for (int i = 0; i < 4; ++i) {
             const int oy = oy0 + 4 * ty + i;
@@ -438,15 +424,7 @@
                 continue;
             }
             if (e.u_save) st_f2<NT>(e.u_save + plane + pix, u2);
-            float2 q;
-            if (lrelu_clamp) {
-                const float zx = __fmaf_rn(u2.x, dv, nz[i].x) + bv, zy = __fmaf_rn(u2.y, dv, nz[i].y) + bv;
-                q.x = smc::lrelu_gain_clamp(zx, e.alpha, e.gain, e.clamp);
-                q.y = smc::lrelu_gain_clamp(zy, e.alpha, e.gain, e.clamp);
-            } else {
-                q = make_float2(smc::epi_y(u2.x, dv, nz[i].x, bv, e.act, e.alpha, e.gain, e.clamp),
-                                smc::epi_y(u2.y, dv, nz[i].y, bv, e.act, e.alpha, e.gain, e.clamp));
-            }
+            const float2 q = smc::modact2(u2, dv, nz[i], bv, lrelu_clamp, e.act, e.alpha, e.gain, e.clamp);
             st_f2<NT>(y + plane + pix, q);
         }
     }
diff --git a/stylemc_amd/modconv.py b/stylemc_amd/modconv.py
--- a/stylemc_amd/modconv.py
+++ b/stylemc_amd/modconv.py
@@ -196,6 +196,33 @@
 
 def wino_flops(n, cin, cout, h, w):
     return 2.0 * n * cin * cout * (h // 2) * (w // 2) * 16
+
+
+FUSED_UP = True
+FUSED_UP_COUT = (32,)
+
+
+def fused_up_ok(spec, n, cin, h, w):
+    P = spec.packed
+    if not (FUSED_UP and spec.up == 2 and spec.std_filter and P.use_x3 and P.cout in FUSED_UP_COUT):
+        return False
+    lib = _hip.load()
+    if not (lib.smc_modconv_up2_supported(n, cin, P.cout, h, w) and lib.smc_modconv_up2_plan_ok(n, cin, P.cout, h, w)):
+        return False
+    return all(p is not None for p in P.x3_phases)
+
+
+def fused_up(x, y, phases, nph, cin, cout, s, epi, alg_flops=0.0, alg_bytes=0):
+    n, _, h, w = x.shape
+    lib = _hip.load()
+    ws_bytes = lib.smc_conv_gemm_workspace_size(n, cin, cout, 2 * h + 1, 2 * w + 1, phases, nph)
+    ws = torch.empty(max(ws_bytes // 4, 1), device=x.device, dtype=torch.float32) if ws_bytes > 0 else None
+    tm = _hip.timer()
+    tok = tm.wrap(alg_flops, alg_bytes, kind="direct_x3") if tm is not None else None
+    _hip.call("smc_modconv_up2_f32", x.data_ptr(), n, cin, h, w, y.data_ptr(), cout, phases, nph, _hip.ptr(s), None,
+              4, 4, 4.0, ctypes.byref(epi), _hip.ptr(ws), ws_bytes, _hip.stream())
+    if tok is not None:
+        tm.finish(tok)
 
 
 def _epilogue(mode, d=None, noise=None, noise_nstride=0, strength=None, bias=None, act="linear", alpha=0.0,
@@ -285,6 +312,10 @@
         gemm(x, y, phases, nph, cin, P.cout, s=styles, epi=epi,
              alg_flops=conv_flops(n, cin, P.cout, r_h, r_w, P.k * P.k),
              alg_bytes=4 * x.numel() + 4 * y.numel() * (2 if u is not None else 1) + wbytes)
+    elif fused_up_ok(spec, n, cin, h, w):
+        fused_up(x, y, phases, nph, cin, P.cout, styles, epi,
+                 alg_flops=conv_flops(n, cin, P.cout, h, w, 9),
+                 alg_bytes=4 * x.numel() + 4 * y.numel() * (2 if u is not None else 1) + wbytes)
     else:
         t = torch.empty(n, P.cout, th, tw, device=x.device, dtype=torch.float32)
         gemm(x, t, phases, nph, cin, P.cout, s=styles, epi=_epilogue(_hip.EPI_STORE),
```

After: 478.1 images/s (median of 6 runs). 1.0% higher.
